# Jerrypiglet/monosdf

Measured on AMD Instinct MI355X. Metric: rays/sec fwd+bwd, 1024 rays x 98 samples, 8x256 SDF MLP, higher is better.
Workload: dtype f32; 1 GPU; configs[1]: 1024 rays x 98 samples per GPU, ImplicitNetwork 8x256 + RenderingNetwork 289-256-256-3, error-bounded sampler, random-init weights (density beta 0.1), training step = fwd + loss + bwd + Adam, a different one of 8 ray batches every step; rays_per_gpu=1024, samples_per_ray=98, ray_batches=8, matrix_core=fp32

## Files before the change

### include/monosdf_hip.h

```cpp
#ifndef MONOSDF_HIP_H
#define MONOSDF_HIP_H

#include <stdint.h>
#include "monosdf_plan.h"

#ifdef __cplusplus
extern "C" {
#endif

#define MSDF_OK 0
#define MSDF_ERR_ARG 1
#define MSDF_ERR_LAUNCH 2
#define MSDF_ERR_UNSUPPORTED 3

#define MSDF_ABI_VERSION 8
int msdf_abi_version(void);

int msdf_hash_encode_forward(const float* inputs, const float* embeddings, const int* offsets, float* outputs,
                             uint32_t B, uint32_t D, uint32_t C, uint32_t L, float S, uint32_t H,
                             int calc_grad_inputs, float* dy_dx, void* stream);
int msdf_hash_encode_backward(const float* grad, const float* inputs, const float* embeddings, const int* offsets,
                              float* grad_embeddings, uint32_t B, uint32_t D, uint32_t C, uint32_t L, float S,
                              uint32_t H, int calc_grad_inputs, const float* dy_dx, float* grad_inputs,
                              void* stream);
int msdf_hash_encode_second_backward(const float* grad, const float* inputs, const float* embeddings,
                                     const int* offsets, uint32_t B, uint32_t D, uint32_t C, uint32_t L, float S,
                                     uint32_t H, int calc_grad_inputs, const float* dy_dx,
                                     const float* grad_grad_inputs, float* grad_grad, float* grad2_embeddings,
                                     void* stream);

int64_t msdf_hash_scatter_workspace_bytes(uint32_t B, uint32_t C, uint32_t L, uint64_t n_entries);
int msdf_hash_encode_backward_ws(const float* grad, const float* inputs, const float* embeddings, const int* offsets,
                                 float* grad_embeddings, uint32_t B, uint32_t D, uint32_t C, uint32_t L, float S,
                                 uint32_t H, int calc_grad_inputs, const float* dy_dx, float* grad_inputs,
                                 uint64_t n_entries, void* workspace, uint64_t workspace_bytes, void* stream);
int msdf_hash_encode_second_backward_ws(const float* grad, const float* inputs, const float* embeddings,
                                        const int* offsets, uint32_t B, uint32_t D, uint32_t C, uint32_t L, float S,
                                        uint32_t H, int calc_grad_inputs, const float* dy_dx,
                                        const float* grad_grad_inputs, float* grad_grad, float* grad2_embeddings,
                                        uint64_t n_entries, void* workspace, uint64_t workspace_bytes, void* stream);
int msdf_hash_encode_backward_fused(const float* grad_first, const float* grad_second, const float* inputs,
                                    const int* offsets, float* grad_embeddings, uint32_t B, uint32_t D, uint32_t C,
                                    uint32_t L, float S, uint32_t H, const float* grad_grad_inputs,
                                    uint64_t n_entries, void* workspace, uint64_t workspace_bytes, void* stream);
int msdf_hash_encode_backward_fused_out(const float* grad_first, const float* grad_second, const float* inputs,
                                        const int* offsets, float* grad_embeddings, uint32_t B, uint32_t D, uint32_t C,
                                        uint32_t L, float S, uint32_t H, const float* grad_grad_inputs,
                                        uint64_t n_entries, void* workspace, uint64_t workspace_bytes, void* stream);

int msdf_hash_node_forward(const float* x, double divide_factor, float* x01_out, const float* embeddings,
                           const int* offsets, float* feat, uint32_t pitch, uint32_t B, uint32_t C, uint32_t L,
                           float S, uint32_t H, float* dy_dx, void* stream);
int msdf_hash_node_input_gradient(const float* g, uint32_t pitch, const float* dy_dx, uint32_t B, uint32_t C,
                                  uint32_t L, float scale, float* inout, void* stream);
int msdf_hash_node_second_grad(const float* g_a, const float* g_b, uint32_t n_split, float scale, float* gg_out,
                               const float* dy_dx, float* grad_grad, uint32_t pitch, uint32_t B, uint32_t C,
                               uint32_t L, void* stream);
int msdf_hash_transpose(const float* src, float* dst, const float* src2, float* dst2, uint32_t L, uint32_t B,
                        uint32_t C, uint32_t pitch, int to_point_major, void* stream);
int msdf_hash_node_scatter(const float* grad_first, const float* grad_second, uint32_t pitch, const float* inputs,
                           const int* offsets, float* grad_embeddings, uint32_t B, uint32_t C, uint32_t L, float S,
                           uint32_t H, const float* grad_grad_inputs, uint64_t n_entries, void* workspace,
                           uint64_t workspace_bytes, void* stream);

int msdf_pack_weights(const msdf_plan_t* plan, const msdf_packrule_t* rules_dev, const int* maps_dev,
                      const float* flat_w, const float* flat_b, void* wpack, float* bpack, void* stream);

typedef struct {
  const float* v;
  const float* g;
  const float* b;
  int32_t rows, cols;
  int32_t w_off;
  int32_t b_off;
  int32_t row_off;
  int32_t has_g;
} msdf_wn_layer_t;
int msdf_weightnorm_forward(const msdf_wn_layer_t* layers_dev, const int* row_layer_dev, int total_rows,
                            float* flat_w, float* flat_b, float* norms, void* stream);
int msdf_weightnorm_backward(const msdf_wn_layer_t* layers_dev, const int* row_layer_dev, int total_rows,
                             const float* g_flat_w, const float* norms, float* dv_flat, float* dg_rows, void* stream);

int msdf_sdf_forward(const msdf_plan_t* plan, const void* wpack, const float* bpack, const float* x,
                     const float* aux, int P, float clamp_radius, float sphere_scale, float* sdf, void* stream);
int msdf_sdf_forward_if(const msdf_plan_t* plan, const void* wpack, const float* bpack, const float* x,
                        const float* aux, int P, float clamp_radius, float sphere_scale, float* sdf,
                        const uint32_t* run_flag, void* stream);
int msdf_sdf_forward_lm(const msdf_plan_t* plan, const void* wpack, const float* bpack, const float* x,
                        const float* aux, int aux_C, int aux_LC, int P, float clamp_radius, float sphere_scale,
                        float* sdf, const uint32_t* run_flag, void* stream);

typedef struct {
  const void* wpack;
  const float* bpack;
  const float* x;
  const float* aux;
  int32_t P, P_pad;
  int32_t n_clamp;
  int32_t n_feat;
  float clamp_radius, sphere_scale;
  float* sdf;
  float* feat;
  float* nrm;
  float* r_aux;
  unsigned char* clamped;
  float* H;
  float* PM;
  float* IN0;
  int32_t save;
  int32_t aux_C;
  int32_t aux_LC;
  float aux_dx_scale;
  const float* dy_dx;
} msdf_fg_args_t;
int msdf_sdf_fwd_grad(const msdf_plan_t* plan, const msdf_fg_args_t* args, void* stream);

typedef struct {
  const void* wpack;
  const float* bpack;
  const float* x;
  int32_t P, P_pad;
  int32_t n_feat;
  int32_t n_split;
  const float* g_sdf;
  const float* g_feat;
  const float* g_nrm;
  const float* g_raux;
  const unsigned char* clamped;
  const float* H;
  const float* PM;
  float* QB;
  float* T;
  float* AB;
  float* GSDF;
  float* QLAST;
  float* g_aux;
  const float* g_sdf_b;
  const float* g_nrm_b;
  int32_t aux_C, aux_LC;
  const float* dy_dx;
  float* gg_out;
  float aux_dx_scale;
  int32_t pad_;
} msdf_bw_args_t;
int msdf_sdf_backward(const msdf_plan_t* plan, const msdf_bw_args_t* args, void* stream);

typedef struct {
  const void* wpack;
  const float* bpack;
  const float* x;
  const float* dirs;
  const float* nrm;
  const float* feat;
  const float* code;
  int32_t P, P_pad;
  int32_t spr;
  int32_t save;
  float* rgb;
  float* H;
  float* MISC;
} msdf_color_fwd_args_t;
int msdf_color_forward(const msdf_plan_t* plan, const msdf_color_fwd_args_t* args, void* stream);

typedef struct {
  const void* wpack;
  const float* bpack;
  const float* rgb;
  const float* g_rgb;
  int32_t P, P_pad;
  const float* H;
  float* AB;
  float* g_feat;
  float* g_misc;
  float* g_nrm;
} msdf_color_bwd_args_t;
int msdf_color_backward(const msdf_plan_t* plan, const msdf_color_bwd_args_t* args, void* stream);

int msdf_wgrad(const msdf_wgrad_item_t* items_dev, const int32_t* wg_map_dev, int n_wgs, float* partials,
               int P_pad, int precision , const float* base0, const float* base1 , void* stream);
int msdf_reduce(const msdf_reduce_rule_t* rules_dev, int n_rules, const int* maps_dev, const float* partials,
                float* dst, void* stream);

typedef struct {
  const float* z;
  const float* sdf;
  const float* rgb;
  const float* nrm;
  const float* beta;
  const float* depth_scale;
  int32_t N, S;
  int32_t white_bkgd;
  float bg0, bg1, bg2;
  float* weights;
  float* rgb_values;
  float* depth_values;
  float* normal_map;
  float* wsum;
  const float* pose;
  int32_t pose_stride;
  int32_t depth_scale_stride;
  float* depth_vals;
} msdf_composite_args_t;
int msdf_composite_forward(const msdf_composite_args_t* args, void* stream);

typedef struct {
  const float* z;
  const float* sdf;
  const float* rgb;
  const float* nrm;
  const float* beta;
  const float* depth_scale;
  const float* weights;
  const float* wsum;
  const float* depth_values;
  const float* g_rgb_values;
  const float* g_depth;
  const float* g_normal;
  const float* g_weights;
  int32_t N, S;
  int32_t white_bkgd;
  float bg0, bg1, bg2;
  float* g_sdf;
  float* g_rgb;
  float* g_nrm;
  float* g_beta_part;
  const float* pose;
  int32_t pose_stride;
  int32_t depth_scale_stride;
} msdf_composite_bwd_args_t;
int msdf_composite_backward(const msdf_composite_bwd_args_t* args, void* stream);

int msdf_beta_eff(const float* beta_raw, float beta_min, float* out, void* stream);
int msdf_beta_grad(const float* beta_raw, const float* g_part, int n, float* g_raw, void* stream);

typedef struct {
  const float* rgb;
  const float* nrm;
  const float* depth;
  const float* g1;
  const float* g2;
  int32_t N, M;
  float w_normal, w_depth, w_eik, w_smooth;
  float* g_rgb; float* g_nrm; float* g_depth; float* g_g1; float* g_g2;
  float* partial;
} msdf_probe_loss_args_t;
int msdf_probe_loss(const msdf_probe_loss_args_t* args, void* stream);

typedef struct {
  const float* rgb;
  const float* depth;
  const float* normal;
  const float* sdf;
  const float* grad_theta;
  const float* grad_nei;
  const float* rgb_gt;
  const float* depth_gt;
  const float* normal_gt;
  const float* mask_gt;
  int32_t N, S, E;
  int32_t gamma;
  int32_t scale_invariant;
  float w_eik, w_smooth, w_depth, w_nl1, w_ncos;
  float* mask;
  float* out;
  float* g_rgb; float* g_depth; float* g_normal; float* g_theta; float* g_nei;
} msdf_monosdf_loss_args_t;
int msdf_monosdf_loss(const msdf_monosdf_loss_args_t* args, void* stream);

typedef struct {
  const float* ray_o;
  const float* ray_d;
  int32_t N;
  int32_t M;
  int32_t m_max;
  int32_t n_eval, n_final, n_extra;
  int32_t round_idx, max_rounds;
  int32_t training;
  int32_t beta_iters;
  float near, far, bound;
  float eps, add_tiny;
  float lemma;
  const float* beta0;
  float* z;
  float* sdf;
  float* new_z;
  const float* new_sdf;
  int32_t* new_pos;
  float* pts;
  float* beta;
  uint32_t* flags;
  const float* jitter;
  const float* u_final;
  float* final_z;
  const int64_t* extra_idx;
  const int64_t* eik_idx;
  float* z_out;
  float* z_eik;
  float* pts_out;
  const float* eik_uniform;
  const float* nei_rand;
  float* far_out;
  int32_t* rounds_out;
  float* dbg_dstar;
  float* dbg_err0;
  float* dbg_cdf;
  const float* eik_u;
  int32_t eik_unit;
  int32_t pad_;
} msdf_sampler_args_t;
int msdf_sampler_init(const msdf_sampler_args_t* args, void* stream);
int msdf_sampler_beta(const msdf_sampler_args_t* args, void* stream);
int msdf_sampler_resample(const msdf_sampler_args_t* args, void* stream);
int msdf_sampler_finish(const msdf_sampler_args_t* args, void* stream);

int msdf_sampler_error_bound(const float* z, const float* sdf, const float* dstar, const float* beta,
                             int beta_stride, int N, int M, float* out, void* stream);

int msdf_laplace_density(const float* sdf, const float* beta, int beta_stride, int64_t n, int cols, float* out,
                         void* stream);
int msdf_laplace_density_backward(const float* sdf, const float* beta, int beta_stride, int64_t n, int cols,
                                  const float* g, float* g_sdf, float* g_beta_elem, void* stream);

int msdf_camera_rays(const float* uv, const float* pose, const float* intrinsics, int n, float* ray_dirs,
                     float* ray_dirs_cam, float* cam_loc, void* stream);

int msdf_pixel_rays(const int64_t* ray_idx, int n, const int32_t* frame_list, int n_frames, const float* pose_all,
                    const float* intrinsics_all, int width, int hw, float* ray_dirs, float* ray_dirs_cam,
                    float* cam_loc, float* ray_pose, int32_t* frame_pos, const float* const* gt_src,
                    float* const* gt_dst, const int32_t* gt_channels, int n_gt, void* stream);

int64_t msdf_mc_workspace_bytes(int nx, int ny, int nz);
int msdf_mc_count(const float* vol, int nx, int ny, int nz, float level, void* workspace, int64_t* totals,
                  void* stream);
int msdf_mc_emit(const float* vol, int nx, int ny, int nz, float level, float sx, float sy, float sz,
                 const void* workspace, float* verts, float* normals, int32_t* faces, void* stream);

int msdf_nn_split_count(int64_t n_ref, int64_t n_query, int n_splits);
int64_t msdf_nn_workspace_bytes(int64_t n_ref, int64_t n_query, int n_splits);
int msdf_nn_search(const float* ref, int64_t n_ref, const float* query, int64_t n_query, int n_splits,
                   void* workspace, float* dist, int32_t* idx, void* stream);
int msdf_voxel_keys(const float* points, int64_t n, const float* min_bound, float voxel_size, int64_t* keys,
                    void* stream);
int msdf_voxel_mean(const float* points, const int64_t* order, const int64_t* seg_start, int64_t n, int64_t m,
                    float* out, void* stream);

int msdf_raster_depth(const float* verts, int64_t n_verts, const int32_t* faces, int64_t n_faces, const float* w2c,
                      int n_views, float fx, float fy, float cx, float cy, int height, int width, float znear,
                      float zfar, float pixel_center, float* depth, void* stream);
int msdf_tsdf_integrate(const float* depth, const float* w2c, int n_views, float fx, float fy, float cx, float cy,
                        int height, int width, float ox, float oy, float oz, int i0, int j0, int k0, int nx, int ny,
                        int nz, float voxel_length, float sdf_trunc, float depth_trunc, int resume, float* tsdf,
                        float* weight, void* stream);
int msdf_tsdf_face_keep(const float* verts, int64_t n_verts, const int32_t* faces, int64_t n_faces,
                        const float* weight, int nx, int ny, int nz, uint8_t* keep, void* stream);
int msdf_cull_vertices(const float* verts, int64_t n_verts, const float* w2c, int n_views, float fx, float fy, float cx,
                       float cy, int height, int width, uint8_t* seen, void* stream);

#ifdef __cplusplus
}
#endif
#endif
```

### monosdf_amd/_lib.py

```python
import ctypes as C
import os

_HERE = os.path.dirname(os.path.abspath(__file__))
LIB_PATH = os.environ.get('MONOSDF_HIP_LIB') or os.path.join(_HERE, 'libmonosdf_hip.so')

MAX_LAYERS = 10
MAX_TILES = 17


class Layer(C.Structure):
    _fields_ = [(n, C.c_int32) for n in
                ('kt', 'ot', 'wf_off', 'wb_off', 'bias_off', 'skip_tile', 'hpre', 'qpre', 'abpre',
                 'ktp', 'otp', 'pad_')]


class Plan(C.Structure):
    _fields_ = [(n, C.c_int32) for n in
                ('n_layers', 'e_tiles', 'aux_tiles', 'n_freqs', 'sdf_slot', 'feat_tiles', 'hsum',
                 'qsum', 'absum', 'wsdf_off', 'mode', 'out_act', 'precision', 'out_rows')] + [('layer', Layer * MAX_LAYERS)]


class PackRule(C.Structure):
    _fields_ = [('w_off', C.c_int32), ('b_off', C.c_int32), ('rows', C.c_int32), ('cols', C.c_int32),
                ('rowmap_off', C.c_int32), ('colmap_off', C.c_int32), ('scale', C.c_float),
                ('pad_', C.c_int32)]


class WgradItem(C.Structure):
    _fields_ = [('x', C.c_int64), ('y', C.c_int64), ('v', C.c_int64),
                ('part_off', C.c_int64), ('colsum_off', C.c_int64), ('vrow_off', C.c_int64),
                ('x_ld', C.c_int32), ('y_ld', C.c_int32), ('wx', C.c_int32), ('wy', C.c_int32),
                ('n_splits', C.c_int32), ('bufs', C.c_int32)]


class ReduceRule(C.Structure):
    _fields_ = [('part_off', C.c_int64), ('dst_off', C.c_int64), ('n_blocks', C.c_int32),
                ('wx', C.c_int32), ('wy', C.c_int32), ('rowmap_off', C.c_int32),
                ('colmap_off', C.c_int32), ('dst_ld', C.c_int32), ('fixed_row', C.c_int32),
                ('scale', C.c_float)]


_P = C.c_void_p


class FgArgs(C.Structure):
    _fields_ = [('wpack', _P), ('bpack', _P), ('x', _P), ('aux', _P),
                ('P', C.c_int32), ('P_pad', C.c_int32), ('n_clamp', C.c_int32), ('n_feat', C.c_int32),
                ('clamp_radius', C.c_float), ('sphere_scale', C.c_float),
                ('sdf', _P), ('feat', _P), ('nrm', _P), ('r_aux', _P), ('clamped', _P),
                ('H', _P), ('PM', _P), ('IN0', _P), ('save', C.c_int32), ('aux_C', C.c_int32), ('aux_LC', C.c_int32),
                ('aux_dx_scale', C.c_float), ('dy_dx', _P)]


class BwArgs(C.Structure):
    _fields_ = [('wpack', _P), ('bpack', _P), ('x', _P),
                ('P', C.c_int32), ('P_pad', C.c_int32), ('n_feat', C.c_int32), ('n_split', C.c_int32),
                ('g_sdf', _P), ('g_feat', _P), ('g_nrm', _P), ('g_raux', _P), ('clamped', _P),
                ('H', _P), ('PM', _P), ('QB', _P), ('T', _P), ('AB', _P), ('GSDF', _P), ('QLAST', _P),
                ('g_aux', _P), ('g_sdf_b', _P), ('g_nrm_b', _P), ('aux_C', C.c_int32), ('aux_LC', C.c_int32),
                ('dy_dx', _P), ('gg_out', _P), ('aux_dx_scale', C.c_float), ('pad_', C.c_int32)]


class ColorFwdArgs(C.Structure):
    _fields_ = [('wpack', _P), ('bpack', _P), ('x', _P), ('dirs', _P), ('nrm', _P), ('feat', _P),
                ('code', _P), ('P', C.c_int32), ('P_pad', C.c_int32), ('spr', C.c_int32),
                ('save', C.c_int32), ('rgb', _P), ('H', _P), ('MISC', _P)]


class ColorBwdArgs(C.Structure):
    _fields_ = [('wpack', _P), ('bpack', _P), ('rgb', _P), ('g_rgb', _P),
                ('P', C.c_int32), ('P_pad', C.c_int32), ('H', _P), ('AB', _P), ('g_feat', _P),
                ('g_misc', _P), ('g_nrm', _P)]


class CompositeArgs(C.Structure):
    _fields_ = [('z', _P), ('sdf', _P), ('rgb', _P), ('nrm', _P), ('beta', _P), ('depth_scale', _P),
                ('N', C.c_int32), ('S', C.c_int32), ('white_bkgd', C.c_int32),
                ('bg0', C.c_float), ('bg1', C.c_float), ('bg2', C.c_float),
                ('weights', _P), ('rgb_values', _P), ('depth_values', _P), ('normal_map', _P),
                ('wsum', _P), ('pose', _P), ('pose_stride', C.c_int32), ('depth_scale_stride', C.c_int32),
                ('depth_vals', _P)]


class CompositeBwdArgs(C.Structure):
    _fields_ = [('z', _P), ('sdf', _P), ('rgb', _P), ('nrm', _P), ('beta', _P), ('depth_scale', _P),
                ('weights', _P), ('wsum', _P), ('depth_values', _P), ('g_rgb_values', _P),
                ('g_depth', _P), ('g_normal', _P), ('g_weights', _P),
                ('N', C.c_int32), ('S', C.c_int32), ('white_bkgd', C.c_int32),
                ('bg0', C.c_float), ('bg1', C.c_float), ('bg2', C.c_float),
                ('g_sdf', _P), ('g_rgb', _P), ('g_nrm', _P), ('g_beta_part', _P),
                ('pose', _P), ('pose_stride', C.c_int32), ('depth_scale_stride', C.c_int32)]


class WnLayer(C.Structure):
    _fields_ = [('v', _P), ('g', _P), ('b', _P), ('rows', C.c_int32), ('cols', C.c_int32),
                ('w_off', C.c_int32), ('b_off', C.c_int32), ('row_off', C.c_int32), ('has_g', C.c_int32)]


class ProbeLossArgs(C.Structure):
    _fields_ = [('rgb', _P), ('nrm', _P), ('depth', _P), ('g1', _P), ('g2', _P), ('N', C.c_int32), ('M', C.c_int32),
                ('w_normal', C.c_float), ('w_depth', C.c_float), ('w_eik', C.c_float), ('w_smooth', C.c_float),
                ('g_rgb', _P), ('g_nrm', _P), ('g_depth', _P), ('g_g1', _P), ('g_g2', _P), ('partial', _P)]


class MonoSdfLossArgs(C.Structure):
    _fields_ = [(n, _P) for n in ('rgb', 'depth', 'normal', 'sdf', 'grad_theta', 'grad_nei', 'rgb_gt', 'depth_gt',
                                  'normal_gt', 'mask_gt')] + \
               [(n, C.c_int32) for n in ('N', 'S', 'E', 'gamma', 'scale_invariant')] + \
               [(n, C.c_float) for n in ('w_eik', 'w_smooth', 'w_depth', 'w_nl1', 'w_ncos')] + \
               [(n, _P) for n in ('mask', 'out', 'g_rgb', 'g_depth', 'g_normal', 'g_theta', 'g_nei')]


class SamplerArgs(C.Structure):
    _fields_ = [('ray_o', _P), ('ray_d', _P), ('N', C.c_int32), ('M', C.c_int32), ('m_max', C.c_int32),
                ('n_eval', C.c_int32), ('n_final', C.c_int32), ('n_extra', C.c_int32),
                ('round_idx', C.c_int32), ('max_rounds', C.c_int32), ('training', C.c_int32),
                ('beta_iters', C.c_int32), ('near', C.c_float), ('far', C.c_float), ('bound', C.c_float),
                ('eps', C.c_float), ('add_tiny', C.c_float), ('lemma', C.c_float),
                ('beta0', _P), ('z', _P), ('sdf', _P), ('new_z', _P), ('new_sdf', _P), ('new_pos', _P),
                ('pts', _P), ('beta', _P), ('flags', _P), ('jitter', _P), ('u_final', _P), ('final_z', _P),
                ('extra_idx', _P), ('eik_idx', _P), ('z_out', _P), ('z_eik', _P), ('pts_out', _P),
                ('eik_uniform', _P), ('nei_rand', _P), ('far_out', _P), ('rounds_out', _P),
                ('dbg_dstar', _P), ('dbg_err0', _P), ('dbg_cdf', _P), ('eik_u', _P), ('eik_unit', C.c_int32),
                ('pad_', C.c_int32)]


_ERR = {1: 'invalid argument', 2: 'kernel launch failed', 3: 'unsupported configuration'}

_SIGNATURES = {
    'msdf_abi_version': [],
    'msdf_hash_encode_forward': [_P, _P, _P, _P, C.c_uint32, C.c_uint32, C.c_uint32, C.c_uint32,
                                 C.c_float, C.c_uint32, C.c_int, _P, _P],
    'msdf_hash_encode_backward': [_P, _P, _P, _P, _P, C.c_uint32, C.c_uint32, C.c_uint32, C.c_uint32,
                                  C.c_float, C.c_uint32, C.c_int, _P, _P, _P],
    'msdf_hash_encode_second_backward': [_P, _P, _P, _P, C.c_uint32, C.c_uint32, C.c_uint32,
                                         C.c_uint32, C.c_float, C.c_uint32, C.c_int, _P, _P, _P, _P, _P],
    'msdf_hash_scatter_workspace_bytes': [C.c_uint32, C.c_uint32, C.c_uint32, C.c_uint64],
    'msdf_hash_encode_backward_ws': [_P, _P, _P, _P, _P, C.c_uint32, C.c_uint32, C.c_uint32, C.c_uint32,
                                     C.c_float, C.c_uint32, C.c_int, _P, _P, C.c_uint64, _P, C.c_uint64, _P],
    'msdf_hash_encode_second_backward_ws': [_P, _P, _P, _P, C.c_uint32, C.c_uint32, C.c_uint32, C.c_uint32,
                                            C.c_float, C.c_uint32, C.c_int, _P, _P, _P, _P, C.c_uint64, _P,
                                            C.c_uint64, _P],
    'msdf_hash_encode_backward_fused': [_P, _P, _P, _P, _P, C.c_uint32, C.c_uint32, C.c_uint32, C.c_uint32,
                                        C.c_float, C.c_uint32, _P, C.c_uint64, _P, C.c_uint64, _P],
    'msdf_hash_encode_backward_fused_out': [_P, _P, _P, _P, _P, C.c_uint32, C.c_uint32, C.c_uint32, C.c_uint32,
                                            C.c_float, C.c_uint32, _P, C.c_uint64, _P, C.c_uint64, _P],
    'msdf_hash_node_forward': [_P, C.c_double, _P, _P, _P, _P, C.c_uint32, C.c_uint32, C.c_uint32, C.c_uint32,
                               C.c_float, C.c_uint32, _P, _P],
    'msdf_hash_node_input_gradient': [_P, C.c_uint32, _P, C.c_uint32, C.c_uint32, C.c_uint32, C.c_float, _P, _P],
    'msdf_hash_node_second_grad': [_P, _P, C.c_uint32, C.c_float, _P, _P, _P, C.c_uint32, C.c_uint32, C.c_uint32,
                                   C.c_uint32, _P],
    'msdf_hash_transpose': [_P, _P, _P, _P, C.c_uint32, C.c_uint32, C.c_uint32, C.c_uint32, C.c_int, _P],
    'msdf_hash_node_scatter': [_P, _P, C.c_uint32, _P, _P, _P, C.c_uint32, C.c_uint32, C.c_uint32, C.c_float,
                               C.c_uint32, _P, C.c_uint64, _P, C.c_uint64, _P],
    'msdf_weightnorm_forward': [_P, _P, C.c_int, _P, _P, _P, _P],
    'msdf_weightnorm_backward': [_P, _P, C.c_int, _P, _P, _P, _P, _P],
    'msdf_pack_weights': [C.POINTER(Plan), _P, _P, _P, _P, _P, _P, _P],
    'msdf_sdf_forward': [C.POINTER(Plan), _P, _P, _P, _P, C.c_int, C.c_float, C.c_float, _P, _P],
    'msdf_sdf_forward_if': [C.POINTER(Plan), _P, _P, _P, _P, C.c_int, C.c_float, C.c_float, _P, _P, _P],
    'msdf_sdf_forward_lm': [C.POINTER(Plan), _P, _P, _P, _P, C.c_int, C.c_int, C.c_int, C.c_float, C.c_float, _P, _P, _P],
    'msdf_sdf_fwd_grad': [C.POINTER(Plan), C.POINTER(FgArgs), _P],
    'msdf_sdf_backward': [C.POINTER(Plan), C.POINTER(BwArgs), _P],
    'msdf_color_forward': [C.POINTER(Plan), C.POINTER(ColorFwdArgs), _P],
    'msdf_color_backward': [C.POINTER(Plan), C.POINTER(ColorBwdArgs), _P],
    'msdf_wgrad': [_P, _P, C.c_int, _P, C.c_int, C.c_int, _P, _P, _P],
    'msdf_camera_rays': [_P, _P, _P, C.c_int, _P, _P, _P, _P],
    'msdf_pixel_rays': [_P, C.c_int, _P, C.c_int, _P, _P, C.c_int, C.c_int, _P, _P, _P, _P, _P, _P, _P, _P, C.c_int, _P],
    'msdf_monosdf_loss': [C.POINTER(MonoSdfLossArgs), _P],
    'msdf_reduce': [_P, C.c_int, _P, _P, _P, _P],
    'msdf_composite_forward': [C.POINTER(CompositeArgs), _P],
    'msdf_composite_backward': [C.POINTER(CompositeBwdArgs), _P],
    'msdf_beta_eff': [_P, C.c_float, _P, _P],
    'msdf_beta_grad': [_P, _P, C.c_int, _P, _P],
    'msdf_probe_loss': [C.POINTER(ProbeLossArgs), _P],
    'msdf_sampler_init': [C.POINTER(SamplerArgs), _P],
    'msdf_sampler_beta': [C.POINTER(SamplerArgs), _P],
    'msdf_sampler_resample': [C.POINTER(SamplerArgs), _P],
    'msdf_sampler_finish': [C.POINTER(SamplerArgs), _P],
    'msdf_sampler_error_bound': [_P, _P, _P, _P, C.c_int, C.c_int, C.c_int, _P, _P],
    'msdf_laplace_density': [_P, _P, C.c_int, C.c_int64, C.c_int, _P, _P],
    'msdf_laplace_density_backward': [_P, _P, C.c_int, C.c_int64, C.c_int, _P, _P, _P, _P],
    'msdf_mc_workspace_bytes': [C.c_int, C.c_int, C.c_int],
    'msdf_mc_count': [_P, C.c_int, C.c_int, C.c_int, C.c_float, _P, _P, _P],
    'msdf_mc_emit': [_P, C.c_int, C.c_int, C.c_int, C.c_float, C.c_float, C.c_float, C.c_float, _P, _P, _P, _P, _P],
    'msdf_nn_split_count': [C.c_int64, C.c_int64, C.c_int],
    'msdf_nn_workspace_bytes': [C.c_int64, C.c_int64, C.c_int],
    'msdf_nn_search': [_P, C.c_int64, _P, C.c_int64, C.c_int, _P, _P, _P, _P],
    'msdf_voxel_keys': [_P, C.c_int64, _P, C.c_float, _P, _P],
    'msdf_voxel_mean': [_P, _P, _P, C.c_int64, C.c_int64, _P, _P],
    'msdf_raster_depth': [_P, C.c_int64, _P, C.c_int64, _P, C.c_int, C.c_float, C.c_float, C.c_float, C.c_float,
                          C.c_int, C.c_int, C.c_float, C.c_float, C.c_float, _P, _P],
    'msdf_tsdf_integrate': [_P, _P, C.c_int, C.c_float, C.c_float, C.c_float, C.c_float, C.c_int, C.c_int,
                            C.c_float, C.c_float, C.c_float, C.c_int, C.c_int, C.c_int, C.c_int, C.c_int, C.c_int,
                            C.c_float, C.c_float, C.c_float, C.c_int, _P, _P, _P],
    'msdf_tsdf_face_keep': [_P, C.c_int64, _P, C.c_int64, _P, C.c_int, C.c_int, C.c_int, _P, _P],
    'msdf_cull_vertices': [_P, C.c_int64, _P, C.c_int, C.c_float, C.c_float, C.c_float, C.c_float, C.c_int, C.c_int,
                           _P, _P],
}

ABI_VERSION = 8

_lib = None


def load():
    global _lib
    if _lib is not None:
        return _lib
    if not os.path.exists(LIB_PATH):
        raise RuntimeError(
            'monosdf_amd: %s not found -- build it with `python __graft_entry__.py` or '
            '`make -C monosdf_amd/csrc` (there is no non-HIP fallback)' % LIB_PATH)
    lib = C.CDLL(LIB_PATH)
    for name, argtypes in _SIGNATURES.items():
        fn = getattr(lib, name)
        fn.argtypes = argtypes
        fn.restype = C.c_int64 if name.endswith('_bytes') else C.c_int
    if lib.msdf_abi_version() != ABI_VERSION:
        raise RuntimeError('monosdf_amd: ABI version mismatch, rebuild the library')
    _lib = lib
    return lib


def exported_symbols():
    return sorted(_SIGNATURES)


PROFILE = None


PROFILE_NAMES = None


def call(name, *args):
    prof = PROFILE
    if prof is not None and PROFILE_NAMES is not None and name not in PROFILE_NAMES:
        prof = None
    if prof is not None:
        import torch
        e0, e1 = torch.cuda.Event(enable_timing=True), torch.cuda.Event(enable_timing=True)
        e0.record()
    status = getattr(load(), name)(*args)
    if prof is not None:
        e1.record()
        prof.setdefault(name, []).append((e0, e1))
    if status != 0:
        raise RuntimeError('%s failed: %s' % (name, _ERR.get(status, 'status %d' % status)))


def ptr(t):
    return None if t is None else C.c_void_p(t.data_ptr())


def stream_ptr():
    import torch
    return C.c_void_p(torch.cuda.current_stream().cuda_stream)
```

### monosdf_amd/csrc/mlp_core.h

```cpp
#pragma once
#include <type_traits>
#include "common.h"
#include "../../include/monosdf_plan.h"

#define MT MSDF_MAX_TILES
#ifndef MLP_WAVES
#define MLP_WAVES 4
#endif
#define MLP_PTS_PER_WAVE 16
#define CHUNK_OT 2
#define LDS_BUF_F4 (CHUNK_OT * MT * 64)

#define V4ZERO ((v4f){0.f, 0.f, 0.f, 0.f})

__device__ __forceinline__ v4f mfma4(const v4f a, const v4f b, v4f c) {
  c = __builtin_amdgcn_mfma_f32_16x16x4f32(a.x, b.x, c, 0, 0, 0);
  c = __builtin_amdgcn_mfma_f32_16x16x4f32(a.y, b.y, c, 0, 0, 0);
  c = __builtin_amdgcn_mfma_f32_16x16x4f32(a.z, b.z, c, 0, 0, 0);
  c = __builtin_amdgcn_mfma_f32_16x16x4f32(a.w, b.w, c, 0, 0, 0);
  return c;
}

__device__ __forceinline__ void mfma4_pair(const v4f a0, const v4f a1, const v4f b, v4f& c0, v4f& c1) {
  c0 = __builtin_amdgcn_mfma_f32_16x16x4f32(a0.x, b.x, c0, 0, 0, 0);
// ... 117 lines not shown
        if (!DYN) {
          v4f a0 = w0[0];
          v4f c0 = acc[o0];
#pragma unroll
          for (int kt = 0; kt < KMAX; ++kt) {
            v4f n0 = a0;
            if (kt + 1 < KMAX) n0 = w0[(kt + 1) * 64];
            __builtin_amdgcn_sched_barrier(0);
            c0 = mfma4(a0, in[kt], c0);
            a0 = n0;
          }
          acc[o0] = c0;
        } else {
#pragma unroll
          for (int kt = 0; kt < KMAX; ++kt) {
            if (kt < K) acc[o0] = mfma4(w0[kt * 64], in[kt], acc[o0]);
          }
        }
      }
      hk.post(o0, 2 * c + 1, 2 * c + 1 < MT && 2 * c + 1 < OT, acc[o0], acc[o1]);
        }
      }
      __syncthreads();
    }
  }
}

template <class Hooks>
__device__ __forceinline__ void gemm_dispatch(const int kp, v4f (&acc)[MT], const v4f (&in)[MT], const int OT,
                                              const v4f* __restrict__ wsrc, v4f* lds, Hooks& hk) {
  switch (kp) {
    case 3: gemm_tiles<3, 4>(acc, in, OT, 3, wsrc, lds, hk); break;
    case 5: gemm_tiles<5, 3>(acc, in, OT, 5, wsrc, lds, hk); break;
    case 16: gemm_tiles<16, 1>(acc, in, OT, 16, wsrc, lds, hk); break;
    case 17: gemm_tiles<17, 1>(acc, in, OT, 17, wsrc, lds, hk); break;
    default: gemm_tiles<0, 1>(acc, in, OT, kp, wsrc, lds, hk); break;
  }
  hk.drain();
}

__device__ __forceinline__ void zero_tiles(v4f (&a)[MT]) {
#pragma unroll
  for (int t = 0; t < MT; ++t) a[t] = V4ZERO;
}

__device__ __forceinline__ void place_tiles(v4f (&dst)[MT], const int base, const v4f (&src)[5], const int n) {
#pragma unroll
  for (int t = 0; t < MT; ++t) {
    if (t >= base) {
      v4f v = V4ZERO;
#pragma unroll
      for (int j = 0; j < 5; ++j)
        if (j < n && t == base + j) v = src[j];
      dst[t] = v;
    }
  }
}

__device__ __forceinline__ void gather_tiles(v4f (&dst)[5], const v4f (&src)[MT], const int base, const int n) {
#pragma unroll
  for (int t = 0; t < MT; ++t) {
#pragma unroll
    for (int j = 0; j < 5; ++j)
      if (j < n && t == base + j) dst[j] += src[t];
  }
}

__device__ __forceinline__ void pe_slot(const int j, const int n_valid, const float x0, const float x1,
                                        const float x2, float& val, float& dval, int& c) {
  val = 0.f; dval = 0.f; c = 3;
  if (j < 3) {
    c = j;
    val = (c == 0) ? x0 : (c == 1) ? x1 : x2;
    dval = 1.f;
  } else if (j < n_valid) {
    const int m = j - 3;
    const int k = m / 6;
    const int w = m - 6 * k;
    c = (w >= 3) ? w - 3 : w;
    const float xc = (c == 0) ? x0 : (c == 1) ? x1 : x2;
    const float f = (float)(1 << k);
    float sn, cs;
    sincosf(xc * f, &sn, &cs);
    if (w < 3) { val = sn; dval = f * cs; } else { val = cs; dval = -f * sn; }
  }
}

__device__ __forceinline__ void pe_values(v4f (&e)[5], const float x0, const float x1, const float x2,
                                          const int n_freqs) {
  const int q = lane_id() >> 4;
  const int n_valid = 3 + 6 * n_freqs;
#pragma unroll
  for (int t = 0; t < 3; ++t) {
#pragma unroll
    for (int r = 0; r < 4; ++r) {
      float v, dv; int c;
      pe_slot(16 * t + 4 * q + r, n_valid, x0, x1, x2, v, dv, c);
      e[t][r] = v;
    }
  }
}

__device__ __forceinline__ void pe_jacobian_transpose(const v4f (&r)[5], const float x0, const float x1,
                                                      const float x2, const int n_freqs, float& n0, float& n1,
                                                      float& n2) {
  const int q = lane_id() >> 4;
  const int n_valid = 3 + 6 * n_freqs;
  float a0 = 0.f, a1 = 0.f, a2 = 0.f;
#pragma unroll
  for (int t = 0; t < 3; ++t) {
#pragma unroll
    for (int k = 0; k < 4; ++k) {
      float v, dv; int c;
      pe_slot(16 * t + 4 * q + k, n_valid, x0, x1, x2, v, dv, c);
      const float w = r[t][k] * dv;
      a0 += (c == 0) ? w : 0.f;
      a1 += (c == 1) ? w : 0.f;
      a2 += (c == 2) ? w : 0.f;
    }
  }
  n0 = sum_over_quarters(a0);
  n1 = sum_over_quarters(a1);
  n2 = sum_over_quarters(a2);
}

__device__ __forceinline__ void pe_jacobian(v4f (&rbar)[5], const float x0, const float x1, const float x2,
                                            const int n_freqs, const float g0, const float g1, const float g2) {
  const int q = lane_id() >> 4;
  const int n_valid = 3 + 6 * n_freqs;
#pragma unroll
  for (int t = 0; t < 3; ++t) {
#pragma unroll
    for (int k = 0; k < 4; ++k) {
      float v, dv; int c;
      pe_slot(16 * t + 4 * q + k, n_valid, x0, x1, x2, v, dv, c);
      const float g = (c == 0) ? g0 : (c == 1) ? g1 : (c == 2) ? g2 : 0.f;
      rbar[t][k] = dv * g;
    }
  }
}


struct CoreF32 {
  typedef v4f wvec;
  static constexpr int THREADS = 64 * MLP_WAVES;
  static constexpr int PTS_PER_WG = MLP_PTS_PER_WAVE * MLP_WAVES;
  static constexpr int WGS_PER_CU = 8 / MLP_WAVES;
  static constexpr int LDS_BYTES = 2 * LDS_BUF_F4 * 16;
  static constexpr bool BIAS_IN_HOOKS = true;
#ifndef MLP_F32_AUX_LEVEL_MAJOR
#define MLP_F32_AUX_LEVEL_MAJOR true
#endif
  static constexpr bool AUX_LEVEL_MAJOR = MLP_F32_AUX_LEVEL_MAJOR;
  static __device__ __forceinline__ float softplus(const float a) {
    float h, s;
    softplus100(a, h, s);
    return h;
  }
  template <class Hooks>
  static __device__ __forceinline__ void gemm(const int kp, v4f (&acc)[MT], const v4f (&in)[MT], const int OT,
                                              const wvec* __restrict__ wsrc, void* lds, Hooks&& hk) {
    gemm_dispatch(kp, acc, in, OT, wsrc, (v4f*)lds, hk);
  }
  template <class Hooks>
  static __device__ __forceinline__ void gemm_bias(const int kp, v4f (&acc)[MT], const v4f (&in)[MT], const int OT,
                                                   const wvec* __restrict__ wsrc, void* lds, Hooks&& hk,
                                                   const float* __restrict__ bias) {
    zero_tiles(acc);
    BiasHooks<typename std::remove_reference<Hooks>::type> bh(hk, bias, OT);
    gemm_dispatch(kp, acc, in, OT, wsrc, (v4f*)lds, bh);
  }
};

__device__ __forceinline__ void pack_bias_rows(const msdf_plan_t& plan, const int l, const msdf_packrule_t& R,
                                               const int* __restrict__ rowmap, const int* __restrict__ colmap,
                                               const float* __restrict__ W, const float* __restrict__ flat_b,
                                               float* __restrict__ bpack, const int t0, const int stride) {
  const msdf_layer_t L = plan.layer[l];
  for (int i = t0; i < 16 * L.ot; i += stride) {
    const int row = rowmap[i];
    bpack[L.bias_off + i] = (row >= 0) ? flat_b[R.b_off + row] : 0.f;
  }
  if (l == plan.n_layers - 1 && plan.wsdf_off >= 0) {
    for (int rr = 0; rr < plan.out_rows; ++rr) {
      const int row = rowmap[plan.sdf_slot + rr];
      for (int i = t0; i < 16 * L.kt; i += stride) {
        const int col = colmap[i];
        bpack[plan.wsdf_off + rr * 16 * L.kt + i] = (col >= 0 && row >= 0) ? R.scale * W[(size_t)row * R.cols + col] : 0.f;
      }
    }
  }
}
```

### monosdf_amd/csrc/mlp_core_b16.h

```cpp
#pragma once
#include "mlp_core.h"


typedef __bf16 v8bf __attribute__((ext_vector_type(8)));
typedef __attribute__((address_space(3))) v8bf lds_v8bf;

__device__ __forceinline__ float softplus100_lean(const float a) {
  const float e = __builtin_amdgcn_exp2f(-fabsf(a * 144.26950408889634f));
  const float relu = __int_as_float(max(__float_as_int(a), 0));
  return fmaf(0.006931471805599453f, __builtin_amdgcn_logf(1.0f + e), relu);
}

#define KB_MAX ((MT + 1) / 2)
#define B16_WAVES 4

template <int NS>
struct B16Cfg {
  static_assert(NS == 2 || NS == 3, "two planes (bf16x3) or three (bf16x6)");
  static constexpr int CH = (NS == 2) ? 2 : 1;
  static constexpr int BUF_V8 = CH * KB_MAX * NS * 64;
  static constexpr int RING = (NS == 2) ? 3 : 2;
};

template <int NS>
// ... 37 lines not shown
__device__ __forceinline__ void b16_chunk_issue(const v8bf* __restrict__ src, v8bf* dst, const int n_v8) {
  const int wave = __builtin_amdgcn_readfirstlane(threadIdx.x >> 6);
  const int lane = threadIdx.x & 63;
  const int pieces = n_v8 >> 6;
#pragma unroll
  for (int i = 0; i < (PIECES_MAX + B16_WAVES - 1) / B16_WAVES; ++i) {
    const int piece = wave + B16_WAVES * i;
    if (piece < pieces) {
      __builtin_amdgcn_global_load_lds((const __attribute__((address_space(1))) void*)(src + piece * 64 + lane),
                                       (__attribute__((address_space(3))) void*)(dst + piece * 64), 16, 0, 0);
    }
  }
}

template <int NS>
__device__ __forceinline__ v4f b16_step(v4f c, const v8bf (&f)[NS], const B16Act<NS>& act, const int kb) {
  c = __builtin_amdgcn_mfma_f32_16x16x32_bf16(f[0], act.p[0][kb], c, 0, 0, 0);
  c = __builtin_amdgcn_mfma_f32_16x16x32_bf16(f[0], act.p[1][kb], c, 0, 0, 0);
  c = __builtin_amdgcn_mfma_f32_16x16x32_bf16(f[1], act.p[0][kb], c, 0, 0, 0);
  if constexpr (NS == 3) {
    c = __builtin_amdgcn_mfma_f32_16x16x32_bf16(f[0], act.p[2][kb], c, 0, 0, 0);
    c = __builtin_amdgcn_mfma_f32_16x16x32_bf16(f[1], act.p[1][kb], c, 0, 0, 0);
    c = __builtin_amdgcn_mfma_f32_16x16x32_bf16(f[2], act.p[0][kb], c, 0, 0, 0);
  }
  return c;
}

template <int NS>
__device__ __forceinline__ v4f b16_tile_dyn(v4f c, const v8bf* __restrict__ w, const B16Act<NS>& act, const int KB) {
  v8bf a[NS];
#pragma unroll
  for (int n = 0; n < NS; ++n) a[n] = w[n * 64];
#pragma unroll
  for (int kb = 0; kb < KB_MAX; ++kb) {
    if (kb < KB) {
      v8bf nx[NS];
#pragma unroll
      for (int n = 0; n < NS; ++n) nx[n] = a[n];
      if (kb + 1 < KB_MAX && kb + 1 < KB) {
#pragma unroll
        for (int n = 0; n < NS; ++n) nx[n] = w[((kb + 1) * NS + n) * 64];
      }
      __builtin_amdgcn_sched_barrier(0);
      c = b16_step<NS>(c, a, act, kb);
#pragma unroll
      for (int n = 0; n < NS; ++n) a[n] = nx[n];
    }
  }
  return c;
}

template <int NS, int KB_T, class Hooks>
__device__ __forceinline__ void gemm_b16(v4f (&acc)[MT], const B16Act<NS>& act, const int OT, const int kb_rt,
                                         const v8bf* __restrict__ wsrc, v8bf* lds, Hooks& hk) {
  typedef B16Cfg<NS> Cfg;
  constexpr int CH = Cfg::CH;
  constexpr int RING = Cfg::RING;
  constexpr bool DYN = (KB_T == 0);
  constexpr int KMAX = DYN ? KB_MAX : KB_T;
  const int KB = DYN ? kb_rt : KB_T;
  const int ch_v8 = CH * KB * NS * 64;
  const int lane = threadIdx.x & 63;
  const int nchunks = (OT + CH - 1) / CH;
  constexpr int BUF = Cfg::BUF_V8;
  b16_chunk_issue<CH * KMAX * NS>(wsrc, lds, ch_v8);
  __syncthreads();
#pragma unroll
  for (int c = 0; c < (MT + CH - 1) / CH; ++c) {
    if (c < nchunks) {
      const int buf = c & 1;
      if (c + 1 < nchunks)
        b16_chunk_issue<CH * KMAX * NS>(wsrc + (size_t)(c + 1) * ch_v8, lds + (buf ^ 1) * BUF, ch_v8);
      const int t0 = CH * c;
      if ((t0 & 1) == 0) hk.pre(t0, t0 + 1);
      const v8bf* w = lds + buf * BUF + lane;
      const lds_v8bf* wl0 = (const lds_v8bf*)w;
      asm volatile("" : "+v"(wl0));
      static_assert(BUF * 16 <= 65536, "fragment offsets must fit the ds_read immediate");
#define B16_FRAG(i, plane) (wl0[((i) * NS + (plane)) * 64])
      if constexpr (DYN) {
#pragma unroll
        for (int o = 0; o < CH; ++o) {
          const int ot = CH * c + o;
          if (ot < MT && ot < OT) {
            const int oi = (ot < MT) ? ot : 0;
            acc[oi] = b16_tile_dyn<NS>(acc[oi], w + o * KB * NS * 64, act, KB);
          }
        }
      } else {
        const int n_o = OT - CH * c;
        v8bf fr[RING][NS];
#pragma unroll
        for (int i = 0; i < RING - 1; ++i) {
          if (i < CH * KB_T) {
#pragma unroll
            for (int n = 0; n < NS; ++n) fr[i][n] = B16_FRAG(i, n);
          }
        }
#pragma unroll
        for (int o = 0; o < CH; ++o) {
          const int ot = CH * c + o;
          if (ot < MT && o < n_o) {
            const int oi = (ot < MT) ? ot : 0;
            v4f cc = acc[oi];
#pragma unroll
            for (int kb = 0; kb < KB_T; ++kb) {
              const int i = o * KB_T + kb;
              if (i + RING - 1 < CH * KB_T) {
#pragma unroll
                for (int n = 0; n < NS; ++n) fr[(i + RING - 1) % RING][n] = B16_FRAG(i + RING - 1, n);
              }
              __builtin_amdgcn_sched_barrier(0);
              cc = b16_step<NS>(cc, fr[i % RING], act, kb);
            }
            acc[oi] = cc;
          }
        }
      }
#undef B16_FRAG
      const int t_last = CH * c + CH - 1;
      if ((t_last & 1) == 1 || t_last + 1 >= OT) {
        const int e = t_last & ~1;
        if (e < MT)
          hk.post(e, e + 1, e + 1 < MT && e + 1 < OT, acc[e < MT ? e : 0], acc[(e + 1 < MT) ? e + 1 : 0]);
      }
      __syncthreads();
    }
  }
}

template <int NS, class Hooks>
__device__ __forceinline__ void gemm_b16_dispatch(const int kbp, v4f (&acc)[MT], const B16Act<NS>& act, const int OT,
                                                  const v8bf* __restrict__ wsrc, v8bf* lds, Hooks& hk) {
  switch (kbp) {
    case 2: gemm_b16<NS, 2>(acc, act, OT, 2, wsrc, lds, hk); break;
    case 3: gemm_b16<NS, 3>(acc, act, OT, 3, wsrc, lds, hk); break;
    case 8: gemm_b16<NS, 8>(acc, act, OT, 8, wsrc, lds, hk); break;
    case 9: gemm_b16<NS, 9>(acc, act, OT, 9, wsrc, lds, hk); break;
    default: gemm_b16<NS, 0>(acc, act, OT, kbp, wsrc, lds, hk); break;
  }
  hk.drain();
}

template <int NS>
struct CoreB16N {
  typedef v8bf wvec;
  static constexpr int PLANES = NS;
  static constexpr int THREADS = 64 * B16_WAVES;
  static constexpr int PTS_PER_WG = MLP_PTS_PER_WAVE * B16_WAVES;
  static constexpr int WGS_PER_CU = 2;
  static constexpr int LDS_BYTES = 2 * B16Cfg<NS>::BUF_V8 * 16;
  static constexpr bool BIAS_IN_HOOKS = (NS == 3);
  static constexpr bool AUX_LEVEL_MAJOR = false;
  static __device__ __forceinline__ float softplus(const float a) {
    if constexpr (NS == 2) return softplus100_lean(a);
    float h, s;
    softplus100(a, h, s);
    return h;
  }
  template <class Hooks>
  static __device__ __forceinline__ void gemm(const int kbp, v4f (&acc)[MT], const v4f (&in)[MT], const int OT,
                                              const wvec* __restrict__ wsrc, void* lds, Hooks&& hk) {
    B16Act<NS> act;
    b16_from_tiles<NS>(act, in);
    gemm_b16_dispatch<NS>(kbp, acc, act, OT, wsrc, (v8bf*)lds, hk);
  }
  template <class Hooks>
  static __device__ __forceinline__ void gemm_bias(const int kbp, v4f (&acc)[MT], const v4f (&in)[MT], const int OT,
                                                   const wvec* __restrict__ wsrc, void* lds, Hooks&& hk,
                                                   const float* __restrict__ bias) {
    B16Act<NS> act;
    b16_from_tiles<NS>(act, in);
    zero_tiles(acc);
    BiasHooks<typename std::remove_reference<Hooks>::type> bh(hk, bias, OT);
    gemm_b16_dispatch<NS>(kbp, acc, act, OT, wsrc, (v8bf*)lds, bh);
  }
};
typedef CoreB16N<2> CoreB16;
typedef CoreB16N<3> CoreB16X6;
```

### monosdf_amd/csrc/sampler.hip

```cpp
#include "common.h"

#define SMP_WAVES 4

__device__ __forceinline__ float smp_scan_incl(float v) {
  const int lane = lane_id();
#pragma unroll
  for (int d = 1; d < 64; d <<= 1) {
    const float o = __shfl_up(v, d, 64);
    if (lane >= d) v += o;
  }
  return v;
}
__device__ __forceinline__ float smp_sum(float v) {
#pragma unroll
  for (int d = 32; d >= 1; d >>= 1) v += __shfl_xor(v, d, 64);
  return v;
}
__device__ __forceinline__ float smp_max(float v) {
#pragma unroll
  for (int d = 32; d >= 1; d >>= 1) v = fmaxf(v, __shfl_xor(v, d, 64));
  return v;
}
__device__ __forceinline__ float smp_density(const float s, const float beta) {
  const float e = expm1f(-fabsf(s) / beta);
  const float sg = (s > 0.f) ? 1.f : (s < 0.f) ? -1.f : 0.f;
  return (1.0f / beta) * (0.5f + 0.5f * sg * e);
}
__device__ __forceinline__ float smp_linspace01(const int j, const int n) {
  const float step = 1.0f / (float)(n - 1);
  return (j < n / 2) ? step * (float)j : 1.0f - step * (float)(n - 1 - j);
}

typedef msdf_sampler_args_t SmpArgs;

__global__ void __launch_bounds__(64 * SMP_WAVES) smp_init_k(const SmpArgs a) {
  const int ray = blockIdx.x * SMP_WAVES + (threadIdx.x >> 6);
  if (ray >= a.N) return;
  const int lane = lane_id();
  if (ray == 0 && a.flags != nullptr)
    for (int i = lane; i < 2 * a.max_rounds; i += 64) a.flags[i] = 0u;
  const int n = a.n_eval;
  const float o0 = a.ray_o[ray * 3 + 0], o1 = a.ray_o[ray * 3 + 1], o2 = a.ray_o[ray * 3 + 2];
  const float d0 = a.ray_d[ray * 3 + 0], d1 = a.ray_d[ray * 3 + 1], d2 = a.ray_d[ray * 3 + 2];
  const float ta0 = (-a.bound - o0) / (d0 + 1e-15f), tb0 = (a.bound - o0) / (d0 + 1e-15f);
  const float ta1 = (-a.bound - o1) / (d1 + 1e-15f), tb1 = (a.bound - o1) / (d1 + 1e-15f);
  const float ta2 = (-a.bound - o2) / (d2 + 1e-15f), tb2 = (a.bound - o2) / (d2 + 1e-15f);
  float near_c = fmaxf(fmaxf(fminf(ta0, tb0), fminf(ta1, tb1)), fminf(ta2, tb2));
  float far_c = fminf(fminf(fmaxf(ta0, tb0), fmaxf(ta1, tb1)), fmaxf(ta2, tb2));
  if (far_c < near_c) far_c = 1e9f;
  const float far = (a.bound > 0.f) ? fminf(far_c, a.far) : a.far;
  const float near = a.near;
  float sumsq = 0.f;
  float* zrow = a.z + (size_t)ray * a.m_max;
  auto zu = [&](int k) { const float t = smp_linspace01(k, n); return near * (1.f - t) + far * t; };
  auto zfin = [&](int k) {
    float z = zu(k);
    if (a.jitter != nullptr) {
      const float zl = (k > 0) ? 0.5f * (zu(k) + zu(k - 1)) : zu(0);
      const float zh = (k + 1 < n) ? 0.5f * (zu(k + 1) + zu(k)) : zu(n - 1);
      z = zl + (zh - zl) * a.jitter[(size_t)ray * n + k];
    }
    return z;
  };
  for (int j = lane; j < n; j += 64) {
    const float z = zfin(j);
    zrow[j] = z;
    a.new_z[(size_t)ray * n + j] = z;
    a.new_pos[(size_t)ray * n + j] = j;
    float* p = a.pts + ((size_t)ray * n + j) * 3;
    p[0] = o0 + z * d0; p[1] = o1 + z * d1; p[2] = o2 + z * d2;
    if (j + 1 < n) {
      const float dz = zfin(j + 1) - z;
      sumsq += dz * dz;
    }
  }
  sumsq = smp_sum(sumsq);
  if (lane == 0) {
    a.beta[ray] = sqrtf(a.lemma * sumsq);
    if (a.far_out != nullptr) a.far_out[ray] = far;
  }
}

struct SmpLds {
  float* z; float* sdf; float* dist; float* dstar; float* tmp; float* snew;
};
__device__ __forceinline__ SmpLds smp_lds(float* base, const int m_max, const int n_eval) {
  const int w = threadIdx.x >> 6;
  const int per = 5 * (m_max + 1) + n_eval;
  float* p = base + (size_t)w * per;
  SmpLds l;
  l.z = p; l.sdf = p + (m_max + 1); l.dist = p + 2 * (m_max + 1); l.dstar = p + 3 * (m_max + 1);
  l.tmp = p + 4 * (m_max + 1); l.snew = p + 5 * (m_max + 1);
  return l;
}
__device__ __forceinline__ void smp_sync() {
  __builtin_amdgcn_fence(__ATOMIC_RELEASE, "workgroup");
  __builtin_amdgcn_wave_barrier();
  __builtin_amdgcn_fence(__ATOMIC_ACQUIRE, "workgroup");
}

__device__ __forceinline__ bool smp_round_active(const SmpArgs& a) {
  return a.round_idx == 0 || a.flags[2 * (a.round_idx - 1) + 1] != 0u;
}

__device__ __forceinline__ void smp_load_ray(const SmpArgs& a, const SmpLds& l, const int ray, const bool scatter) {
  const int lane = lane_id();
  const int M = a.M;
  const float* zrow = a.z + (size_t)ray * a.m_max;
  float* srow = a.sdf + (size_t)ray * a.m_max;
  for (int i = lane; i < M; i += 64) { l.z[i] = zrow[i]; l.sdf[i] = srow[i]; }
  smp_sync();
  if (scatter) {
    for (int j = lane; j < a.n_eval; j += 64)
      l.sdf[a.new_pos[(size_t)ray * a.n_eval + j]] = a.new_sdf[(size_t)ray * a.n_eval + j];
    smp_sync();
    for (int i = lane; i < M; i += 64) srow[i] = l.sdf[i];
  }
  for (int i = lane; i + 1 < M; i += 64) {
    const float aa = l.z[i + 1] - l.z[i];
    const float b = fabsf(l.sdf[i]), c = fabsf(l.sdf[i + 1]);
    const bool first = aa * aa + b * b <= c * c;
    const bool second = aa * aa + c * c <= b * b;
    float ds = 0.f;
    if (first) ds = b;
    if (second) ds = c;
    if (!first && !second && (b + c - aa > 0.f)) {
      const float s = (aa + b + c) / 2.0f;
      const float area = s * (s - aa) * (s - b) * (s - c);
      ds = (2.0f * sqrtf(area)) / aa;
    }
    const float s0 = l.sdf[i], s1 = l.sdf[i + 1];
    const float sg0 = (s0 > 0.f) ? 1.f : (s0 < 0.f) ? -1.f : 0.f;
    const float sg1 = (s1 > 0.f) ? 1.f : (s1 < 0.f) ? -1.f : 0.f;
    l.dist[i] = aa;
    const float dsv = (sg0 * sg1 == 1.f) ? ds : 0.f;
    l.dstar[i] = dsv;
    if (scatter && a.dbg_dstar != nullptr) a.dbg_dstar[(size_t)ray * a.m_max + i] = dsv;
  }
  smp_sync();
}

__device__ __forceinline__ float smp_error_bound(const SmpLds& l, const int M, const float beta) {
  const int lane = lane_id();
  float carry_fe = 0.f, carry_err = 0.f, best = -1e30f;
  const float inv4b2 = 1.0f / (4.0f * beta * beta);
  for (int base = 0; base < M - 1; base += 64) {
    const int i = base + lane;
    const bool ok = i < M - 1;
    float fe = 0.f, er = 0.f;
    if (ok) {
      const float d = l.dist[i];
      fe = d * smp_density(l.sdf[i], beta);
      er = expf(-l.dstar[i] / beta) * (d * d) * inv4b2;
    }
    const float fe_incl = smp_scan_incl(fe);
    const float er_incl = smp_scan_incl(er);
    if (ok) {
      const float integral = carry_fe + fe_incl - fe;
      const float errint = carry_err + er_incl;
      const float bound = (fminf(expf(errint), 1.0e6f) - 1.0f) * expf(-integral);
      best = fmaxf(best, bound);
    }
    carry_fe += __shfl(fe_incl, 63, 64);
    carry_err += __shfl(er_incl, 63, 64);
  }
  return smp_max(best);
}

__global__ void __launch_bounds__(64 * SMP_WAVES) smp_beta_k(const SmpArgs a) {
  extern __shared__ float smp_lds_mem[];
  const int ray = blockIdx.x * SMP_WAVES + (threadIdx.x >> 6);
  if (ray >= a.N || !smp_round_active(a)) return;
  const SmpLds l = smp_lds(smp_lds_mem, a.m_max, a.n_eval);
  smp_load_ray(a, l, ray, true);
  const float beta0 = a.beta0[0];
  float beta = a.beta[ray];
  const float e0 = smp_error_bound(l, a.M, beta0);
  if (a.dbg_err0 != nullptr && lane_id() == 0) a.dbg_err0[ray] = e0;
  if (e0 <= a.eps) beta = beta0;
  float lo = beta0, hi = beta;
  const int iters = (e0 <= a.eps) ? 0 : a.beta_iters;
  for (int it = 0; it < iters; ++it) {
    const float mid = (lo + hi) / 2.0f;
    const float e = smp_error_bound(l, a.M, mid);
    if (e <= a.eps) hi = mid;
    if (e > a.eps) lo = mid;
  }
  if (lane_id() == 0) {
    a.beta[ray] = hi;
    atomicMax(a.flags + 2 * a.round_idx, __float_as_uint(hi));
  }
}

__global__ void __launch_bounds__(64 * SMP_WAVES) smp_resample_k(const SmpArgs a) {
  extern __shared__ float smp_lds_mem[];
  const int ray = blockIdx.x * SMP_WAVES + (threadIdx.x >> 6);
  if (ray >= a.N || !smp_round_active(a)) return;
  const int lane = lane_id();
  const int M = a.M;
  const SmpLds l = smp_lds(smp_lds_mem, a.m_max, a.n_eval);
  const float beta0 = a.beta0[0];
  const float maxbeta = __uint_as_float(a.flags[2 * a.round_idx]);
  const bool unconverged = maxbeta > beta0;
  const bool more = unconverged && (a.round_idx + 1 < a.max_rounds);
  if (ray == 0 && lane == 0) a.flags[2 * a.round_idx + 1] = more ? 1u : 0u;
  smp_load_ray(a, l, ray, false);
  const float beta = a.beta[ray];
  const float inv4b2 = 1.0f / (4.0f * beta * beta);

  float carry_fe = 0.f, carry_err = 0.f, psum = 0.f;
  for (int base = 0; base < M; base += 64) {
    const int i = base + lane;
    const bool ok = i < M;
    float fe = 0.f, er = 0.f;
    if (ok) {
      const float d = (i + 1 < M) ? l.dist[i] : 1e10f;
      fe = d * smp_density(l.sdf[i], beta);
      if (more && i + 1 < M) er = expf(-l.dstar[i] / beta) * (l.dist[i] * l.dist[i]) * inv4b2;
    }
    float fprev = __shfl_up(fe, 1, 64);
    if (lane == 0) fprev = 0.f;
    const float fe_excl = smp_scan_incl(fprev);
    const float fe_incl = fe_excl + fe;
    const float er_incl = smp_scan_incl(er);
    if (ok && i + 1 < M) {
      const float trans = expf(-(carry_fe + fe_excl));
      float p;
      if (more) p = (fminf(expf(carry_err + er_incl), 1.0e6f) - 1.0f) * trans + a.add_tiny;
      else p = (1.0f - expf(-fe)) * trans + 1e-5f;
      l.tmp[i] = p;
      psum += p;
    }
    carry_fe += __shfl(fe_incl, 63, 64);
    carry_err += __shfl(er_incl, 63, 64);
  }
  psum = smp_sum(psum);
  smp_sync();
  float carry = 0.f;
  for (int base = 0; base < M - 1; base += 64) {
    const int i = base + lane;
    const float p = (i < M - 1) ? l.tmp[i] / psum : 0.f;
    const float incl = smp_scan_incl(p);
    if (i < M - 1) l.dstar[i + 1] = carry + incl;
    carry += __shfl(incl, 63, 64);
  }
  if (lane == 0) l.dstar[0] = 0.f;
  smp_sync();
  const float* cdf = l.dstar;
  if (a.dbg_cdf != nullptr)
    for (int i = lane; i < M; i += 64) a.dbg_cdf[(size_t)ray * a.m_max + i] = cdf[i];

  const int n_new = more ? a.n_eval : a.n_final;
  for (int j = lane; j < n_new; j += 64) {
    float u;
    if (more || !a.training || a.u_final == nullptr) u = smp_linspace01(j, n_new);
    else u = a.u_final[(size_t)ray * a.n_final + j];
    int lo = 0, hi = M;
    while (lo < hi) {
      const int mid = (lo + hi) >> 1;
      if (cdf[mid] <= u) lo = mid + 1; else hi = mid;
    }
    const int below = max(lo - 1, 0), above = min(lo, M - 1);
    float denom = cdf[above] - cdf[below];
    if (denom < 1e-5f) denom = 1.0f;
    const float t = (u - cdf[below]) / denom;
    const float s = l.z[below] + t * (l.z[above] - l.z[below]);
    l.snew[j] = s;
  }
  smp_sync();

  if (!more) {
    for (int j = lane; j < n_new; j += 64) a.final_z[(size_t)ray * a.n_final + j] = l.snew[j];
    return;
  }
  const float o0 = a.ray_o[ray * 3 + 0], o1 = a.ray_o[ray * 3 + 1], o2 = a.ray_o[ray * 3 + 2];
  const float d0 = a.ray_d[ray * 3 + 0], d1 = a.ray_d[ray * 3 + 1], d2 = a.ray_d[ray * 3 + 2];
  float* zrow = a.z + (size_t)ray * a.m_max;
  float* srow = a.sdf + (size_t)ray * a.m_max;
  for (int i = lane; i < M; i += 64) {
    const float zi = l.z[i];
    int cnt = 0;
    for (int k = 0; k < n_new; ++k) cnt += (l.snew[k] < zi) ? 1 : 0;
    zrow[i + cnt] = zi;
    srow[i + cnt] = l.sdf[i];
  }
  for (int j = lane; j < n_new; j += 64) {
    const float sj = l.snew[j];
    int cnt = 0;
    for (int i = 0; i < M; ++i) cnt += (l.z[i] <= sj) ? 1 : 0;
    for (int k = 0; k < n_new; ++k) cnt += (l.snew[k] < sj || (l.snew[k] == sj && k < j)) ? 1 : 0;
    zrow[cnt] = sj;
    a.new_z[(size_t)ray * a.n_eval + j] = sj;
    a.new_pos[(size_t)ray * a.n_eval + j] = cnt;
    float* p = a.pts + ((size_t)ray * a.n_eval + j) * 3;
    p[0] = o0 + sj * d0; p[1] = o1 + sj * d1; p[2] = o2 + sj * d2;
  }
}

__global__ void __launch_bounds__(64 * SMP_WAVES) smp_finish_k(const SmpArgs a) {
  extern __shared__ float smp_lds_mem[];
  const int ray = blockIdx.x * SMP_WAVES + (threadIdx.x >> 6);
  if (ray >= a.N) return;
  const int lane = lane_id();
  const int S = a.n_final + a.n_extra + 2;
  float* v = smp_lds_mem + (size_t)(threadIdx.x >> 6) * 2 * S;
  float* sorted = v + S;
  const float* zrow = a.z + (size_t)ray * a.m_max;
  int rounds = 1;
  while (rounds < a.max_rounds && a.flags[2 * (rounds - 1) + 1] != 0u) ++rounds;
  const int64_t* extra = a.extra_idx + (size_t)(rounds - 1) * a.n_extra;
  if (a.rounds_out != nullptr && ray == 0 && lane == 0) a.rounds_out[0] = rounds;
  for (int j = lane; j < S; j += 64) {
    float x;
    if (j < a.n_final) x = a.final_z[(size_t)ray * a.n_final + j];
    else if (j == a.n_final) x = a.near;
    else if (j == a.n_final + 1) x = a.far;
    else x = zrow[min((int)extra[j - a.n_final - 2], rounds * a.n_eval - 1)];
    v[j] = x;
  }
  smp_sync();
  const float o0 = a.ray_o[ray * 3 + 0], o1 = a.ray_o[ray * 3 + 1], o2 = a.ray_o[ray * 3 + 2];
  const float d0 = a.ray_d[ray * 3 + 0], d1 = a.ray_d[ray * 3 + 1], d2 = a.ray_d[ray * 3 + 2];
  for (int j = lane; j < S; j += 64) {
    const float x = v[j];
    int r = 0;
    for (int k = 0; k < S; ++k) r += (v[k] < x || (v[k] == x && k < j)) ? 1 : 0;
    sorted[r] = x;
    a.z_out[(size_t)ray * S + r] = x;
    if (a.pts_out != nullptr) {
      float* p = a.pts_out + ((size_t)ray * S + r) * 3;
      p[0] = o0 + x * d0; p[1] = o1 + x * d1; p[2] = o2 + x * d2;
    }
  }
  smp_sync();
  if (lane == 0) {
    const int idx = (a.eik_idx != nullptr) ? (int)a.eik_idx[ray]
                    : (a.eik_u != nullptr) ? min(S - 1, (int)(a.eik_u[ray] * (float)S)) : 0;
    const float ze = sorted[idx];
    if (a.z_eik != nullptr) a.z_eik[ray] = ze;
    if (a.pts_out != nullptr && a.eik_uniform != nullptr) {
      float* e = a.pts_out + (size_t)a.N * S * 3;
      const float od[3] = {o0 + ze * d0, o1 + ze * d1, o2 + ze * d2};
#pragma unroll
      for (int c = 0; c < 3; ++c) {
        float u = a.eik_uniform[(size_t)ray * 3 + c];
        if (a.eik_unit) u = (2.0f * u - 1.0f) * a.bound;
        e[((size_t)ray) * 3 + c] = u;
        e[((size_t)a.N + ray) * 3 + c] = od[c];
        e[((size_t)2 * a.N + ray) * 3 + c] = u + (a.nei_rand[(size_t)ray * 3 + c] - 0.5f) * 0.01f;
        e[((size_t)3 * a.N + ray) * 3 + c] = od[c] + (a.nei_rand[((size_t)a.N + ray) * 3 + c] - 0.5f) * 0.01f;
      }
    }
  }
}

__global__ void __launch_bounds__(64 * SMP_WAVES) smp_error_bound_k(const float* __restrict__ z,
                                                                     const float* __restrict__ sdf,
                                                                     const float* __restrict__ dstar,
                                                                     const float* __restrict__ beta, const int beta_stride,
                                                                     const int N, const int M, float* __restrict__ out) {
  extern __shared__ float smp_lds_mem[];
  const int ray = blockIdx.x * SMP_WAVES + (threadIdx.x >> 6);
  if (ray >= N) return;
  const int lane = lane_id();
  const SmpLds l = smp_lds(smp_lds_mem, M, 0);
  for (int i = lane; i < M; i += 64) { l.z[i] = z[(size_t)ray * M + i]; l.sdf[i] = sdf[(size_t)ray * M + i]; }
  smp_sync();
  for (int i = lane; i + 1 < M; i += 64) {
    l.dist[i] = l.z[i + 1] - l.z[i];
    l.dstar[i] = dstar[(size_t)ray * (M - 1) + i];
  }
  smp_sync();
  const float e = smp_error_bound(l, M, beta[(size_t)ray * beta_stride]);
  if (lane == 0) out[ray] = e;
}

__global__ void __launch_bounds__(256) laplace_density_k(const float* __restrict__ sdf, const float* __restrict__ beta,
                                                         const int beta_stride, const int64_t n, const int cols,
                                                         float* __restrict__ out) {
  for (int64_t i = (int64_t)blockIdx.x * 256 + threadIdx.x; i < n; i += (int64_t)gridDim.x * 256)
    out[i] = smp_density(sdf[i], beta[(i / cols) * beta_stride]);
}
__global__ void __launch_bounds__(256) laplace_density_bwd_k(const float* __restrict__ sdf, const float* __restrict__ beta,
                                                             const int beta_stride, const int64_t n, const int cols,
                                                             const float* __restrict__ g, float* __restrict__ g_sdf,
                                                             float* __restrict__ g_beta_elem) {
  for (int64_t i = (int64_t)blockIdx.x * 256 + threadIdx.x; i < n; i += (int64_t)gridDim.x * 256) {
    const float s = sdf[i], b = beta[(i / cols) * beta_stride], gi = g[i];
    const float a = fabsf(s);
    const float ex = expf(-a / b);
    const float sg = (s > 0.f) ? 1.f : (s < 0.f) ? -1.f : 0.f;
    g_sdf[i] = gi * (1.0f / b) * 0.5f * sg * ex * (-sg / b);
    const float em1 = expm1f(-a / b);
    g_beta_elem[i] = gi * (-(1.0f / (b * b)) * (0.5f + 0.5f * sg * em1) + (1.0f / b) * 0.5f * sg * ex * (a / (b * b)));
  }
}

static int smp_check(const msdf_sampler_args_t* a) {
  if (a == nullptr || a->N < 0 || a->n_eval < 2 || a->m_max < a->n_eval) return MSDF_ERR_ARG;
  return MSDF_OK;
}
static size_t smp_lds_bytes(const msdf_sampler_args_t* a) {
  return (size_t)SMP_WAVES * (5 * (a->m_max + 1) + a->n_eval) * sizeof(float);
}
template <typename K>
static int smp_launch(K kernel, const msdf_sampler_args_t* a, size_t lds, void* stream) {
  if (a->N == 0) return MSDF_OK;
  if (lds > 160 * 1024) return MSDF_ERR_UNSUPPORTED;
  if (lds > 48 * 1024 &&
      hipFuncSetAttribute((const void*)kernel, hipFuncAttributeMaxDynamicSharedMemorySize, (int)lds) != hipSuccess)
    return MSDF_ERR_LAUNCH;
  kernel<<<(a->N + SMP_WAVES - 1) / SMP_WAVES, 64 * SMP_WAVES, lds, (hipStream_t)stream>>>(*a);
  return msdf_check_launch();
}

extern "C" int msdf_sampler_init(const msdf_sampler_args_t* a, void* stream) {
  if (smp_check(a)) return MSDF_ERR_ARG;
  return smp_launch(smp_init_k, a, 0, stream);
}
static int smp_round_check(const msdf_sampler_args_t* a) {
  return a->flags == nullptr || a->round_idx < 0 || a->round_idx >= a->max_rounds || a->M > a->m_max || a->M < 2;
}
extern "C" int msdf_sampler_beta(const msdf_sampler_args_t* a, void* stream) {
  if (smp_check(a) || smp_round_check(a)) return MSDF_ERR_ARG;
  return smp_launch(smp_beta_k, a, smp_lds_bytes(a), stream);
}
extern "C" int msdf_sampler_resample(const msdf_sampler_args_t* a, void* stream) {
  if (smp_check(a) || smp_round_check(a) || a->n_final > a->n_eval) return MSDF_ERR_ARG;
  return smp_launch(smp_resample_k, a, smp_lds_bytes(a), stream);
}
extern "C" int msdf_sampler_finish(const msdf_sampler_args_t* a, void* stream) {
  if (smp_check(a) || a->flags == nullptr || (a->extra_idx == nullptr && a->n_extra > 0) ||
      a->m_max < a->n_eval * a->max_rounds)
    return MSDF_ERR_ARG;
  const size_t lds = (size_t)SMP_WAVES * 2 * (a->n_final + a->n_extra + 2) * sizeof(float);
  return smp_launch(smp_finish_k, a, lds, stream);
}

extern "C" int msdf_sampler_error_bound(const float* z, const float* sdf, const float* dstar, const float* beta,
                                        int beta_stride, int N, int M, float* out, void* stream) {
  if (N < 0 || M < 2 || (beta_stride != 0 && beta_stride != 1)) return MSDF_ERR_ARG;
  if (N == 0) return MSDF_OK;
  const size_t lds = (size_t)SMP_WAVES * 5 * (M + 1) * sizeof(float);
  if (lds > 160 * 1024) return MSDF_ERR_UNSUPPORTED;
  if (lds > 48 * 1024 && hipFuncSetAttribute((const void*)smp_error_bound_k,
                                             hipFuncAttributeMaxDynamicSharedMemorySize, (int)lds) != hipSuccess)
    return MSDF_ERR_LAUNCH;
  smp_error_bound_k<<<(N + SMP_WAVES - 1) / SMP_WAVES, 64 * SMP_WAVES, lds, (hipStream_t)stream>>>(
      z, sdf, dstar, beta, beta_stride, N, M, out);
  return msdf_check_launch();
}

static int dens_grid(int64_t n) { return (int)((n + 255) / 256 < 2048 ? (n + 255) / 256 : 2048); }
extern "C" int msdf_laplace_density(const float* sdf, const float* beta, int beta_stride, int64_t n, int cols,
                                    float* out, void* stream) {
  if (n < 0 || cols < 1 || (beta_stride != 0 && beta_stride != 1)) return MSDF_ERR_ARG;
  if (n == 0) return MSDF_OK;
  laplace_density_k<<<dens_grid(n), 256, 0, (hipStream_t)stream>>>(sdf, beta, beta_stride, n, cols, out);
  return msdf_check_launch();
}
extern "C" int msdf_laplace_density_backward(const float* sdf, const float* beta, int beta_stride, int64_t n, int cols,
                                             const float* g, float* g_sdf, float* g_beta_elem, void* stream) {
  if (n < 0 || cols < 1 || (beta_stride != 0 && beta_stride != 1)) return MSDF_ERR_ARG;
  if (n == 0) return MSDF_OK;
  laplace_density_bwd_k<<<dens_grid(n), 256, 0, (hipStream_t)stream>>>(sdf, beta, beta_stride, n, cols, g, g_sdf,
                                                                     g_beta_elem);
  return msdf_check_launch();
}
```

### monosdf_amd/csrc/sdf_kernels.h

```cpp
#pragma once
#include "mlp_core.h"

struct PointCtx {
  int pt;
  int ptc;
  bool valid;
  int q;
  float x0, x1, x2;
};

template <class Core>
__device__ __forceinline__ PointCtx load_point(const float* __restrict__ x, const int P) {
  PointCtx c;
  const int lane = lane_id();
  const int wave = threadIdx.x >> 6;
  c.pt = blockIdx.x * Core::PTS_PER_WG + wave * MLP_PTS_PER_WAVE + (lane & 15);
  c.valid = c.pt < P;
  c.ptc = c.valid ? c.pt : (P - 1);
  c.q = lane >> 4;
  c.x0 = x[(size_t)c.ptc * 3 + 0];
  c.x1 = x[(size_t)c.ptc * 3 + 1];
  c.x2 = x[(size_t)c.ptc * 3 + 2];
  return c;
}

struct AuxView {
  int C, LC, P;
};
typedef float v2f_aux __attribute__((ext_vector_type(2)));

template <bool LM>
__device__ __forceinline__ v4f aux_load_tile(const float* __restrict__ base, const AuxView av, const int aux_tiles,
                                             const int t, const int pt, const int q) {
  const int s0 = 16 * t + 4 * q;
  if (!LM || av.C == 0) return *(const v4f*)(base + (size_t)pt * (16 * aux_tiles) + s0);
  const int l = (s0 < av.LC) ? (s0 >> 1) : 0;
  const v2f_aux a = *(const v2f_aux*)(base + ((size_t)l * av.P + pt) * 2);
  const v2f_aux b = *(const v2f_aux*)(base + ((size_t)(l + (s0 + 2 < av.LC ? 1 : 0)) * av.P + pt) * 2);
  v4f v = (v4f){a.x, a.y, b.x, b.y};
  if (s0 >= av.LC) v = V4ZERO;
  else if (s0 + 2 >= av.LC) { v.z = 0.f; v.w = 0.f; }
  return v;
}

template <bool LM>
__device__ __forceinline__ void aux_store_tile(float* __restrict__ base, const AuxView av, const int aux_tiles,
                                               const int t, const int pt, const int q, const v4f v) {
  const int s0 = 16 * t + 4 * q;
  if (!LM || av.C == 0) { *(v4f*)(base + (size_t)pt * (16 * aux_tiles) + s0) = v; return; }
  if (s0 >= av.LC) return;
  const int l = s0 >> 1;
  *(v2f_aux*)(base + ((size_t)l * av.P + pt) * 2) = (v2f_aux){v.x, v.y};
  if (s0 + 2 < av.LC) *(v2f_aux*)(base + ((size_t)(l + 1) * av.P + pt) * 2) = (v2f_aux){v.z, v.w};
}

__device__ __forceinline__ void aux_jacobian_transpose(const float* __restrict__ dy_dx, const AuxView av,
                                                       const int aux_tiles, const v4f (&r)[2], const int pt, const int q,
                                                       float& m0, float& m1, float& m2) {
  m0 = m1 = m2 = 0.f;
#pragma unroll
  for (int t = 0; t < 2; ++t) {
#pragma unroll
    for (int h = 0; h < 2; ++h) {
      const int s0 = 16 * t + 4 * q + 2 * h;
      if (t < aux_tiles && s0 < av.LC) {
        const float* d = dy_dx + ((size_t)(s0 >> 1) * av.P + pt) * 6;
        const v2f_aux j0 = *(const v2f_aux*)d, j1 = *(const v2f_aux*)(d + 2), j2 = *(const v2f_aux*)(d + 4);
        const float g0 = r[t][2 * h], g1 = r[t][2 * h + 1];
        m0 += g0 * j0.x + g1 * j0.y;
        m1 += g0 * j1.x + g1 * j1.y;
        m2 += g0 * j2.x + g1 * j2.y;
      }
    }
  }
}

__device__ __forceinline__ v4f aux_jacobian_tile(const float* __restrict__ dy_dx, const AuxView av, const int t,
                                                 const int pt, const int q, const float g0, const float g1, const float g2) {
  v4f v = V4ZERO;
#pragma unroll
  for (int h = 0; h < 2; ++h) {
    const int s0 = 16 * t + 4 * q + 2 * h;
    if (s0 < av.LC) {
      const float* d = dy_dx + ((size_t)(s0 >> 1) * av.P + pt) * 6;
      const v2f_aux j0 = *(const v2f_aux*)d, j1 = *(const v2f_aux*)(d + 2), j2 = *(const v2f_aux*)(d + 4);
      v[2 * h] = __fadd_rn(__fadd_rn(__fmul_rn(g0, j0.x), __fmul_rn(g1, j1.x)), __fmul_rn(g2, j2.x));
      v[2 * h + 1] = __fadd_rn(__fadd_rn(__fmul_rn(g0, j0.y), __fmul_rn(g1, j1.y)), __fmul_rn(g2, j2.y));
    }
  }
  return v;
}

template <bool LM>
__device__ __forceinline__ void load_input_tiles(v4f (&in0)[5], const msdf_plan_t& plan,
                                                 const float* __restrict__ aux, const AuxView av, const PointCtx& c) {
  pe_values(in0, c.x0, c.x1, c.x2, plan.n_freqs);
  in0[3] = in0[4] = V4ZERO;
  if (plan.aux_tiles > 0) {
#pragma unroll
    for (int t = 0; t < 2; ++t)
      if (t < plan.aux_tiles) in0[3 + t] = aux_load_tile<LM>(aux, av, plan.aux_tiles, t, c.ptc, c.q);
  }
}

__device__ __forceinline__ float sdf_row_dot(const v4f (&in)[MT], const msdf_plan_t& plan,
                                             const float* __restrict__ bpack, const int q) {
  const msdf_layer_t LL = plan.layer[plan.n_layers - 1];
  float part = 0.f;
#pragma unroll
  for (int t = 0; t < MT; ++t) {
    if (t < LL.kt) {
      const v4f w = *(const v4f*)(bpack + plan.wsdf_off + 16 * t + 4 * q);
      part += w.x * in[t].x + w.y * in[t].y + w.z * in[t].z + w.w * in[t].w;
    }
  }
  return sum_over_quarters(part) + bpack[LL.bias_off + plan.sdf_slot];
}

struct PendingStores {
  float* dst;
  v4f s0, s1;
  int t0, n;
  __device__ __forceinline__ void issue() {
    if (n > 0) *(v4f*)(dst + 16 * t0) = s0;
    if (n > 1) *(v4f*)(dst + 16 * t0 + 16) = s1;
    n = 0;
  }
};

template <class Core>
struct SoftplusHooks {
  __device__ __forceinline__ void pre(const int, const int) {}
  __device__ __forceinline__ void post(const int, const int, const bool pair, v4f& a0, v4f& a1) {
#pragma unroll
    for (int r = 0; r < 4; ++r) a0[r] = Core::softplus(a0[r]);
    if (pair) {
#pragma unroll
      for (int r = 0; r < 4; ++r) a1[r] = Core::softplus(a1[r]);
    }
  }
  __device__ __forceinline__ void drain() {}
};

template <class Core>
struct SoftplusSaveHooks {
  PendingStores st;
  __device__ __forceinline__ SoftplusSaveHooks(float* H) { st.dst = H; st.n = 0; st.t0 = 0; }
  __device__ __forceinline__ void pre(const int, const int) { st.issue(); }
  __device__ __forceinline__ void post(const int o0, const int, const bool pair, v4f& a0, v4f& a1) {
#pragma unroll
    for (int r = 0; r < 4; ++r) a0[r] = Core::softplus(a0[r]);
    st.s0 = a0; st.t0 = o0; st.n = 1;
    if (pair) {
#pragma unroll
      for (int r = 0; r < 4; ++r) a1[r] = Core::softplus(a1[r]);
      st.s1 = a1; st.n = 2;
    }
  }
  __device__ __forceinline__ void drain() { st.issue(); }
};

struct GradSweepHooks {
  const float* H;
  int ot;
  bool save;
  v4f h0, h1;
  PendingStores st;
  __device__ __forceinline__ GradSweepHooks(const float* H_, float* PM, const int ot_, const bool save_)
      : H(H_), ot(ot_), save(save_) { st.dst = PM; st.n = 0; st.t0 = 0; }
  __device__ __forceinline__ void pre(const int o0, const int o1) {
    st.issue();
    if (ot > 0) {
      h0 = *(const v4f*)(H + 16 * (o0 < ot ? o0 : ot - 1));
      h1 = *(const v4f*)(H + 16 * (o1 < ot ? o1 : ot - 1));
    }
  }
  __device__ __forceinline__ void post(const int o0, const int o1, const bool pair, v4f& a0, v4f& a1) {
    if (o0 < ot) {
#pragma unroll
      for (int r = 0; r < 4; ++r) a0[r] = (1.0f - one_minus_sigmoid_from_h(h0[r])) * a0[r];
      st.s0 = a0; st.t0 = o0; st.n = save ? 1 : 0;
      if (pair && o1 < ot) {
#pragma unroll
        for (int r = 0; r < 4; ++r) a1[r] = (1.0f - one_minus_sigmoid_from_h(h1[r])) * a1[r];
        st.s1 = a1; st.n = save ? 2 : 0;
      }
    }
  }
  __device__ __forceinline__ void drain() { st.issue(); }
};

struct SweepUpHooks {
  const float* H;
  int ot;
  v4f h0, h1;
  __device__ __forceinline__ SweepUpHooks(const float* H_, const int ot_) : H(H_), ot(ot_) {}
  __device__ __forceinline__ void pre(const int o0, const int o1) {
    const int c0 = o0 < ot ? o0 : ot - 1, c1 = o1 < ot ? o1 : ot - 1;
    h0 = *(const v4f*)(H + 16 * c0);
    h1 = *(const v4f*)(H + 16 * c1);
  }
  __device__ __forceinline__ void post(const int, const int, const bool pair, v4f& a0, v4f& a1) {
#pragma unroll
    for (int r = 0; r < 4; ++r) a0[r] = (1.0f - one_minus_sigmoid_from_h(h0[r])) * a0[r];
    if (pair) {
#pragma unroll
      for (int r = 0; r < 4; ++r) a1[r] = (1.0f - one_minus_sigmoid_from_h(h1[r])) * a1[r];
    }
  }
  __device__ __forceinline__ void drain() {}
};

struct SweepDownHooks {
  const float* H;
  const float* PM;
  const float* Q;
  int ot;
  v4f h0, h1, p0, p1, q0, q1;
  PendingStores st;
  __device__ __forceinline__ SweepDownHooks(const float* H_, const float* PM_, const float* Q_, float* AB, const int ot_)
      : H(H_), PM(PM_), Q(Q_), ot(ot_) { st.dst = AB; st.n = 0; st.t0 = 0; }
  __device__ __forceinline__ void pre(const int o0, const int o1) {
    st.issue();
    if (ot > 0) {
      const int c0 = o0 < ot ? o0 : ot - 1, c1 = o1 < ot ? o1 : ot - 1;
      h0 = *(const v4f*)(H + 16 * c0);
      h1 = *(const v4f*)(H + 16 * c1);
      p0 = *(const v4f*)(PM + 16 * c0);
      p1 = *(const v4f*)(PM + 16 * c1);
      q0 = *(const v4f*)(Q + 16 * c0);
      q1 = *(const v4f*)(Q + 16 * c1);
    }
  }
  static __device__ __forceinline__ void tile(const v4f h, const v4f p, const v4f q, v4f& a) {
#pragma unroll
    for (int r = 0; r < 4; ++r) {
      const float u = one_minus_sigmoid_from_h(h[r]);
      const float sg = 1.0f - u;
      const float pb = (sg > 0.f) ? q[r] * __builtin_amdgcn_rcpf(sg) : 0.f;
      a[r] = a[r] * sg + 100.0f * u * p[r] * pb;
    }
  }
  __device__ __forceinline__ void post(const int o0, const int o1, const bool pair, v4f& a0, v4f& a1) {
    if (o0 < ot) {
      tile(h0, p0, q0, a0);
      st.s0 = a0; st.t0 = o0; st.n = 1;
      if (pair && o1 < ot) {
        tile(h1, p1, q1, a1);
        st.s1 = a1; st.n = 2;
      }
    }
  }
  __device__ __forceinline__ void drain() { st.issue(); }
};

template <class Core>
__device__ __forceinline__ void sdf_forward_body(const msdf_plan_t& plan, const typename Core::wvec* __restrict__ wpack,
                                                 const float* __restrict__ bpack, const float* __restrict__ x,
                                                 const float* __restrict__ aux, const AuxView av, const int P,
                                                 const float clamp_radius, const float sphere_scale,
                                                 float* __restrict__ sdf_out, void* lds) {
  const PointCtx c = load_point<Core>(x, P);
  v4f in[MT], acc[MT];
  const int in0_tiles = plan.e_tiles + plan.aux_tiles;
  {
    v4f in0[5];
    load_input_tiles<Core::AUX_LEVEL_MAJOR>(in0, plan, aux, av, c);
    place_tiles(in, 0, in0, in0_tiles);
  }
  const int nl = plan.n_layers;
  for (int l = 0; l < nl - 1; ++l) {
    const msdf_layer_t L = plan.layer[l];
    if (L.skip_tile >= 0) {
      v4f in0[5];
      load_input_tiles<Core::AUX_LEVEL_MAJOR>(in0, plan, aux, av, c);
      place_tiles(in, L.skip_tile, in0, in0_tiles);
    }
    if constexpr (Core::BIAS_IN_HOOKS) {
      Core::gemm_bias(L.ktp, acc, in, L.ot, wpack + L.wf_off, lds, SoftplusHooks<Core>(), bpack + L.bias_off + 4 * c.q);
    } else {
      load_bias(acc, bpack + L.bias_off, L.ot, c.q);
      Core::gemm(L.ktp, acc, in, L.ot, wpack + L.wf_off, lds, SoftplusHooks<Core>());
    }
#pragma unroll
    for (int t = 0; t < MT; ++t) in[t] = (t < L.ot) ? acc[t] : V4ZERO;
  }
  float sdf = sdf_row_dot(in, plan, bpack, c.q);
  if (clamp_radius > 0.f) {
    const float nx = sqrtf(c.x0 * c.x0 + c.x1 * c.x1 + c.x2 * c.x2);
    sdf = fminf(sdf, sphere_scale * (clamp_radius - nx));
  }
  if (c.valid && c.q == 0) sdf_out[c.pt] = sdf;
}

typedef msdf_fg_args_t FgArgs;

template <class Core>
__device__ __forceinline__ void sdf_fwd_grad_body(const msdf_plan_t& plan, const FgArgs& a, void* lds) {
  typedef typename Core::wvec wvec;
  const PointCtx c = load_point<Core>(a.x, a.P);
  const AuxView av = {a.aux_C, a.aux_LC, a.P};
  v4f in[MT], acc[MT];
  const int nl = plan.n_layers;
  const int in0_tiles = plan.e_tiles + plan.aux_tiles;
  const size_t Pp = (size_t)a.P_pad;
  {
    v4f in0[5];
    load_input_tiles<Core::AUX_LEVEL_MAJOR>(in0, plan, a.aux, av, c);
    place_tiles(in, 0, in0, in0_tiles);
    if (a.save) {
#pragma unroll
      for (int t = 0; t < 5; ++t)
        if (t < in0_tiles) *(v4f*)(a.IN0 + (size_t)c.pt * (16 * in0_tiles) + 16 * t + 4 * c.q) = in0[t];
    }
  }
  const bool want_feat = (int)(blockIdx.x * Core::PTS_PER_WG) < a.n_feat;

  for (int l = 0; l < nl - 1; ++l) {
    const msdf_layer_t L = plan.layer[l];
    if (L.skip_tile >= 0) {
      v4f in0[5];
      load_input_tiles<Core::AUX_LEVEL_MAJOR>(in0, plan, a.aux, av, c);
      place_tiles(in, L.skip_tile, in0, in0_tiles);
    }
    float* Hl = a.H + (size_t)L.hpre * Pp + (size_t)c.pt * (16 * L.ot) + 4 * c.q;
    if constexpr (Core::BIAS_IN_HOOKS) {
      Core::gemm_bias(L.ktp, acc, in, L.ot, (const wvec*)a.wpack + L.wf_off, lds, SoftplusSaveHooks<Core>(Hl),
                      a.bpack + L.bias_off + 4 * c.q);
    } else {
      load_bias(acc, a.bpack + L.bias_off, L.ot, c.q);
      Core::gemm(L.ktp, acc, in, L.ot, (const wvec*)a.wpack + L.wf_off, lds, SoftplusSaveHooks<Core>(Hl));
    }
#pragma unroll
    for (int t = 0; t < MT; ++t) in[t] = (t < L.ot) ? acc[t] : V4ZERO;
  }
  const msdf_layer_t LL = plan.layer[nl - 1];
  float sdf;
  if (want_feat) {
    if constexpr (Core::BIAS_IN_HOOKS) {
      Core::gemm_bias(LL.ktp, acc, in, LL.ot, (const wvec*)a.wpack + LL.wf_off, lds, NoHooks(),
                      a.bpack + LL.bias_off + 4 * c.q);
    } else {
      load_bias(acc, a.bpack + LL.bias_off, LL.ot, c.q);
      Core::gemm(LL.ktp, acc, in, LL.ot, (const wvec*)a.wpack + LL.wf_off, lds, NoHooks());
    }
    if (c.valid && c.pt < a.n_feat) {
      float* f = a.feat + (size_t)c.pt * (16 * plan.feat_tiles) + 4 * c.q;
#pragma unroll
      for (int t = 0; t < MT; ++t)
        if (t < plan.feat_tiles) *(v4f*)(f + 16 * t) = acc[t];
    }
    float sv = 0.f;
#pragma unroll
    for (int t = 0; t < MT; ++t)
      if (t == plan.feat_tiles) sv = acc[t].x;
    sdf = __shfl(sv, lane_id() & 15, 64);
  } else {
    sdf = sdf_row_dot(in, plan, a.bpack, c.q);
  }

#pragma unroll
  for (int t = 0; t < MT; ++t)
    acc[t] = (t < LL.kt) ? *(const v4f*)(a.bpack + plan.wsdf_off + 16 * t + 4 * c.q) : V4ZERO;
  float n0 = 0.f, n1 = 0.f, n2 = 0.f;
  v4f r_aux[2] = {V4ZERO, V4ZERO};
  auto take_input_grad = [&](const int base) {
    v4f r[5];
#pragma unroll
    for (int t = 0; t < 5; ++t) r[t] = V4ZERO;
    gather_tiles(r, acc, base, in0_tiles);
    float m0, m1, m2;
    pe_jacobian_transpose(r, c.x0, c.x1, c.x2, plan.n_freqs, m0, m1, m2);
    n0 += m0; n1 += m1; n2 += m2;
    r_aux[0] += r[3];
    r_aux[1] += r[4];
  };
  auto row = [&](const msdf_layer_t& L) { return (size_t)L.hpre * Pp + (size_t)c.pt * (16 * L.ot) + 4 * c.q; };
  if (nl >= 2) {
    const msdf_layer_t L = plan.layer[nl - 2];
    const float* Hl = a.H + row(L);
    float* Pl = a.PM + row(L);
    const int otl = L.ot - 1;
    v4f hh[MT];
#pragma unroll
    for (int t = 0; t < MT; ++t) hh[t] = *(const v4f*)(Hl + 16 * (t < otl ? t : otl));
#pragma unroll
    for (int t = 0; t < MT; ++t) {
      if (t == 0 || t < L.ot) {
#pragma unroll
        for (int r = 0; r < 4; ++r) acc[t][r] = (1.0f - one_minus_sigmoid_from_h(hh[t][r])) * acc[t][r];
        if (a.save) *(v4f*)(Pl + 16 * t) = acc[t];
      }
    }
  }
  for (int l = nl - 2; l >= 0; --l) {
    const msdf_layer_t L = plan.layer[l];
#pragma unroll
    for (int t = 0; t < MT; ++t) in[t] = (t < L.ot) ? acc[t] : V4ZERO;
    zero_tiles(acc);
    const msdf_layer_t Lp = plan.layer[l > 0 ? l - 1 : 0];
    Core::gemm(L.otp, acc, in, L.kt, (const wvec*)a.wpack + L.wb_off, lds,
               GradSweepHooks(a.H + row(Lp), a.PM + row(Lp), l > 0 ? Lp.ot : 0, a.save != 0));
    if (l == 0) take_input_grad(0);
    else if (L.skip_tile >= 0) take_input_grad(L.skip_tile);
  }
  if (Core::AUX_LEVEL_MAJOR && a.dy_dx != nullptr && plan.aux_tiles > 0) {
    float m0, m1, m2;
    aux_jacobian_transpose(a.dy_dx, av, plan.aux_tiles, r_aux, c.ptc, c.q, m0, m1, m2);
    n0 = __fadd_rn(n0, __fmul_rn(sum_over_quarters(m0), a.aux_dx_scale));
    n1 = __fadd_rn(n1, __fmul_rn(sum_over_quarters(m1), a.aux_dx_scale));
    n2 = __fadd_rn(n2, __fmul_rn(sum_over_quarters(m2), a.aux_dx_scale));
  }
  bool is_clamped = false;
  if (a.clamp_radius > 0.f && c.pt < a.n_clamp) {
    const float nx = sqrtf(c.x0 * c.x0 + c.x1 * c.x1 + c.x2 * c.x2);
    const float sph = a.sphere_scale * (a.clamp_radius - nx);
    if (sph < sdf) {
      is_clamped = true;
      sdf = sph;
      const float inv = -a.sphere_scale / nx;
      n0 = c.x0 * inv; n1 = c.x1 * inv; n2 = c.x2 * inv;
    }
  }
  if (c.valid) {
    if (c.q == 0) {
      a.sdf[c.pt] = sdf;
      a.nrm[(size_t)c.pt * 3 + 0] = n0;
      a.nrm[(size_t)c.pt * 3 + 1] = n1;
      a.nrm[(size_t)c.pt * 3 + 2] = n2;
      a.clamped[c.pt] = is_clamped ? 1 : 0;
    }
    if (a.r_aux != nullptr) {
#pragma unroll
      for (int t = 0; t < 2; ++t)
        if (t < plan.aux_tiles) {
          v4f v = r_aux[t];
          if (is_clamped) v = V4ZERO;
          aux_store_tile<Core::AUX_LEVEL_MAJOR>(a.r_aux, av, plan.aux_tiles, t, c.pt, c.q, v);
        }
    }
  }
}

typedef msdf_bw_args_t BwArgs;

template <bool LM>
__device__ __forceinline__ void load_rbar(v4f (&rbar)[5], const msdf_plan_t& plan, const BwArgs& a,
                                          const PointCtx& c, const bool live, const float gn0, const float gn1,
                                          const float gn2) {
  pe_jacobian(rbar, c.x0, c.x1, c.x2, plan.n_freqs, gn0, gn1, gn2);
  rbar[3] = rbar[4] = V4ZERO;
  if (LM && a.dy_dx != nullptr && live) {
    const AuxView av = {a.aux_C, a.aux_LC, a.P};
    const float g0 = __fmul_rn(gn0, a.aux_dx_scale), g1 = __fmul_rn(gn1, a.aux_dx_scale), g2 = __fmul_rn(gn2, a.aux_dx_scale);
#pragma unroll
    for (int t = 0; t < 2; ++t)
      if (t < plan.aux_tiles) rbar[3 + t] = aux_jacobian_tile(a.dy_dx, av, t, c.pt, c.q, g0, g1, g2);
  } else if (a.g_raux != nullptr && live) {
    const AuxView av = {a.aux_C, a.aux_LC, a.P};
#pragma unroll
    for (int t = 0; t < 2; ++t)
      if (t < plan.aux_tiles) rbar[3 + t] = aux_load_tile<LM>(a.g_raux, av, plan.aux_tiles, t, c.pt, c.q);
  }
}

template <class Core>
__device__ __forceinline__ void sdf_backward_body(const msdf_plan_t& plan, const BwArgs& a, void* lds) {
  typedef typename Core::wvec wvec;
  const PointCtx c = load_point<Core>(a.x, a.P);
  const int nl = plan.n_layers;
  const size_t Pp = (size_t)a.P_pad;
  const bool live = c.valid && !(a.clamped != nullptr && a.clamped[c.ptc]);
  float gs = 0.f, gn0 = 0.f, gn1 = 0.f, gn2 = 0.f;
  if (live) {
    const bool first = c.pt < a.n_split;
    const float* gsp = first ? a.g_sdf : a.g_sdf_b;
    const float* gnp = first ? a.g_nrm : a.g_nrm_b;
    const size_t j = first ? (size_t)c.pt : (size_t)(c.pt - a.n_split);
    if (gsp) gs = gsp[j];
    if (gnp) {
      gn0 = gnp[j * 3 + 0];
      gn1 = gnp[j * 3 + 1];
      gn2 = gnp[j * 3 + 2];
    }
  }
  if (c.q == 0) a.GSDF[c.pt] = gs;
  if (Core::AUX_LEVEL_MAJOR && a.gg_out != nullptr && c.valid && c.q == 0) {
    float r0 = 0.f, r1 = 0.f, r2 = 0.f;
    const bool first = c.pt < a.n_split;
    const float* gnp = first ? a.g_nrm : a.g_nrm_b;
    if (gnp != nullptr) {
      const size_t j = first ? (size_t)c.pt : (size_t)(c.pt - a.n_split);
      r0 = gnp[j * 3 + 0]; r1 = gnp[j * 3 + 1]; r2 = gnp[j * 3 + 2];
    }
    a.gg_out[(size_t)c.pt * 3 + 0] = __fmul_rn(r0, a.aux_dx_scale);
    a.gg_out[(size_t)c.pt * 3 + 1] = __fmul_rn(r1, a.aux_dx_scale);
    a.gg_out[(size_t)c.pt * 3 + 2] = __fmul_rn(r2, a.aux_dx_scale);
  }
  const int in0_tiles = plan.e_tiles + plan.aux_tiles;

  v4f in[MT], acc[MT];
  {
    v4f rbar[5];
    load_rbar<Core::AUX_LEVEL_MAJOR>(rbar, plan, a, c, live, gn0, gn1, gn2);
    place_tiles(in, 0, rbar, in0_tiles);
  }

  for (int l = 0; l < nl - 1; ++l) {
    const msdf_layer_t L = plan.layer[l];
    if (L.skip_tile >= 0) {
      v4f rbar[5];
      load_rbar<Core::AUX_LEVEL_MAJOR>(rbar, plan, a, c, live, gn0, gn1, gn2);
      place_tiles(in, L.skip_tile, rbar, in0_tiles);
    }
    float* Ql = a.QB + (size_t)L.qpre * Pp + (size_t)c.pt * (16 * L.kt) + 4 * c.q;
#pragma unroll
    for (int t = 0; t < MT; ++t)
      if (t < L.kt) *(v4f*)(Ql + 16 * t) = in[t];
    zero_tiles(acc);
    const size_t off = (size_t)L.hpre * Pp + (size_t)c.pt * (16 * L.ot) + 4 * c.q;
    Core::gemm(L.ktp, acc, in, L.ot, (const wvec*)a.wpack + L.wf_off, lds, SweepUpHooks(a.H + off, L.ot));
#pragma unroll
    for (int t = 0; t < MT; ++t) in[t] = (t < L.ot) ? acc[t] : V4ZERO;
  }
  const msdf_layer_t LL = plan.layer[nl - 1];
  {
    float* Ql = a.QLAST + (size_t)c.pt * (16 * LL.kt) + 4 * c.q;
#pragma unroll
    for (int t = 0; t < MT; ++t)
      if (t < LL.kt) *(v4f*)(Ql + 16 * t) = in[t];
  }

  const bool has_feat = (a.g_feat != nullptr) && c.valid && c.pt < a.n_feat;
  {
    float* ABl = a.AB + (size_t)LL.abpre * Pp + (size_t)c.pt * (16 * LL.ot) + 4 * c.q;
    const float* gf = a.g_feat + (size_t)(has_feat ? c.pt : 0) * (16 * plan.feat_tiles) + 4 * c.q;
    const int ftl = plan.feat_tiles - 1;
#pragma unroll
    for (int t = 0; t < MT; ++t) {
      v4f v = V4ZERO;
      if (a.g_feat != nullptr && ftl >= 0) v = *(const v4f*)(gf + 16 * (t < ftl ? t : ftl));
      if (!has_feat || t >= plan.feat_tiles) v = V4ZERO;
      if (t == plan.feat_tiles && c.q == 0) v.x = gs;
      in[t] = v;
    }
#pragma unroll
    for (int t = 0; t < MT; ++t)
      if (t < LL.ot) *(v4f*)(ABl + 16 * t) = in[t];
  }
  zero_tiles(acc);
  auto down_hooks = [&](const int l) {
    const msdf_layer_t Ln = plan.layer[l >= 0 ? l : 0];
    const size_t off = (size_t)Ln.hpre * Pp + (size_t)c.pt * (16 * Ln.ot) + 4 * c.q;
    const int ln = (l >= 0 ? l : 0) + 1;
    const msdf_layer_t Lq = plan.layer[ln];
    const float* Q = (ln == nl - 1) ? a.QLAST + (size_t)c.pt * (16 * Lq.kt) + 4 * c.q
                                    : a.QB + (size_t)Lq.qpre * Pp + (size_t)c.pt * (16 * Lq.kt) + 4 * c.q;
    return SweepDownHooks(a.H + off, a.PM + off, Q,
                          a.AB + (size_t)Ln.abpre * Pp + (size_t)c.pt * (16 * Ln.ot) + 4 * c.q, l >= 0 ? Ln.ot : 0);
  };
  Core::gemm(LL.otp, acc, in, LL.kt, (const wvec*)a.wpack + LL.wb_off, lds, down_hooks(nl - 2));
  v4f g_in_aux[5];
#pragma unroll
  for (int t = 0; t < 5; ++t) g_in_aux[t] = V4ZERO;
  for (int l = nl - 2; l >= 0; --l) {
    const msdf_layer_t L = plan.layer[l];
#pragma unroll
    for (int t = 0; t < MT; ++t) in[t] = (t < L.ot) ? acc[t] : V4ZERO;
    if (l == 0 && a.g_aux == nullptr) break;
    zero_tiles(acc);
    Core::gemm(L.otp, acc, in, L.kt, (const wvec*)a.wpack + L.wb_off, lds, down_hooks(l - 1));
    if (a.g_aux != nullptr) {
      if (l == 0) gather_tiles(g_in_aux, acc, plan.e_tiles, plan.aux_tiles);
      else if (L.skip_tile >= 0) gather_tiles(g_in_aux, acc, L.skip_tile + plan.e_tiles, plan.aux_tiles);
    }
  }
  if (a.g_aux != nullptr && c.valid) {
    const AuxView av = {a.aux_C, a.aux_LC, a.P};
#pragma unroll
    for (int t = 0; t < 2; ++t)
      if (t < plan.aux_tiles) aux_store_tile<Core::AUX_LEVEL_MAJOR>(a.g_aux, av, plan.aux_tiles, t, c.pt, c.q, g_in_aux[t]);
  }
}
```

### monosdf_amd/csrc/sdf_mlp.hip

```cpp
#include "mlp_launch.h"

__global__ void __launch_bounds__(256) msdf_pack_kernel(const msdf_plan_t plan,
                                                        const msdf_packrule_t* __restrict__ rules,
                                                        const int* __restrict__ maps,
                                                        const float* __restrict__ flat_w,
                                                        const float* __restrict__ flat_b,
                                                        v4f* __restrict__ wpack, float* __restrict__ bpack) {
  const int l = blockIdx.y;
  const int which = blockIdx.z;
  const msdf_layer_t L = plan.layer[l];
  const msdf_packrule_t R = rules[l];
  const int* rowmap = maps + R.rowmap_off;
  const int* colmap = maps + R.colmap_off;
  const float* W = flat_w + R.w_off;
  const int stride = gridDim.x * blockDim.x;
  const int t0 = blockIdx.x * blockDim.x + threadIdx.x;
  if (which < 2) {
    const int n_rt = which == 0 ? L.ot : L.kt;
    const int n_kt = which == 0 ? L.kt : L.ot;
    const int ktp = which == 0 ? L.ktp : L.otp;
    const int off = which == 0 ? L.wf_off : L.wb_off;
    const int total = ((n_rt + 1) & ~1) * ktp * 64;
    for (int i = t0; i < total; i += stride) {
      const int lane = i & 63;
      const int blk = i >> 6;
      const int kt = blk % ktp, rt = blk / ktp;
      const int rslot = 16 * rt + (lane & 15);
      v4f v;
#pragma unroll
      for (int r = 0; r < 4; ++r) {
        const int kslot = 16 * kt + 4 * (lane >> 4) + r;
        float w = 0.f;
        if (rt < n_rt && kt < n_kt) {
          const int row = which == 0 ? rowmap[rslot] : rowmap[kslot];
          const int col = which == 0 ? colmap[kslot] : colmap[rslot];
          if (row >= 0 && col >= 0) w = R.scale * W[(size_t)row * R.cols + col];
        }
        v[r] = w;
      }
      wpack[off + i] = v;
    }
  } else {
    pack_bias_rows(plan, l, R, rowmap, colmap, W, flat_b, bpack, t0, stride);
  }
}

__global__ void __launch_bounds__(CoreF32::THREADS, CoreF32::WGS_PER_CU)
msdf_sdf_forward_k(const msdf_plan_t plan, const v4f* __restrict__ wpack, const float* __restrict__ bpack,
                   const float* __restrict__ x, const float* __restrict__ aux, const AuxView av, const int P,
                   const float clamp_radius, const float sphere_scale, float* __restrict__ sdf_out,
                   const uint32_t* __restrict__ run_flag) {
  extern __shared__ v4f lds[];
  if (run_flag != nullptr && *run_flag == 0u) return;
  sdf_forward_body<CoreF32>(plan, wpack, bpack, x, aux, av, P, clamp_radius, sphere_scale, sdf_out, lds);
}

__global__ void __launch_bounds__(CoreF32::THREADS, CoreF32::WGS_PER_CU)
msdf_sdf_fwd_grad_k(const msdf_plan_t plan, const FgArgs a) {
  extern __shared__ v4f lds[];
  sdf_fwd_grad_body<CoreF32>(plan, a, lds);
}

__global__ void __launch_bounds__(CoreF32::THREADS, CoreF32::WGS_PER_CU)
msdf_sdf_backward_k(const msdf_plan_t plan, const BwArgs a) {
  extern __shared__ v4f lds[];
  sdf_backward_body<CoreF32>(plan, a, lds);
}

static auto pack_kernel(CoreF32) { return msdf_pack_kernel; }
static auto forward_kernel(CoreF32) { return msdf_sdf_forward_k; }
static auto fwd_grad_kernel(CoreF32) { return msdf_sdf_fwd_grad_k; }
static auto backward_kernel(CoreF32) { return msdf_sdf_backward_k; }
template <int NS> static auto pack_kernel(CoreB16N<NS>) { return msdf_pack_b16_kernel<NS>; }
template <int NS> static auto forward_kernel(CoreB16N<NS>) { return msdf_sdf_forward_b16_k<NS>; }
template <int NS> static auto fwd_grad_kernel(CoreB16N<NS>) { return msdf_sdf_fwd_grad_b16_k<NS>; }
template <int NS> static auto backward_kernel(CoreB16N<NS>) { return msdf_sdf_backward_b16_k<NS>; }

extern "C" int msdf_abi_version(void) { return MSDF_ABI_VERSION; }

extern "C" int msdf_pack_weights(const msdf_plan_t* plan, const msdf_packrule_t* rules_dev, const int* maps_dev,
                                 const float* flat_w, const float* flat_b, void* wpack, float* bpack,
                                 void* stream) {
  if (plan == nullptr || plan->n_layers < 1 || plan->n_layers > MSDF_MAX_LAYERS) return MSDF_ERR_ARG;
  return mlp_with_core(plan, [&](auto core) {
    typedef typename decltype(core)::wvec wvec;
    const dim3 grid(32, plan->n_layers, 3);
    pack_kernel(core)<<<grid, 256, 0, (hipStream_t)stream>>>(*plan, rules_dev, maps_dev, flat_w, flat_b, (wvec*)wpack,
                                                             bpack);
    return msdf_check_launch();
  });
}

static bool aux_layout_ok(const msdf_plan_t* plan, const int aux_C, const int aux_LC) {
  if (aux_C == 0) return true;
  return aux_C == 2 && aux_LC > 0 && (aux_LC % aux_C) == 0 &&
         aux_LC <= 16 * plan->aux_tiles;
}

static bool padded_ok(const int P, const int P_pad) { return P_pad >= P && (P_pad % CoreF32::PTS_PER_WG) == 0; }

extern "C" int msdf_sdf_forward_lm(const msdf_plan_t* plan, const void* wpack, const float* bpack, const float* x,
                                   const float* aux, int aux_C, int aux_LC, int P, float clamp_radius,
                                   float sphere_scale, float* sdf, const uint32_t* run_flag, void* stream) {
  if (plan == nullptr || P < 0) return MSDF_ERR_ARG;
  if (P == 0) return MSDF_OK;
  if (plan->aux_tiles > 0 && aux == nullptr) return MSDF_ERR_ARG;
  if (!aux_layout_ok(plan, aux_C, aux_LC)) return MSDF_ERR_ARG;
  return mlp_with_core(plan, [&](auto core) {
    typedef decltype(core) Core;
    if (!Core::AUX_LEVEL_MAJOR && aux_C != 0) return MSDF_ERR_UNSUPPORTED;
    const AuxView av = {aux_C, aux_LC, P};
    return mlp_launch<Core>(forward_kernel(core), (P + Core::PTS_PER_WG - 1) / Core::PTS_PER_WG, stream, *plan,
                            (const typename Core::wvec*)wpack, bpack, x, aux, av, P, clamp_radius, sphere_scale, sdf,
                            run_flag);
  });
}

extern "C" int msdf_sdf_forward_if(const msdf_plan_t* plan, const void* wpack, const float* bpack, const float* x,
                                   const float* aux, int P, float clamp_radius, float sphere_scale, float* sdf,
                                   const uint32_t* run_flag, void* stream) {
  return msdf_sdf_forward_lm(plan, wpack, bpack, x, aux, 0, 0, P, clamp_radius, sphere_scale, sdf, run_flag, stream);
}

extern "C" int msdf_sdf_forward(const msdf_plan_t* plan, const void* wpack, const float* bpack, const float* x,
                                const float* aux, int P, float clamp_radius, float sphere_scale, float* sdf,
                                void* stream) {
  return msdf_sdf_forward_if(plan, wpack, bpack, x, aux, P, clamp_radius, sphere_scale, sdf, nullptr, stream);
}

extern "C" int msdf_sdf_fwd_grad(const msdf_plan_t* plan, const msdf_fg_args_t* a, void* stream) {
  if (plan == nullptr || a == nullptr || a->P < 0) return MSDF_ERR_ARG;
  if (a->P == 0) return MSDF_OK;
  if (!padded_ok(a->P, a->P_pad)) return MSDF_ERR_ARG;
  if (plan->aux_tiles > 0 && a->aux == nullptr) return MSDF_ERR_ARG;
  if (!aux_layout_ok(plan, a->aux_C, a->aux_LC)) return MSDF_ERR_ARG;
  if (a->dy_dx != nullptr && (a->aux_C != 2 || a->r_aux == nullptr)) return MSDF_ERR_ARG;
  return mlp_with_core(plan, [&](auto core) {
    typedef decltype(core) Core;
    if (!Core::AUX_LEVEL_MAJOR && (a->aux_C != 0 || a->dy_dx != nullptr)) return MSDF_ERR_UNSUPPORTED;
    return mlp_launch<Core>(fwd_grad_kernel(core), a->P_pad / Core::PTS_PER_WG, stream, *plan, *a);
  });
}

extern "C" int msdf_sdf_backward(const msdf_plan_t* plan, const msdf_bw_args_t* a, void* stream) {
  if (plan == nullptr || a == nullptr || a->P < 0) return MSDF_ERR_ARG;
  if (a->P == 0) return MSDF_OK;
  if (!padded_ok(a->P, a->P_pad)) return MSDF_ERR_ARG;
  if (!aux_layout_ok(plan, a->aux_C, a->aux_LC)) return MSDF_ERR_ARG;
  if (a->dy_dx != nullptr && a->aux_C != 2) return MSDF_ERR_ARG;
  return mlp_with_core(plan, [&](auto core) {
    typedef decltype(core) Core;
    if (!Core::AUX_LEVEL_MAJOR && (a->aux_C != 0 || a->dy_dx != nullptr)) return MSDF_ERR_UNSUPPORTED;
    return mlp_launch<Core>(backward_kernel(core), a->P_pad / Core::PTS_PER_WG, stream, *plan, *a);
  });
}
```

### monosdf_amd/model/network.py

```python
import math

import os

import numpy as np
import torch
import torch.nn as nn

from .. import ops, plan as planlib
from ..hashencoder.hashgrid import HashEncoder
from .density import LaplaceDensity
from .ray_sampler import ErrorBoundSampler


class WNLinear(nn.Module):

    def __init__(self, in_dim, out_dim, init_fn=None, weight_norm=True):
        super().__init__()
        lin = nn.Linear(in_dim, out_dim)
        if init_fn is not None:
            init_fn(lin)
        self.in_features, self.out_features = in_dim, out_dim
        self.has_weight_norm = weight_norm
        self.bias = nn.Parameter(lin.bias.data.clone())
        if weight_norm:
            w = lin.weight.data
            self.weight_g = nn.Parameter(torch.norm_except_dim(w, 2, 0).clone())
            self.weight_v = nn.Parameter(w.clone())
        else:
            self.weight = nn.Parameter(lin.weight.data.clone())

    def effective_weight(self):
        if self.has_weight_norm:
            return torch._weight_norm(self.weight_v, self.weight_g, 0)
        return self.weight


class _FusedNet(nn.Module):

    def _layers(self):
        return [getattr(self, 'lin%d' % l) for l in range(self.num_layers - 1)]

    precision = None
    supports_bf16x3 = False

    def set_precision(self, precision):
        if precision not in ops.PRECISIONS:
            raise ValueError('precision must be one of %s' % (ops.PRECISIONS,))
        if precision != 'fp32' and not self.supports_bf16x3:
            precision = 'fp32'
        object.__setattr__(self, 'precision', precision)
        object.__setattr__(self, '_fused_state', None)

    def _fused(self, device):
        f = getattr(self, '_fused_state', None)
        if f is None or f.device != device:
            prec = self.precision or os.environ.get('MONOSDF_PRECISION', 'fp32')
            if not self.supports_bf16x3:
                prec = 'fp32'
            f = ops.FusedMlp(self._build_plan(), device, prec)
            object.__setattr__(self, '_fused_state', f)
        return f

    def packed(self, device):
        shared = getattr(self, '_shared', None)
        if shared is not None:
            return shared
        fused = self._fused(device)
        wn = getattr(self, '_wn_state', None)
        if wn is None:
            wn = ops.WeightNormState()
            object.__setattr__(self, '_wn_state', wn)
        flat_w, flat_b = ops.fused_weight_norm(wn, self._layers())
        wpack, bpack = fused.pack(flat_w, flat_b)
        return fused, flat_w, flat_b, wpack, bpack

    def share(self, device):
        object.__setattr__(self, '_shared', None)
        object.__setattr__(self, '_shared', self.packed(device))

    def unshare(self):
        object.__setattr__(self, '_shared', None)


def _geometric_init(l, num_layers, dims, skip_in, multires, bias, inside_outside, out_dim):
    def fn(lin):
        if l == num_layers - 2:
            if not inside_outside:
                torch.nn.init.normal_(lin.weight, mean=np.sqrt(np.pi) / np.sqrt(dims[l]), std=0.0001)
                torch.nn.init.constant_(lin.bias, -bias)
            else:
                torch.nn.init.normal_(lin.weight, mean=-np.sqrt(np.pi) / np.sqrt(dims[l]), std=0.0001)
                torch.nn.init.constant_(lin.bias, bias)
        elif multires > 0 and l == 0:
            torch.nn.init.constant_(lin.bias, 0.0)
            torch.nn.init.constant_(lin.weight[:, 3:], 0.0)
            torch.nn.init.normal_(lin.weight[:, :3], 0.0, np.sqrt(2) / np.sqrt(out_dim))
        elif multires > 0 and l in skip_in:
            torch.nn.init.constant_(lin.bias, 0.0)
            torch.nn.init.normal_(lin.weight, 0.0, np.sqrt(2) / np.sqrt(out_dim))
            torch.nn.init.constant_(lin.weight[:, -(dims[0] - 3):], 0.0)
        else:
            torch.nn.init.constant_(lin.bias, 0.0)
            torch.nn.init.normal_(lin.weight, 0.0, np.sqrt(2) / np.sqrt(out_dim))
    return fn


class _SdfBase(_FusedNet):

    supports_bf16x3 = True

    def _make_layers(self, dims, geometric_init, bias, skip_in, weight_norm, multires, inside_outside):
        self.num_layers = len(dims)
        self.skip_in = tuple(skip_in)
        self.dims = list(dims)
        for l in range(self.num_layers - 1):
            out_dim = dims[l + 1] - dims[0] if (l + 1) in self.skip_in else dims[l + 1]
            init = _geometric_init(l, self.num_layers, dims, self.skip_in, multires, bias, inside_outside,
                                   out_dim) if geometric_init else None
            setattr(self, 'lin%d' % l, WNLinear(dims[l], out_dim, init, weight_norm))

    def _build_plan(self):
        shapes = [(l.out_features, l.in_features) for l in self._layers()]
        return planlib.build_sdf_plan(shapes, self.skip_in, self.multires, self.aux_cols, self.aux_active,
                                      self.feature_vector_size)

    def evaluate(self, x, n_clamp, n_feat, save=None, split=None):
        if save is None:
            save = torch.is_grad_enabled()
        x = x.detach()
        fused, flat_w, flat_b, wpack, bpack = self.packed(x.device)
        ns = x.shape[0] if split is None else int(split)
        if self.aux_active and ops.HASH_SCATTER == 'binned' and self.encoding.level_dim > 1:
            enc = self.encoding
            sdf, _, feat, nrm, nrm_b = ops.GridSdfFunction.apply(
                x, enc.embeddings, enc.offsets, flat_w, flat_b, wpack, bpack, fused, enc.kernel_dims, int(n_clamp),
                int(n_feat), self.sphere_scale, bool(save), ns, float(self.divide_factor))
            feat = self._trim_features(feat)
            return (sdf, feat, nrm) if split is None else (sdf, feat, nrm, nrm_b)
        aux, handle = None, None
        if self.aux_active:
            aux, handle = self.encoding.encode_with_jacobian((x / self.divide_factor + 1.0) / 2.0)
            aux = self._pad_aux(aux)
        radius = self.sdf_bounding_sphere if self.clamps else 0.0
        sdf, _, feat, nrm, nrm_b, r_aux = ops.SdfMlpFunction.apply(
            x, aux, flat_w, flat_b, wpack, bpack, fused, int(n_clamp), int(n_feat), radius, self.sphere_scale,
            bool(save), ns)
        if self.aux_active:
            r_aux = r_aux[:, :self.aux_cols]
            through_grid = self.encoding.input_gradient(handle, r_aux) * (0.5 / self.divide_factor)
            nrm = nrm + through_grid[:ns]
            nrm_b = nrm_b + through_grid[ns:]
        feat = self._trim_features(feat)
        if split is None:
            return sdf, feat, nrm
        return sdf, feat, nrm, nrm_b

    def _trim_features(self, feat):
        F = self.feature_vector_size
        return feat if feat.shape[1] == F else feat[:, :F]

    def _pad_aux(self, aux):
        pad = (-aux.shape[1]) % 16
        if pad:
            aux = torch.nn.functional.pad(aux, (0, pad))
        return aux.contiguous()

    def gradient_sdf(self, x):
        return self.evaluate(x, 0, 0)[2]

    def get_outputs(self, x):
        P = x.shape[0]
        return self.evaluate(x, P, P)

    def raw_sdf(self, x):
        with torch.no_grad():
            return self._sdf_only(x, clamp=False)[:, 0]

    def _sdf_only(self, x, run_flag=None, clamp=True):
        fused, _, _, wpack, bpack = self.packed(x.device)
        aux, aux_lm = None, None
        if self.aux_active:
            enc = self.encoding
            if x.shape[-1] == 3 and x.dim() == 2:
                aux, aux_lm = ops.hash_node_features(
                    x, self.divide_factor, enc.embeddings, enc.offsets, enc.kernel_dims, 16 * fused.plan.aux_tiles,
                    level_major=(fused.precision == 'fp32'))
            else:
                with torch.no_grad():
                    aux = self._pad_aux(enc((x / self.divide_factor).detach(), calc_grad_inputs=False))
        radius = self.sdf_bounding_sphere if (self.clamps and clamp) else 0.0
        return ops.sdf_forward_nograd(fused, wpack, bpack, x.detach(), aux, radius, self.sphere_scale, run_flag, aux_lm)


class ImplicitNetwork(_SdfBase):
    def __init__(self, feature_vector_size, sdf_bounding_sphere, d_in, d_out, dims, geometric_init=True,
                 bias=1.0, skip_in=(), weight_norm=True, multires=0, sphere_scale=1.0, inside_outside=False):
        super().__init__()
        self.sdf_bounding_sphere = sdf_bounding_sphere
        self.sphere_scale = sphere_scale
        self.feature_vector_size = feature_vector_size
        self.multires = multires
        self.aux_cols, self.aux_active, self.clamps = 0, False, True
        dims = [d_in] + list(dims) + [d_out + feature_vector_size]
        if multires > 0:
            dims[0] = d_in + 2 * d_in * multires
        self._make_layers(dims, geometric_init, bias, skip_in, weight_norm, multires, inside_outside)

    def forward(self, x):
        P = x.shape[0]
        sdf, feat, _ = self.evaluate(x, 0, P)
        return torch.cat([sdf, feat], 1)

    def get_sdf_vals(self, x):
        if torch.is_grad_enabled() and any(p.requires_grad for p in self.parameters()):
            P = x.shape[0]
            return self.evaluate(x, P, 0)[0]
        return self._sdf_only(x)


class ImplicitNetworkGrid(_SdfBase):
    def __init__(self, feature_vector_size, sdf_bounding_sphere, d_in, d_out, dims, geometric_init=True,
                 bias=1.0, skip_in=(), weight_norm=True, multires=0, sphere_scale=1.0, inside_outside=False,
                 base_size=16, end_size=2048, logmap=19, num_levels=16, level_dim=2, divide_factor=1.5,
                 use_grid_feature=True, debug=False):
        super().__init__()
        self.sdf_bounding_sphere = sdf_bounding_sphere
        self.sphere_scale = sphere_scale
        self.feature_vector_size = feature_vector_size
        self.multires = multires
        self.divide_factor = divide_factor
        self.grid_feature_dim = num_levels * level_dim
        self.use_grid_feature = use_grid_feature
        self.aux_cols, self.aux_active, self.clamps = self.grid_feature_dim, bool(use_grid_feature), False
        dims = [d_in] + list(dims) + [d_out + feature_vector_size]
        dims[0] += self.grid_feature_dim
        self.encoding = HashEncoder(input_dim=3, num_levels=num_levels, level_dim=level_dim, per_level_scale=2,
                                    base_resolution=base_size, log2_hashmap_size=logmap,
                                    desired_resolution=end_size)
        if multires > 0:
            dims[0] += 2 * d_in * multires
        self._make_layers(dims, geometric_init, bias, skip_in, weight_norm, multires, inside_outside)

    def forward(self, x):
        P = x.shape[0]
        sdf, feat, _ = self.evaluate(x, 0, P)
        return {'sdf': sdf, 'feature': feat}

    def get_sdf_vals(self, x):
        if torch.is_grad_enabled() and any(p.requires_grad for p in self.parameters()):
            return self.evaluate(x, 0, 0)[0]
        return self._sdf_only(x)

    def mlp_parameters(self):
        params = []
        for l in self._layers():
            params += list(l.parameters())
        return params

    def grid_parameters(self):
        return self.encoding.parameters()


class RenderingNetwork(_FusedNet):
    supports_bf16x3 = True

    def __init__(self, feature_vector_size, mode, d_in, d_out, dims, weight_norm=True, multires_view=0,
                 per_image_code=False, if_hdr=False, spec=False, debug=False):
        super().__init__()
        if spec:
            raise NotImplementedError('monosdf_amd: the diffuse/specular split (spec=True) is outside the hot path')
        if mode not in ('idr', 'nerf'):
            raise NotImplementedError(mode)
        self.mode = mode
        self.spec = False
        self.feature_vector_size = feature_vector_size
        self.multires_view = multires_view
        dims = [d_in + feature_vector_size] + list(dims) + [d_out]
        if multires_view > 0:
            dims[0] += 6 * multires_view
        self.per_image_code = per_image_code
        if per_image_code:
            self.embeddings = nn.Parameter(torch.empty(1024, 32))
            self.embeddings.data.uniform_(-1e-4, 1e-4)
            dims[0] += 32
        self.num_layers = len(dims)
        self.if_hdr = if_hdr
        for l in range(self.num_layers - 1):
            setattr(self, 'lin%d' % l, WNLinear(dims[l], dims[l + 1], None, weight_norm))

    def _build_plan(self):
        shapes = [(l.out_features, l.in_features) for l in self._layers()]
        return planlib.build_color_plan(shapes, self.mode, self.multires_view, self.feature_vector_size,
                                        32 if self.per_image_code else 0, self.if_hdr)

    def forward(self, points, normals, view_dirs, feature_vectors, indices, if_pixel_input=False,
                samples_per_ray=None):
        P = points.shape[0]
        if samples_per_ray is None:
            samples_per_ray, dirs = 1, view_dirs
        else:
            dirs = view_dirs
        code = None
        if self.per_image_code:
            n_rays = P // samples_per_ray
            if not if_pixel_input:
                code = self.embeddings[indices].expand(n_rays, -1)
            else:
                code = self.embeddings[indices]
                if code.shape[0] != n_rays:
                    code = code.unsqueeze(1).expand(-1, n_rays // code.shape[0], -1).flatten(0, 1)
            code = code.contiguous()
        fused, flat_w, flat_b, wpack, bpack = self.packed(points.device)
        rgb = ops.ColorMlpFunction.apply(points, dirs, normals, feature_vectors, code, flat_w, flat_b, wpack, bpack,
                                         fused, int(samples_per_ray), torch.is_grad_enabled())
        return {'rgb': rgb}


class MonoSDFNetwork(nn.Module):
    def __init__(self, conf, if_hdr=False):
        super().__init__()
        self.feature_vector_size = conf.get_int('feature_vector_size')
        self.scene_bounding_sphere = conf.get_float('scene_bounding_sphere', default=1.0)
        self.white_bkgd = conf.get_bool('white_bkgd', default=False)
        self.register_buffer('bg_color', torch.tensor(conf.get_list('bg_color', default=[1.0, 1.0, 1.0])).float(),
                             persistent=False)
        self.if_hdr = if_hdr
        Grid_MLP = conf.get_bool('Grid_MLP', default=False)
        self.Grid_MLP = Grid_MLP
        sphere = 0.0 if self.white_bkgd else self.scene_bounding_sphere
        cls = ImplicitNetworkGrid if Grid_MLP else ImplicitNetwork
        self.implicit_network = cls(self.feature_vector_size, sphere, **conf.get_config('implicit_network'))
        self.rendering_network = RenderingNetwork(self.feature_vector_size, **conf.get_config('rendering_network'),
                                                  if_hdr=self.if_hdr)
        self.spec = False
        self.density = LaplaceDensity(**conf.get_config('density'))
        self.ray_sampler = ErrorBoundSampler(self.scene_bounding_sphere, **conf.get_config('ray_sampler'))
        self._noise = None
        env = os.environ.get('MSDF_SPECULATE_ROUNDS', '1')
        self.speculate_rounds = False if env == '0' else ('all' if env == 'all' else True)

    def set_precision(self, precision):
        self.implicit_network.set_precision(precision)
        self.rendering_network.set_precision(precision)
        return self

    def _bg_list(self):
        bg = getattr(self, '_bg_cache', None)
        if bg is None:
            bg = [float(v) for v in self.bg_color.tolist()]
            object.__setattr__(self, '_bg_cache', bg)
        return bg

    def _rays(self, input_dict, if_pixel_input):
        if not if_pixel_input:
            uv, pose, intrinsics = input_dict['uv'], input_dict['pose'], input_dict['intrinsics']
            if uv.shape[0] != 1:
                raise NotImplementedError('image mode renders one image (one pose) per call, as the runner does')
            ray_dirs, ray_dirs_tmp, cam_loc = ops.camera_rays(uv[0], pose[0], intrinsics[0])
            ray_dirs, ray_dirs_tmp = ray_dirs.unsqueeze(0), ray_dirs_tmp.unsqueeze(0)
        else:
            ray_dirs = input_dict['ray_dirs'].unsqueeze(0)
            cam_loc = input_dict['ray_cam_loc']
            ray_dirs_tmp = input_dict['ray_dirs_tmp'].unsqueeze(0)
        return ray_dirs, cam_loc, ray_dirs_tmp

    def forward(self, input_dict, indices, if_pixel_input=False):
        ray_dirs, cam_loc, ray_dirs_tmp = self._rays(input_dict, if_pixel_input)
        depth_scale = ray_dirs_tmp[0, :, 2:]
        batch_size, num_pixels, _ = ray_dirs.shape
        ray_dirs = ray_dirs.reshape(-1, 3).contiguous()
        cam_loc = cam_loc.contiguous()
        device = ray_dirs.device
        noise = self._noise or {}
        net = self.implicit_network
        beta = ops.effective_beta(self.density.beta, self.density.beta_min_f)
        net.share(device)
        self.rendering_network.share(device)
        try:
            pose = input_dict['ray_pose'] if if_pixel_input else input_dict['pose'][:1]
            K = self.ray_sampler.max_total_iters
            mode = self.speculate_rounds
            guess = 0 if not mode else (K if mode == 'all' else min(K, self.ray_sampler.guess_rounds()))
            for attempt in (guess, K if guess else 0):
                z_vals, z_samples_eik, x_all = self.ray_sampler.sample(ray_dirs, cam_loc, self, speculate=attempt,
                                                                      beta0=beta)
                N, S = z_vals.shape
                P = N * S
                points_flat = x_all[:P]
                sdf, feature_vectors, gradients_sdf, grad_eik = net.evaluate(x_all, P, P, save=torch.is_grad_enabled(),
                                                                                split=P)
                rgb_flat = self.rendering_network(points_flat, gradients_sdf, ray_dirs, feature_vectors, indices,
                                                  if_pixel_input=if_pixel_input, samples_per_ray=S)['rgb']
                rgb = rgb_flat.reshape(-1, S, 3)
                weights, rgb_values, depth_values, normal_map, depth_vals = ops.CompositeFunction.apply(
                    z_vals, sdf, rgb_flat, gradients_sdf, beta, depth_scale, self.white_bkgd,
                    self._bg_list(), pose, self.density.beta, True)
                if attempt == 0 or attempt == K or self.ray_sampler.confirm():
                    break
        finally:
            net.unshare()
            self.rendering_network.unshare()

        output = {
            'rgb': rgb,
            'rgb_values': rgb_values,
            'depth_values': depth_values,
            'z_vals': z_vals,
            'depth_vals': depth_vals,
            'sdf': sdf.reshape(z_vals.shape),
            'weights': weights,
        }
        if self.training:
            output['grad_theta'], output['grad_theta_nei'] = ops.SplitRowsFunction.apply(grad_eik,
                                                                                          grad_eik.shape[0] // 2)
        output['normal_map'] = normal_map
        return output

    def volume_rendering(self, z_vals, sdf):
        N, S = z_vals.shape
        zeros = torch.zeros(N * S, 3, device=z_vals.device)
        ones = torch.ones(N, device=z_vals.device)
        return ops.CompositeFunction.apply(z_vals, sdf, zeros, zeros, self.density.get_beta(), ones, False,
                                           [0.0, 0.0, 0.0])[0]
```

### monosdf_amd/model/ray_sampler.py

```python
import ctypes as C

import torch

from .. import _lib


class RaySampler:
    def __init__(self, near, far):
        self.near, self.far = near, far


def _need_gpu(t):
    if not t.is_cuda:
        raise RuntimeError('monosdf_amd: the samplers run on the GPU only (no CPU fallback)')
    return t.detach().float().contiguous()


class UniformSampler(RaySampler):

    def __init__(self, scene_bounding_sphere, near, N_samples, take_sphere_intersection=False, far=-1):
        super().__init__(near, 2.0 * scene_bounding_sphere * 1.75 if far == -1 else far)
        self.N_samples = N_samples
        self.scene_bounding_sphere = scene_bounding_sphere
        self.take_sphere_intersection = take_sphere_intersection

    def get_z_vals(self, ray_dirs, cam_loc, model, jitter=None):
        ray_dirs, cam_loc = _need_gpu(ray_dirs), _need_gpu(cam_loc)
        dev = ray_dirs.device
        N, n = ray_dirs.shape[0], self.N_samples
        f32 = dict(device=dev, dtype=torch.float32)
        if model.training and jitter is None:
            jitter = torch.rand(N, n, **f32)
        z = torch.empty(N, n, **f32)
        far = torch.empty(N, 1, **f32)
        scratch = torch.empty(N * n * 5 + N, **f32)
        a = _lib.SamplerArgs()
        a.ray_o, a.ray_d, a.N = cam_loc.data_ptr(), ray_dirs.data_ptr(), N
        a.M, a.m_max, a.n_eval, a.n_final, a.n_extra = n, n, n, 0, 0
        a.max_rounds = 1
        a.near, a.far = float(self.near), float(self.far)
        a.bound = float(self.scene_bounding_sphere) if self.take_sphere_intersection else 0.0
        a.lemma = 1.0
        a.z, a.new_z = z.data_ptr(), scratch.data_ptr()
        a.new_pos = scratch.data_ptr() + 4 * N * n
        a.pts, a.beta = scratch.data_ptr() + 8 * N * n, scratch.data_ptr() + 20 * N * n
        a.jitter = _need_gpu(jitter).data_ptr() if jitter is not None else None
        a.far_out = far.data_ptr()
        _lib.call('msdf_sampler_init', C.byref(a), _lib.stream_ptr())
        self._keep = (jitter, scratch)
        return z, torch.full((N, 1), float(self.near), **f32), far


class ErrorBoundSampler(RaySampler):
    def __init__(self, scene_bounding_sphere, near, N_samples, N_samples_eval, N_samples_extra, eps, beta_iters,
                 max_total_iters, inverse_sphere_bg=False, N_samples_inverse_sphere=0, add_tiny=1.0e-6):
        super().__init__(near, 2.0 * scene_bounding_sphere * 1.75)
        if inverse_sphere_bg:
            raise NotImplementedError('monosdf_amd: inverse_sphere_bg is not used by any conf of the reference fork')
        self.N_samples = N_samples
        self.N_samples_eval = N_samples_eval
        self.uniform_sampler = UniformSampler(scene_bounding_sphere, near, N_samples_eval,
                                              take_sphere_intersection=True)
        self.N_samples_extra = N_samples_extra
        self.eps = eps
        self.beta_iters = beta_iters
        self.max_total_iters = max_total_iters
        self.scene_bounding_sphere = scene_bounding_sphere
        self.add_tiny = add_tiny
        self._last_rounds = 0
        self._hist = [[], []]
        self._miss = [0, 0]
        self._pending = None
        self._eval_columns = {}
        self.stats = {'calls': 0, 'repeats': 0, 'idle_rounds': 0}
        self.global_rounds = None
        self._lemma = float(1.0 / (4.0 * torch.log(torch.tensor(self.eps + 1.0))))

    def get_z_vals(self, ray_dirs, cam_loc, model):
        z, z_eik, _ = self.sample(ray_dirs, cam_loc, model, want_points=False)
        return z, z_eik

    def get_error_bound(self, beta, model, sdf, z_vals, dists, d_star):
        z = _need_gpu(z_vals)
        N, M = z.shape
        sdf = _need_gpu(sdf).reshape(N, M)
        d_star = _need_gpu(d_star).reshape(N, M - 1)
        beta = _need_gpu(beta if torch.is_tensor(beta) else torch.tensor(beta, device=z.device)).reshape(-1)
        if beta.numel() not in (1, N):
            raise RuntimeError('monosdf_amd: beta must hold one value or one per ray')
        out = torch.empty(N, device=z.device, dtype=torch.float32)
        _lib.call('msdf_sampler_error_bound', _lib.ptr(z), _lib.ptr(sdf), _lib.ptr(d_star), _lib.ptr(beta),
                  int(beta.numel() == N and N > 1), N, M, _lib.ptr(out), _lib.stream_ptr())
        return out

    def _extra_columns(self, training, noise, dev):
        n_extra, n_eval, K = self.N_samples_extra, self.N_samples_eval, self.max_total_iters
        if n_extra <= 0:
            return torch.zeros(K, 1, device=dev, dtype=torch.int64)
        if training:
            given = noise.get('extra_idx')
            if given is not None:
                given = given.to(device=dev, dtype=torch.int64)
                if given.dim() == 2:
                    return given.contiguous()
                return given.reshape(1, n_extra).expand(K, n_extra).contiguous()
            host = torch.empty(K, n_extra, dtype=torch.int64, pin_memory=True)
            for k in range(K):
                host[k] = torch.randperm(n_eval * (k + 1))[:n_extra]
            return host.to(dev, non_blocking=True)
        key = (str(dev), n_eval, K, n_extra)
        if key not in self._eval_columns:
            rows = [torch.linspace(0, n_eval * (k + 1) - 1, n_extra).long() for k in range(K)]
            self._eval_columns[key] = torch.stack(rows).to(dev)
        return self._eval_columns[key]

    @property
    def last_rounds(self):
        self._resolve()
        return self._last_rounds

    @last_rounds.setter
    def last_rounds(self, value):
        self._resolve()
        self._last_rounds = int(value)

    def _resolve(self):
        if self._pending is None:
            return True
        ev, host, k, which = self._pending
        self._pending = None
        ev.synchronize()
        ran = 1
        while ran <= k and int(host[2 * (ran - 1) + 1]):
            ran += 1
        if ran > k:
            self.stats['repeats'] += 1
            self._note_rounds(k + 1, which)
            self._miss[which] = self.HISTORY
            return False
        self.stats['idle_rounds'] += k - ran
        self._note_rounds(ran, which)
        return True

    def confirm(self):
        if self._pending is None or self._pending[2] >= self.max_total_iters:
            return True
        return self._resolve()

    HISTORY = 32

    def _note_rounds(self, rounds, which=0):
        self._last_rounds = rounds
        self._hist[which] = (self._hist[which] + [rounds])[-self.HISTORY:]

    def guess_rounds(self):
        which = 1 if self.global_rounds is not None else 0
        if self._miss[which] > 0:
            self._miss[which] -= 1
            return self.max_total_iters
        return max(self._hist[which]) if self._hist[which] else 1

    def sample(self, ray_dirs, cam_loc, model, want_points=True, speculate=0, beta0=None):
        dev = ray_dirs.device
        ray_dirs, cam_loc = _need_gpu(ray_dirs), _need_gpu(cam_loc)
        self._resolve()
        N = ray_dirs.shape[0]
        n_eval, n_final, n_extra = self.N_samples_eval, self.N_samples, self.N_samples_extra
        K = self.max_total_iters
        m_max = n_eval * K
        S = n_final + n_extra + 2
        noise = getattr(model, '_noise', None) or {}
        training = bool(model.training)
        net = model.implicit_network
        beta0 = (model.density.get_beta() if beta0 is None else beta0).detach().float().reshape(1).contiguous()
        f32 = dict(device=dev, dtype=torch.float32)
        z = torch.empty(N, m_max, **f32)
        sdf = torch.empty(N, m_max, **f32)
        new_z = torch.empty(N, n_eval, **f32)
        new_pos = torch.empty(N, n_eval, device=dev, dtype=torch.int32)
        pts = torch.empty(N * n_eval, 3, **f32)
        beta = torch.empty(N, **f32)
        flags = torch.empty(2 * K, device=dev, dtype=torch.int32)
        final_z = torch.empty(N, n_final, **f32)
        jitter = u_final = nei_drawn = eik_u_drawn = eik_unit_drawn = None
        if training:
            need = [k for k in ('jitter', 'final_u', 'nei_rand', 'eik_idx', 'eik_uniform') if noise.get(k) is None]
            sizes = {'jitter': N * n_eval, 'final_u': N * n_final, 'nei_rand': 6 * N if want_points else 0,
                     'eik_idx': N, 'eik_uniform': 3 * N if want_points else 0}
            pool = torch.rand(sum(sizes[k] for k in need), **f32) if need else None
            drawn, off = {}, 0
            for k in need:
                drawn[k] = pool[off:off + sizes[k]]
                off += sizes[k]
            jitter = noise.get('jitter')
            jitter = drawn['jitter'].view(N, n_eval) if jitter is None else jitter.to(**f32).contiguous()
            u_final = noise.get('final_u')
            u_final = drawn['final_u'].view(N, n_final) if u_final is None else u_final.to(**f32).contiguous()
            nei_drawn = drawn.get('nei_rand')
            eik_u_drawn, eik_unit_drawn = drawn.get('eik_idx'), drawn.get('eik_uniform')
        a = _lib.SamplerArgs()
        a.ray_o, a.ray_d, a.N = cam_loc.data_ptr(), ray_dirs.data_ptr(), N
        a.m_max, a.n_eval, a.n_final, a.n_extra = m_max, n_eval, n_final, n_extra
        a.max_rounds, a.training, a.beta_iters = K, int(training), self.beta_iters
        a.near, a.far, a.bound = float(self.near), float(self.far), float(self.scene_bounding_sphere)
        a.eps, a.add_tiny, a.lemma = float(self.eps), float(self.add_tiny), self._lemma
        a.beta0, a.z, a.sdf = beta0.data_ptr(), z.data_ptr(), sdf.data_ptr()
        a.new_z, a.new_pos, a.pts, a.beta = new_z.data_ptr(), new_pos.data_ptr(), pts.data_ptr(), beta.data_ptr()
        a.flags = flags.data_ptr()
        a.jitter = jitter.data_ptr() if jitter is not None else None
        a.u_final = u_final.data_ptr() if u_final is not None else None
        a.final_z = final_z.data_ptr()
        st = _lib.stream_ptr()
        a.M = n_eval
        _lib.call('msdf_sampler_init', C.byref(a), st)
        z_out = z_eik = x_all = extra_idx = eik_idx = None

        def prepare_finish():
            nonlocal z_out, z_eik, x_all, extra_idx, eik_idx
            eik_idx = noise.get('eik_idx')
            a.eik_u, a.eik_unit = None, 0
            if eik_idx is None and eik_u_drawn is not None:
                a.eik_idx, a.eik_u = None, eik_u_drawn.data_ptr()
            else:
                if eik_idx is None:
                    eik_idx = torch.randint(S, (N,), device=dev)
                eik_idx = eik_idx.to(device=dev, dtype=torch.int64).contiguous()
                a.eik_idx = eik_idx.data_ptr()
            z_out = torch.empty(N, S, **f32)
            z_eik = torch.empty(N, 1, **f32)
            a.z_out, a.z_eik, a.pts_out = z_out.data_ptr(), z_eik.data_ptr(), None
            if want_points:
                n_eik = 4 * N if training else 0
                x_all = torch.empty(N * S + n_eik, 3, **f32)
                a.pts_out = x_all.data_ptr()
                if training:
                    R = self.scene_bounding_sphere
                    eik_uniform = noise.get('eik_uniform')
                    if eik_uniform is None and eik_unit_drawn is not None and eik_unit_drawn.numel() == 3 * N:
                        eik_uniform, a.eik_unit = eik_unit_drawn.view(N, 3), 1
                    else:
                        eik_uniform = (torch.empty(N, 3, **f32).uniform_(-R, R) if eik_uniform is None
                                       else eik_uniform.to(**f32).contiguous())
                    nei = noise.get('nei_rand')
                    nei = nei_drawn.view(2 * N, 3) if nei is None else nei.to(**f32).contiguous()
                    a.eik_uniform, a.nei_rand = eik_uniform.data_ptr(), nei.data_ptr()
                    self._keep = (eik_uniform, nei)
            extra_idx = self._extra_columns(training, noise, dev)
            a.extra_idx = extra_idx.data_ptr()

        group = self.global_rounds
        which = 1 if group is not None else 0
        rounds = 0
        with torch.no_grad():
            while True:
                run_flag = flags.data_ptr() + 4 * (2 * rounds - 1) if (speculate > 0 and rounds > 0) else None
                new_sdf = net._sdf_only(pts, run_flag=run_flag)
                a.new_sdf = new_sdf.data_ptr()
                a.M, a.round_idx = n_eval * (rounds + 1), rounds
                _lib.call('msdf_sampler_beta', C.byref(a), st)
                if group is not None:
                    import torch.distributed as dist
                    dist.all_reduce(flags[2 * rounds:2 * rounds + 1], op=dist.ReduceOp.MAX,
                                    group=None if group is True else group)
                _lib.call('msdf_sampler_resample', C.byref(a), st)
                if rounds == 0:
                    prepare_finish()
                rounds += 1
                if speculate > 0:
                    more = rounds < min(speculate, K)
                else:
                    more = bool(flags[2 * rounds - 1].item())
                if not more:
                    break
        self._pending = None
        self.stats['calls'] += 1
        if speculate > 0:
            host = torch.empty(flags.shape, dtype=flags.dtype, pin_memory=True)
            host.copy_(flags, non_blocking=True)
            ev = torch.cuda.Event()
            ev.record()
            self._pending = (ev, host, rounds, which)
        else:
            self._note_rounds(rounds, which)
        _lib.call('msdf_sampler_finish', C.byref(a), st)
        return z_out, z_eik, x_all
```

### monosdf_amd/ops.py

```python
import collections
import ctypes as C

import numpy as np
import torch

from . import _lib, parallel, plan as planlib


def _need_cuda(t, name):
    if not t.is_cuda:
        raise RuntimeError('monosdf_amd: %s must be a GPU tensor (the HIP path has no CPU fallback)' % name)
    if t.dtype != torch.float32:
        raise RuntimeError('monosdf_amd: %s must be float32' % name)
    return t.contiguous()


def _pad64(n):
    return (n + 63) // 64 * 64


def _cont(t):
    return None if t is None else t.contiguous()


# ... 53 lines not shown

    def __init__(self, mlp_plan, device, precision='fp32'):
        if precision not in PRECISIONS:
            raise ValueError('monosdf_amd: precision must be one of %s, got %r' % (PRECISIONS, precision))
        self.mp = mlp_plan
        self.device = device
        self.precision = precision
        self.plan = mlp_plan.plan if precision == 'fp32' else mlp_plan.build_b16(_PLANES[precision])
        self.rules_dev = torch.from_numpy(mlp_plan.rules_np).to(device)
        self.maps_dev = torch.from_numpy(mlp_plan.maps_np).to(device)
        self._wgrad_cache = {}

    def pack(self, flat_w, flat_b):
        mp = self.mp
        flat_w = _need_cuda(flat_w.detach(), 'weights')
        flat_b = _need_cuda(flat_b.detach(), 'biases')
        assert flat_w.numel() == mp.n_w and flat_b.numel() == mp.n_b
        units16 = mp.wpack_f4 if self.precision == 'fp32' else mp.wpack16_units(_PLANES[self.precision])
        wpack = torch.empty(units16 * 4 + 4 * 17 * 64 * 4, device=self.device, dtype=torch.float32)
        bpack = torch.empty(mp.bpack_f + 64, device=self.device, dtype=torch.float32)
        _lib.call('msdf_pack_weights', C.byref(self.plan), _lib.ptr(self.rules_dev), _lib.ptr(self.maps_dev),
                  _lib.ptr(flat_w), _lib.ptr(flat_b), _lib.ptr(wpack), _lib.ptr(bpack), _lib.stream_ptr())
        return wpack, bpack

    def wgrad_program(self, P_pad):
        key = P_pad
        if key not in self._wgrad_cache:
            build = planlib.build_sdf_wgrad if self.mp.kind == 'sdf' else planlib.build_color_wgrad
            program = planlib.uniform_program if self.precision == 'bf16x3' else planlib.balanced_program
            prog = program(build, self.mp, P_pad)
            rules_dev = torch.from_numpy(prog.rules_bytes()).to(self.device)
            wg_map = torch.from_numpy(prog.wg_map()).to(self.device)
            items_dev = torch.from_numpy(prog.items_bytes()).to(self.device)
            full = prog.writes_every_element(self.mp.n_w + self.mp.n_b, self.mp.maps_np)
            self._wgrad_cache[key] = dict(prog=prog, rules=rules_dev, wg_map=wg_map, items=items_dev, full=full)
        return self._wgrad_cache[key]

    def run_wgrad(self, P_pad, base_addr, defer=False):
        ent = self.wgrad_program(P_pad)
        prog = ent['prog']
        items_dev = ent['items']
        bases = [base_addr.get(name) for name in prog.BUFFERS]
        part = torch.empty(prog.part_f + 64, device=self.device, dtype=torch.float32)
        alloc = torch.empty if ent['full'] else torch.zeros
        grad = alloc(self.mp.n_w + self.mp.n_b, device=self.device, dtype=torch.float32)
        wg_map = ent['wg_map']
        held = list(base_addr.values())

        rules_dev = ent['rules']

        def launch(stream=None):
            if stream is not None:
                for t in held + [part, grad, items_dev, wg_map, rules_dev, self.maps_dev]:
                    t.record_stream(stream)
            st = _lib.stream_ptr()
            _lib.call('msdf_wgrad', _lib.ptr(items_dev), _lib.ptr(wg_map), wg_map.numel() // 2,
                      _lib.ptr(part), P_pad, PRECISIONS.index(self.precision), _lib.ptr(bases[0]), _lib.ptr(bases[1]), st)
            _lib.call('msdf_reduce', _lib.ptr(rules_dev), len(prog.rules), _lib.ptr(self.maps_dev),
                      _lib.ptr(part), _lib.ptr(grad), st)

        if defer:
            _DEFERRED.append(launch)
        else:
            launch()
        return grad


class WeightNormTables:

    def __init__(self, shapes, tensors):
        dev = tensors[0].device
        recs, row_layer, w_off, b_off, it = [], [], 0, 0, iter(tensors)
        for i, (rows, cols, has_g) in enumerate(shapes):
            r = _lib.WnLayer()
            v = next(it)
            g = next(it) if has_g else None
            b = next(it)
            r.v, r.g, r.b = v.data_ptr(), _addr(g), b.data_ptr()
            r.rows, r.cols = rows, cols
            r.w_off, r.b_off, r.row_off, r.has_g = w_off, b_off, b_off, int(has_g)
            recs.append(bytes(r))
            row_layer += [i] * rows
            w_off += rows * cols
            b_off += rows
        self.layers_dev = torch.from_numpy(np.frombuffer(b''.join(recs), dtype=np.uint8).copy()).to(dev)
        self.row_layer_dev = torch.tensor(row_layer, dtype=torch.int32, device=dev)
        self.n_w, self.total_rows = w_off, b_off


class WeightNormState:

    def __init__(self):
        self.key, self.cur = None, None

    def tables(self, shapes, tensors):
        key = tuple(t.data_ptr() for t in tensors)
        if key != self.key:
            self.cur = WeightNormTables(shapes, tensors)
            self.key = key
        return self.cur


class FusedWeightNormFunction(torch.autograd.Function):

    @staticmethod
    def forward(ctx, state, shapes, *params):
        st = state.tables(shapes, params)
        dev = params[0].device
        flat_w = torch.empty(st.n_w, device=dev, dtype=torch.float32)
        flat_b = torch.empty(st.total_rows, device=dev, dtype=torch.float32)
        norms = torch.empty(st.total_rows, device=dev, dtype=torch.float32)
        _lib.call('msdf_weightnorm_forward', _lib.ptr(st.layers_dev), _lib.ptr(st.row_layer_dev), st.total_rows,
                  _lib.ptr(flat_w), _lib.ptr(flat_b), _lib.ptr(norms), _lib.stream_ptr())
        ctx.state, ctx.shapes = state, shapes
        ctx.save_for_backward(norms, *params)
        return flat_w, flat_b

    @staticmethod
    @torch.autograd.function.once_differentiable
    def backward(ctx, g_w, g_b):
        norms, *params = ctx.saved_tensors
        shapes = ctx.shapes
        st = ctx.state.tables(shapes, params)
        dev = norms.device
        join_side_work()
        g_w = g_w.contiguous()
        dv = torch.empty(st.n_w, device=dev, dtype=torch.float32)
        dg = torch.empty(st.total_rows, device=dev, dtype=torch.float32)
        _lib.call('msdf_weightnorm_backward', _lib.ptr(st.layers_dev), _lib.ptr(st.row_layer_dev), st.total_rows,
                  _lib.ptr(g_w), _lib.ptr(norms), _lib.ptr(dv), _lib.ptr(dg), _lib.stream_ptr())
        grads, w_off, b_off = [], 0, 0
        for rows, cols, has_g in shapes:
            n = rows * cols
            grads.append(dv[w_off:w_off + n].view(rows, cols))
            if has_g:
                grads.append(dg[b_off:b_off + rows].view(rows, 1))
            grads.append(g_b[b_off:b_off + rows])
            w_off += n
            b_off += rows
        return (None, None) + tuple(grads)


def fused_weight_norm(state, layers):
    params, shapes = [], []
    for l in layers:
        params.append(l.weight_v if l.has_weight_norm else l.weight)
        if l.has_weight_norm:
            params.append(l.weight_g)
        params.append(l.bias)
        shapes.append((l.out_features, l.in_features, bool(l.has_weight_norm)))
    return FusedWeightNormFunction.apply(state, tuple(shapes), *params)


def sdf_forward_nograd(mlp, wpack, bpack, x, aux, clamp_radius, sphere_scale, run_flag=None, aux_lm=None):
    x = _need_cuda(x, 'points')
    P = x.shape[0]
    out = torch.empty(P, 1, device=x.device, dtype=torch.float32)
    aC, aLC = aux_lm if aux_lm is not None else (0, 0)
    _lib.call('msdf_sdf_forward_lm', C.byref(mlp.plan), _lib.ptr(wpack), _lib.ptr(bpack),
              _lib.ptr(x), _lib.ptr(aux), int(aC), int(aLC), P, float(clamp_radius), float(sphere_scale), _lib.ptr(out),
              C.c_void_p(run_flag) if run_flag else None, _lib.stream_ptr())
    return out


_SdfState = collections.namedtuple(
    '_SdfState', 'mlp P P_pad n_feat n_split saved has_aux aux_lm aux_shape jac_scale')


def _sdf_fwd_grad(x, aux, wpack, bpack, mlp, n_clamp, n_feat, clamp_radius, sphere_scale, save, n_split=None,
                  aux_lm=None, aux_jac=None):
    mp = mlp.mp
    plan = mlp.plan
    x = _need_cuda(x.detach(), 'points')
    P = x.shape[0]
    P_pad = _pad64(max(P, 1))
    dev = x.device
    has_aux = plan.aux_tiles > 0
    aux = _need_cuda(aux.detach(), 'aux features') if has_aux else None
    woff, total = planlib.sdf_workspace(mp, P_pad)
    if not save:
        total = woff['PM']
    ws = torch.empty(max(total, 64), device=dev, dtype=torch.float32)
    F = 16 * plan.feat_tiles
    sdf = torch.empty(P, 1, device=dev, dtype=torch.float32)
    feat_full = torch.empty(_pad64(max(n_feat, 1)), F, device=dev, dtype=torch.float32)
    feat_full[n_feat:].zero_()
    feat = feat_full[:n_feat]
    nrm = torch.empty(P, 3, device=dev, dtype=torch.float32)
    aC, aLC = aux_lm if (aux_lm is not None and has_aux) else (0, 0)
    aux_shape = (aLC // aC, P, aC) if aC else (P, 16 * plan.aux_tiles)
    r_aux = torch.empty(*aux_shape, device=dev, dtype=torch.float32) if has_aux else None
    clamped = torch.empty(max(P, 1), device=dev, dtype=torch.uint8)
    a = _lib.FgArgs()
    a.wpack, a.bpack, a.x, a.aux = wpack.data_ptr(), bpack.data_ptr(), x.data_ptr(), _addr(aux)
    a.P, a.P_pad, a.n_clamp, a.n_feat = P, P_pad, n_clamp, n_feat
    a.clamp_radius, a.sphere_scale = float(clamp_radius), float(sphere_scale)
    a.sdf, a.feat, a.nrm, a.r_aux, a.clamped = sdf.data_ptr(), feat.data_ptr(), nrm.data_ptr(), _addr(r_aux), \
        clamped.data_ptr()
    base = ws.data_ptr()
    a.H = base + 4 * woff['H']
    a.PM = base + 4 * woff['PM'] if save else None
    a.IN0 = base + 4 * woff['IN0'] if save else None
    a.save = 1 if save else 0
    a.aux_C, a.aux_LC = int(aC), int(aLC)
    jac_scale = None
    if aux_jac is not None and aC == 2:
        jac_scale = float(aux_jac[1])
        a.dy_dx, a.aux_dx_scale = aux_jac[0].data_ptr(), jac_scale
    if P > 0:
        _lib.call('msdf_sdf_fwd_grad', C.byref(plan), C.byref(a), _lib.stream_ptr())
    ns = P if n_split is None else int(n_split)
    state = _SdfState(mlp, P, P_pad, n_feat, ns, save, has_aux, (int(aC), int(aLC)), aux_shape, jac_scale)
    return (sdf[:ns], sdf[ns:], feat, nrm[:ns], nrm[ns:], r_aux), (x, ws, clamped, wpack, bpack), state


def _sdf_backward(state, saved, grads, dy_dx=None, gg_out=None, after_sweeps=None):
    if not state.saved:
        raise RuntimeError('monosdf_amd: backward through an inference-mode SDF evaluation')
    x, ws, clamped, wpack, bpack = saved
    mlp, P, P_pad = state.mlp, state.P, state.P_pad
    mp = mlp.mp
    dev = x.device
    woff, _ = planlib.sdf_workspace(mp, P_pad)
    g_sdf, g_sdf_b, g_feat, g_nrm, g_nrm_b, g_raux = [_cont(g) for g in grads]
    g_aux = torch.empty(*state.aux_shape, device=dev, dtype=torch.float32) if state.has_aux else None
    b = _lib.BwArgs()
    b.aux_C, b.aux_LC = state.aux_lm
    if state.jac_scale is not None:
        b.dy_dx, b.aux_dx_scale, b.gg_out = dy_dx.data_ptr(), state.jac_scale, _addr(gg_out)
    b.wpack, b.bpack, b.x = wpack.data_ptr(), bpack.data_ptr(), x.data_ptr()
    b.P, b.P_pad, b.n_feat, b.n_split = P, P_pad, state.n_feat, state.n_split
    b.g_sdf, b.g_sdf_b, b.g_nrm, b.g_nrm_b = _addr(g_sdf), _addr(g_sdf_b), _addr(g_nrm), _addr(g_nrm_b)
    b.g_feat = _addr(g_feat) if state.n_feat > 0 else None
    b.g_raux = _addr(g_raux) if state.has_aux else None
    b.clamped = clamped.data_ptr()
    base = ws.data_ptr()
    for k in ('H', 'PM', 'QB', 'AB', 'GSDF', 'QLAST'):
        setattr(b, k, base + 4 * woff[k])
    b.g_aux = _addr(g_aux)
    if P > 0:
        _lib.call('msdf_sdf_backward', C.byref(mlp.plan), C.byref(b), _lib.stream_ptr())
        start_side_work(dev)
    if after_sweeps is not None:
        after_sweeps(g_aux)
    grad = mlp.run_wgrad(P_pad, {'ws': ws}) if P > 0 else torch.zeros(mp.n_w + mp.n_b, device=dev)
    return g_aux, grad


class SdfMlpFunction(torch.autograd.Function):

    @staticmethod
    def forward(ctx, x, aux, flat_w, flat_b, wpack, bpack, mlp, n_clamp, n_feat, clamp_radius,
                sphere_scale, save, n_split=None):
        ctx.set_materialize_grads(False)
        outs, saved, ctx.state = _sdf_fwd_grad(x, aux, wpack, bpack, mlp, n_clamp, n_feat, clamp_radius,
                                               sphere_scale, save, n_split)
        ctx.save_for_backward(*saved)
        return outs

    @staticmethod
    @torch.autograd.function.once_differentiable
    def backward(ctx, *grads):
        g_aux, grad = _sdf_backward(ctx.state, ctx.saved_tensors, grads)
        n_w = ctx.state.mlp.mp.n_w
        return (None, g_aux, grad[:n_w], grad[n_w:]) + (None,) * 9


def _encode_points(x, divide_factor, embeddings, offsets, enc, pitch, level_major, jacobian):
    x = _need_cuda(x.detach(), 'points')
    emb = _need_cuda(embeddings.detach(), 'embeddings')
    L, Cdim, S, H = enc
    B, D = x.shape
    dev = x.device
    x01 = torch.empty(B, D, device=dev, dtype=torch.float32) if jacobian else None
    outputs = torch.empty(L, B, Cdim, device=dev, dtype=torch.float32)
    dy_dx = torch.empty(B, L * D * Cdim, device=dev, dtype=torch.float32) if jacobian else None
    st = _lib.stream_ptr()
    _lib.call('msdf_hash_node_forward', _lib.ptr(x), float(divide_factor), _lib.ptr(x01), _lib.ptr(emb),
              _lib.ptr(offsets), _lib.ptr(outputs), 0, B, Cdim, L, S, H, _lib.ptr(dy_dx), st)
    if Cdim == 2 and level_major:
        return x, outputs, (Cdim, L * Cdim), x01, dy_dx
    aux = torch.empty(B, pitch, device=dev, dtype=torch.float32)
    _lib.call('msdf_hash_transpose', _lib.ptr(outputs), _lib.ptr(aux), None, None, L, B, Cdim, pitch, 1, st)
    return x, aux, None, x01, dy_dx


class GridSdfFunction(torch.autograd.Function):

    @staticmethod
    def forward(ctx, x, embeddings, offsets, flat_w, flat_b, wpack, bpack, mlp, enc, n_clamp, n_feat, sphere_scale,
                save, n_split, divide_factor):
        ctx.set_materialize_grads(False)
        L, Cdim, S, H = enc
        A = 16 * mlp.plan.aux_tiles
        x, aux, lm, x01, dy_dx = _encode_points(x, divide_factor, embeddings, offsets, enc, A,
                                                mlp.precision == 'fp32', True)
        B = x.shape[0]
        k = 0.5 / divide_factor
        jac = (dy_dx, k) if (lm is not None and FUSE_JACOBIAN) else None
        (sdf_a, sdf_b, feat, nrm_a, nrm_b, r_aux), saved, ctx.state = _sdf_fwd_grad(
            x, aux, wpack, bpack, mlp, n_clamp, n_feat, 0.0, sphere_scale, save, n_split, lm, jac)
        if jac is None:
            assert nrm_a.data_ptr() + 12 * nrm_a.shape[0] == nrm_b.data_ptr() or nrm_b.shape[0] == 0
            _lib.call('msdf_hash_node_input_gradient', _lib.ptr(r_aux), 0 if lm is not None else A, _lib.ptr(dy_dx), B,
                      Cdim, L, float(k), _lib.ptr(nrm_a), _lib.stream_ptr())
        ctx.enc, ctx.k, ctx.n_entries, ctx.lm, ctx.offsets = enc, k, embeddings.shape[0], lm, offsets
        ctx.save_for_backward(x01, dy_dx, r_aux, *saved)
        return sdf_a, sdf_b, feat, nrm_a, nrm_b

    @staticmethod
    @torch.autograd.function.once_differentiable
    def backward(ctx, g_sdf, g_sdf_b, g_feat, g_nrm, g_nrm_b):
        x01, dy_dx, r_aux, *saved = ctx.saved_tensors
        state, (L, Cdim, S, H), k, lm = ctx.state, ctx.enc, ctx.k, ctx.lm
        B, D = x01.shape
        dev = x01.device
        st = _lib.stream_ptr()
        A = 16 * state.mlp.plan.aux_tiles
        gg = torch.empty(B, D, device=dev, dtype=torch.float32)
        if state.jac_scale is not None:
            g_raux = None
        else:
            g_raux = torch.empty(*((L, B, Cdim) if lm is not None else (B, A)), device=dev, dtype=torch.float32)
            _lib.call('msdf_hash_node_second_grad', _lib.ptr(_cont(g_nrm)), _lib.ptr(_cont(g_nrm_b)), state.n_split,
                      float(k), _lib.ptr(gg), _lib.ptr(dy_dx), _lib.ptr(g_raux), 0 if lm is not None else A, B, Cdim,
                      L, st)
        done = []

        def scatter(g_aux):
            g_emb = torch.empty(ctx.n_entries, Cdim, device=dev, dtype=torch.float32)
            ws, nbytes = _hash_workspace(B, Cdim, L, g_emb)
            if lm is not None:
                g_lm = (g_aux, r_aux)
            else:
                g_lm = torch.empty(2, L, B, Cdim, device=dev, dtype=torch.float32)
                _lib.call('msdf_hash_transpose', _lib.ptr(g_aux), _lib.ptr(g_lm[0]), _lib.ptr(r_aux), _lib.ptr(g_lm[1]),
                          L, B, Cdim, A, 0, st)
            _lib.call('msdf_hash_node_scatter', _lib.ptr(g_lm[0]), _lib.ptr(g_lm[1]), 0, _lib.ptr(x01),
                      _lib.ptr(ctx.offsets), _lib.ptr(g_emb), B, Cdim, L, S, H, _lib.ptr(gg), ctx.n_entries,
                      _lib.ptr(ws), nbytes, st)
            parallel.mark_grad_ready(g_emb)
            done.append(g_emb)

        _, grad = _sdf_backward(state, saved, (g_sdf, g_sdf_b, g_feat, g_nrm, g_nrm_b, g_raux), dy_dx=dy_dx, gg_out=gg,
                                after_sweeps=scatter)
        n_w = state.mlp.mp.n_w
        return (None, done.pop(), None, grad[:n_w], grad[n_w:]) + (None,) * 10


def hash_node_features(x, divide_factor, embeddings, offsets, enc, pitch, level_major=True):
    _, aux, aux_lm, _, _ = _encode_points(x, divide_factor, embeddings, offsets, enc, pitch, level_major, False)
    return aux, aux_lm


class ColorMlpFunction(torch.autograd.Function):

    @staticmethod
    def forward(ctx, x, dirs, nrm, feat, code, flat_w, flat_b, wpack, bpack, cmlp, spr, save):
        mp = cmlp.mp
        plan = cmlp.plan
        x = _need_cuda(x.detach(), 'points')
        dirs = _need_cuda(dirs.detach(), 'view dirs')
        nrm = _need_cuda(nrm.detach(), 'normals')
        feat = feat.detach()
        P = x.shape[0]
        P_pad = _pad64(max(P, 1))
        dev = x.device
        Fk = 16 * plan.layer[0].kt
        ctx.feat_cols = feat.shape[1]
        if feat.shape[1] > Fk or Fk - feat.shape[1] >= 16:
            raise RuntimeError('monosdf_amd: feature width %d does not fit the colour network plan (%d slots)'
                               % (feat.shape[1], Fk))
        if feat.shape[1] < Fk:
            if feat.is_cuda and feat.dim() == 2 and feat.stride() == (Fk, 1) and \
                    feat.untyped_storage().nbytes() // 4 - feat.storage_offset() >= P * Fk:
                feat = feat.as_strided((P, Fk), (Fk, 1))
            else:
                feat = torch.nn.functional.pad(feat, (0, Fk - feat.shape[1]))
        feat = _need_cuda(feat, 'features')
        room = feat.untyped_storage().nbytes() // 4 - feat.storage_offset()
        if room < P_pad * feat.shape[1]:
            padded = torch.zeros(P_pad, feat.shape[1], device=dev, dtype=torch.float32)
            padded[:P] = feat
            feat = padded[:P]
        has_code = plan.aux_tiles > 0
        if has_code:
            code = _need_cuda(code.detach(), 'image code')
        woff, total = planlib.color_workspace(mp, P_pad)
        ws = torch.empty(max(total if save else 64, 64), device=dev, dtype=torch.float32)
        rgb = torch.empty(P, 3, device=dev, dtype=torch.float32)
        a = _lib.ColorFwdArgs()
        a.wpack, a.bpack = wpack.data_ptr(), bpack.data_ptr()
        a.x, a.dirs, a.nrm, a.feat = x.data_ptr(), dirs.data_ptr(), nrm.data_ptr(), feat.data_ptr()
        a.code = _addr(code) if has_code else None
        a.P, a.P_pad, a.spr, a.save = P, P_pad, int(spr), 1 if save else 0
        a.rgb = rgb.data_ptr()
        base = ws.data_ptr()
        a.H = base + 4 * woff['H'] if save else None
        a.MISC = base + 4 * woff['MISC'] if save else None
        if P > 0:
            _lib.call('msdf_color_forward', C.byref(plan), C.byref(a), _lib.stream_ptr())
        ctx.cmlp, ctx.P, ctx.P_pad, ctx.saved, ctx.has_code, ctx.spr = cmlp, P, P_pad, save, has_code, spr
        ctx.save_for_backward(rgb, feat, ws, wpack, bpack)
        return rgb

    @staticmethod
    @torch.autograd.function.once_differentiable
    def backward(ctx, g_rgb):
        if not ctx.saved:
            raise RuntimeError('monosdf_amd: backward through an inference-mode colour evaluation')
        rgb, feat, ws, wpack, bpack = ctx.saved_tensors
        cmlp, P, P_pad = ctx.cmlp, ctx.P, ctx.P_pad
        mp = cmlp.mp
        plan = cmlp.plan
        dev = rgb.device
        woff, _ = planlib.color_workspace(mp, P_pad)
        g_rgb = g_rgb.contiguous()
        g_feat = torch.empty_like(feat)
# ... 391 lines not shown
```

Measured before the change: 119,300 rays/s.

## Reuse sampler's first-round SDF hidden activations in the training forward pass

During the first sampler round, the no-grad SDF evaluation now saves the softplus hidden activations for points that also appear in the final sample set into a staging buffer. A row map built by the sampler links final sorted sample rows to these saved rows. The training fwd_grad kernel then skips recomputing the forward layers for those points, loading the staged activations and copying them into the workspace during the backward sweep. This cuts redundant MLP forward work at the cost of extra stores in the sampler pass, indirection through a row map, and extra API and state complexity. It also adds NaN-to-inf handling in the sort.

```diff
diff --git a/include/monosdf_hip.h b/include/monosdf_hip.h
--- a/include/monosdf_hip.h
+++ b/include/monosdf_hip.h
@@ -89,6 +89,10 @@
 int msdf_sdf_forward_lm(const msdf_plan_t* plan, const void* wpack, const float* bpack, const float* x,
                         const float* aux, int aux_C, int aux_LC, int P, float clamp_radius, float sphere_scale,
                         float* sdf, const uint32_t* run_flag, void* stream);
+int msdf_sdf_forward_save(const msdf_plan_t* plan, const void* wpack, const float* bpack, const float* x,
+                          const float* aux, int aux_C, int aux_LC, int P, float clamp_radius, float sphere_scale,
+                          float* sdf, const uint32_t* run_flag, float* H, int P_pad, const int32_t* col_slot,
+                          int n_cols, int n_slots, uint32_t* h_saved, void* stream);
 
 typedef struct {
   const void* wpack;
@@ -112,6 +116,12 @@
   int32_t aux_LC;
   float aux_dx_scale;
   const float* dy_dx;
+  const int32_t* row_map;
+  const uint32_t* smp_flags;
+  const uint32_t* h_saved;
+  int32_t n_reuse;
+  int32_t stage_pad;
+  const float* h_stage;
 } msdf_fg_args_t;
 int msdf_sdf_fwd_grad(const msdf_plan_t* plan, const msdf_fg_args_t* args, void* stream);
 
@@ -142,6 +152,7 @@
   float* gg_out;
   float aux_dx_scale;
   int32_t pad_;
+  const int32_t* row_map;
 } msdf_bw_args_t;
 int msdf_sdf_backward(const msdf_plan_t* plan, const msdf_bw_args_t* args, void* stream);
 
@@ -307,6 +318,8 @@
   const float* eik_u;
   int32_t eik_unit;
   int32_t pad_;
+  int32_t* row_map;
+  uint32_t* h_saved;
 } msdf_sampler_args_t;
 int msdf_sampler_init(const msdf_sampler_args_t* args, void* stream);
 int msdf_sampler_beta(const msdf_sampler_args_t* args, void* stream);
diff --git a/monosdf_amd/_lib.py b/monosdf_amd/_lib.py
--- a/monosdf_amd/_lib.py
+++ b/monosdf_amd/_lib.py
@@ -49,7 +49,8 @@
                 ('clamp_radius', C.c_float), ('sphere_scale', C.c_float),
                 ('sdf', _P), ('feat', _P), ('nrm', _P), ('r_aux', _P), ('clamped', _P),
                 ('H', _P), ('PM', _P), ('IN0', _P), ('save', C.c_int32), ('aux_C', C.c_int32), ('aux_LC', C.c_int32),
-                ('aux_dx_scale', C.c_float), ('dy_dx', _P)]
+                ('aux_dx_scale', C.c_float), ('dy_dx', _P),
+                ('row_map', _P), ('smp_flags', _P), ('h_saved', _P), ('n_reuse', C.c_int32), ('stage_pad', C.c_int32), ('h_stage', _P)]
 
 
 class BwArgs(C.Structure):
@@ -58,7 +59,8 @@
                 ('g_sdf', _P), ('g_feat', _P), ('g_nrm', _P), ('g_raux', _P), ('clamped', _P),
                 ('H', _P), ('PM', _P), ('QB', _P), ('T', _P), ('AB', _P), ('GSDF', _P), ('QLAST', _P),
                 ('g_aux', _P), ('g_sdf_b', _P), ('g_nrm_b', _P), ('aux_C', C.c_int32), ('aux_LC', C.c_int32),
-                ('dy_dx', _P), ('gg_out', _P), ('aux_dx_scale', C.c_float), ('pad_', C.c_int32)]
+                ('dy_dx', _P), ('gg_out', _P), ('aux_dx_scale', C.c_float), ('pad_', C.c_int32),
+                ('row_map', _P)]
 
 
 class ColorFwdArgs(C.Structure):
@@ -122,7 +124,7 @@
                 ('extra_idx', _P), ('eik_idx', _P), ('z_out', _P), ('z_eik', _P), ('pts_out', _P),
                 ('eik_uniform', _P), ('nei_rand', _P), ('far_out', _P), ('rounds_out', _P),
                 ('dbg_dstar', _P), ('dbg_err0', _P), ('dbg_cdf', _P), ('eik_u', _P), ('eik_unit', C.c_int32),
-                ('pad_', C.c_int32)]
+                ('pad_', C.c_int32), ('row_map', _P), ('h_saved', _P)]
 
 
 _ERR = {1: 'invalid argument', 2: 'kernel launch failed', 3: 'unsupported configuration'}
@@ -159,6 +161,8 @@
     'msdf_sdf_forward': [C.POINTER(Plan), _P, _P, _P, _P, C.c_int, C.c_float, C.c_float, _P, _P],
     'msdf_sdf_forward_if': [C.POINTER(Plan), _P, _P, _P, _P, C.c_int, C.c_float, C.c_float, _P, _P, _P],
     'msdf_sdf_forward_lm': [C.POINTER(Plan), _P, _P, _P, _P, C.c_int, C.c_int, C.c_int, C.c_float, C.c_float, _P, _P, _P],
+    'msdf_sdf_forward_save': [C.POINTER(Plan), _P, _P, _P, _P, C.c_int, C.c_int, C.c_int, C.c_float, C.c_float, _P, _P,
+                              _P, C.c_int, _P, C.c_int, C.c_int, _P, _P],
     'msdf_sdf_fwd_grad': [C.POINTER(Plan), C.POINTER(FgArgs), _P],
     'msdf_sdf_backward': [C.POINTER(Plan), C.POINTER(BwArgs), _P],
     'msdf_color_forward': [C.POINTER(Plan), C.POINTER(ColorFwdArgs), _P],
diff --git a/monosdf_amd/csrc/mlp_core.h b/monosdf_amd/csrc/mlp_core.h
--- a/monosdf_amd/csrc/mlp_core.h
+++ b/monosdf_amd/csrc/mlp_core.h
@@ -293,6 +293,7 @@
 #define MLP_F32_AUX_LEVEL_MAJOR true
 #endif
   static constexpr bool AUX_LEVEL_MAJOR = MLP_F32_AUX_LEVEL_MAJOR;
+  static constexpr bool ROW_MAP = true;
   static __device__ __forceinline__ float softplus(const float a) {
     float h, s;
     softplus100(a, h, s);
diff --git a/monosdf_amd/csrc/mlp_core_b16.h b/monosdf_amd/csrc/mlp_core_b16.h
--- a/monosdf_amd/csrc/mlp_core_b16.h
+++ b/monosdf_amd/csrc/mlp_core_b16.h
@@ -213,6 +213,7 @@
   static constexpr int LDS_BYTES = 2 * B16Cfg<NS>::BUF_V8 * 16;
   static constexpr bool BIAS_IN_HOOKS = (NS == 3);
   static constexpr bool AUX_LEVEL_MAJOR = false;
+  static constexpr bool ROW_MAP = false;
   static __device__ __forceinline__ float softplus(const float a) {
     if constexpr (NS == 2) return softplus100_lean(a);
     float h, s;
diff --git a/monosdf_amd/csrc/sampler.hip b/monosdf_amd/csrc/sampler.hip
--- a/monosdf_amd/csrc/sampler.hip
+++ b/monosdf_amd/csrc/sampler.hip
@@ -39,6 +39,7 @@
   const int lane = lane_id();
   if (ray == 0 && a.flags != nullptr)
     for (int i = lane; i < 2 * a.max_rounds; i += 64) a.flags[i] = 0u;
+  if (ray == 0 && lane == 0 && a.h_saved != nullptr) a.h_saved[0] = 0u;
   const int n = a.n_eval;
   const float o0 = a.ray_o[ray * 3 + 0], o1 = a.ray_o[ray * 3 + 1], o2 = a.ray_o[ray * 3 + 2];
   const float d0 = a.ray_d[ray * 3 + 0], d1 = a.ray_d[ray * 3 + 1], d2 = a.ray_d[ray * 3 + 2];
@@ -316,6 +317,7 @@
     else if (j == a.n_final) x = a.near;
     else if (j == a.n_final + 1) x = a.far;
     else x = zrow[min((int)extra[j - a.n_final - 2], rounds * a.n_eval - 1)];
+    if (x != x) x = INFINITY;
     v[j] = x;
   }
   smp_sync();
@@ -323,10 +325,19 @@
   const float d0 = a.ray_d[ray * 3 + 0], d1 = a.ray_d[ray * 3 + 1], d2 = a.ray_d[ray * 3 + 2];
   for (int j = lane; j < S; j += 64) {
     const float x = v[j];
-    int r = 0;
-    for (int k = 0; k < S; ++k) r += (v[k] < x || (v[k] == x && k < j)) ? 1 : 0;
+    int r = 0, rn = 0;
+    for (int k = 0; k < S; ++k) {
+      const int before = (v[k] < x || (v[k] == x && k < j)) ? 1 : 0;
+      r += before;
+      rn += (k < a.n_final + 2) ? before : 0;
+    }
     sorted[r] = x;
     a.z_out[(size_t)ray * S + r] = x;
+    if (a.row_map != nullptr) {
+      const int e = j - a.n_final - 2;
+      const int er = (e >= 0) ? ray * a.n_extra + e : a.N * a.n_extra + ray * (S - a.n_extra) + rn;
+      a.row_map[er] = ray * S + r;
+    }
     if (a.pts_out != nullptr) {
       float* p = a.pts_out + ((size_t)ray * S + r) * 3;
       p[0] = o0 + x * d0; p[1] = o1 + x * d1; p[2] = o2 + x * d2;
@@ -340,6 +351,8 @@
     if (a.z_eik != nullptr) a.z_eik[ray] = ze;
     if (a.pts_out != nullptr && a.eik_uniform != nullptr) {
       float* e = a.pts_out + (size_t)a.N * S * 3;
+      if (a.row_map != nullptr)
+        for (int i = 0; i < 4; ++i) a.row_map[a.N * S + i * a.N + ray] = a.N * S + i * a.N + ray;
       const float od[3] = {o0 + ze * d0, o1 + ze * d1, o2 + ze * d2};
 #pragma unroll
       for (int c = 0; c < 3; ++c) {
diff --git a/monosdf_amd/csrc/sdf_kernels.h b/monosdf_amd/csrc/sdf_kernels.h
--- a/monosdf_amd/csrc/sdf_kernels.h
+++ b/monosdf_amd/csrc/sdf_kernels.h
@@ -10,13 +10,25 @@
 };
 
 template <class Core>
-__device__ __forceinline__ PointCtx load_point(const float* __restrict__ x, const int P) {
+__device__ __forceinline__ int eval_row() {
+  return blockIdx.x * Core::PTS_PER_WG + (threadIdx.x >> 6) * MLP_PTS_PER_WAVE + (lane_id() & 15);
+}
+
+template <class Core>
+__device__ __forceinline__ PointCtx load_point(const float* __restrict__ x, const int P,
+                                               const int32_t* __restrict__ row_map = nullptr) {
   PointCtx c;
   const int lane = lane_id();
-  const int wave = threadIdx.x >> 6;
-  c.pt = blockIdx.x * Core::PTS_PER_WG + wave * MLP_PTS_PER_WAVE + (lane & 15);
-  c.valid = c.pt < P;
-  c.ptc = c.valid ? c.pt : (P - 1);
+  const int pe = eval_row<Core>();
+  c.valid = pe < P;
+  c.ptc = c.valid ? pe : (P - 1);
+  if constexpr (Core::ROW_MAP) {
+    if (row_map != nullptr) {
+      const int m = row_map[c.ptc];
+      if ((unsigned)m < (unsigned)P) c.ptc = m;
+    }
+  }
+  c.pt = c.valid ? c.ptc : pe;
   c.q = lane >> 4;
   c.x0 = x[(size_t)c.ptc * 3 + 0];
   c.x1 = x[(size_t)c.ptc * 3 + 1];
@@ -158,6 +170,25 @@
     }
   }
   __device__ __forceinline__ void drain() { st.issue(); }
+};
+
+template <class Core>
+struct SoftplusSaveLaneHooks {
+  PendingStores st;
+  bool on;
+  __device__ __forceinline__ SoftplusSaveLaneHooks(float* H) : on(H != nullptr) { st.dst = H; st.n = 0; st.t0 = 0; }
+  __device__ __forceinline__ void pre(const int, const int) { if (on) st.issue(); else st.n = 0; }
+  __device__ __forceinline__ void post(const int o0, const int, const bool pair, v4f& a0, v4f& a1) {
+#pragma unroll
+    for (int r = 0; r < 4; ++r) a0[r] = Core::softplus(a0[r]);
+    st.s0 = a0; st.t0 = o0; st.n = 1;
+    if (pair) {
+#pragma unroll
+      for (int r = 0; r < 4; ++r) a1[r] = Core::softplus(a1[r]);
+      st.s1 = a1; st.n = 2;
+    }
+  }
+  __device__ __forceinline__ void drain() { if (on) st.issue(); else st.n = 0; }
 };
 
 struct GradSweepHooks {
@@ -181,6 +212,39 @@
       for (int r = 0; r < 4; ++r) a0[r] = (1.0f - one_minus_sigmoid_from_h(h0[r])) * a0[r];
       st.s0 = a0; st.t0 = o0; st.n = save ? 1 : 0;
       if (pair && o1 < ot) {
+#pragma unroll
+        for (int r = 0; r < 4; ++r) a1[r] = (1.0f - one_minus_sigmoid_from_h(h1[r])) * a1[r];
+        st.s1 = a1; st.n = save ? 2 : 0;
+      }
+    }
+  }
+  __device__ __forceinline__ void drain() { st.issue(); }
+};
+
+struct GradSweepCopyHooks {
+  const float* HS;
+  float* H;
+  int ot;
+  bool save;
+  v4f h0, h1;
+  PendingStores st;
+  __device__ __forceinline__ GradSweepCopyHooks(const float* HS_, float* H_, float* PM, const int ot_, const bool save_)
+      : HS(HS_), H(H_), ot(ot_), save(save_) { st.dst = PM; st.n = 0; st.t0 = 0; }
+  __device__ __forceinline__ void pre(const int o0, const int o1) {
+    st.issue();
+    if (ot > 0) {
+      h0 = *(const v4f*)(HS + 16 * (o0 < ot ? o0 : ot - 1));
+      h1 = *(const v4f*)(HS + 16 * (o1 < ot ? o1 : ot - 1));
+    }
+  }
+  __device__ __forceinline__ void post(const int o0, const int o1, const bool pair, v4f& a0, v4f& a1) {
+    if (o0 < ot) {
+      *(v4f*)(H + 16 * o0) = h0;
+#pragma unroll
+      for (int r = 0; r < 4; ++r) a0[r] = (1.0f - one_minus_sigmoid_from_h(h0[r])) * a0[r];
+      st.s0 = a0; st.t0 = o0; st.n = save ? 1 : 0;
+      if (pair && o1 < ot) {
+        *(v4f*)(H + 16 * o1) = h1;
 #pragma unroll
         for (int r = 0; r < 4; ++r) a1[r] = (1.0f - one_minus_sigmoid_from_h(h1[r])) * a1[r];
         st.s1 = a1; st.n = save ? 2 : 0;
@@ -254,13 +318,27 @@
   __device__ __forceinline__ void drain() { st.issue(); }
 };
 
-template <class Core>
+struct HSaveArgs {
+  float* H;
+  int P_pad;
+  const int32_t* col_slot;
+  int n_cols, n_slots;
+};
+
+template <class Core, bool SAVE = false>
 __device__ __forceinline__ void sdf_forward_body(const msdf_plan_t& plan, const typename Core::wvec* __restrict__ wpack,
                                                  const float* __restrict__ bpack, const float* __restrict__ x,
                                                  const float* __restrict__ aux, const AuxView av, const int P,
                                                  const float clamp_radius, const float sphere_scale,
-                                                 float* __restrict__ sdf_out, void* lds) {
+                                                 float* __restrict__ sdf_out, void* lds,
+                                                 const HSaveArgs hs = HSaveArgs()) {
   const PointCtx c = load_point<Core>(x, P);
+  int srow = -1;
+  if constexpr (SAVE) {
+    const int ray = c.ptc / hs.n_cols;
+    const int slot = hs.col_slot[c.ptc - ray * hs.n_cols];
+    if (c.valid && slot >= 0 && slot < hs.n_slots) srow = ray * hs.n_slots + slot;
+  }
   v4f in[MT], acc[MT];
   const int in0_tiles = plan.e_tiles + plan.aux_tiles;
   {
@@ -276,7 +354,12 @@
       load_input_tiles<Core::AUX_LEVEL_MAJOR>(in0, plan, aux, av, c);
       place_tiles(in, L.skip_tile, in0, in0_tiles);
     }
-    if constexpr (Core::BIAS_IN_HOOKS) {
+    if constexpr (SAVE) {
+      static_assert(!SAVE || Core::BIAS_IN_HOOKS, "the save kernel exists for the fp32 core");
+      float* Hl = (srow >= 0) ? hs.H + (size_t)L.hpre * hs.P_pad + (size_t)srow * (16 * L.ot) + 4 * c.q : nullptr;
+      Core::gemm_bias(L.ktp, acc, in, L.ot, wpack + L.wf_off, lds, SoftplusSaveLaneHooks<Core>(Hl),
+                      bpack + L.bias_off + 4 * c.q);
+    } else if constexpr (Core::BIAS_IN_HOOKS) {
       Core::gemm_bias(L.ktp, acc, in, L.ot, wpack + L.wf_off, lds, SoftplusHooks<Core>(), bpack + L.bias_off + 4 * c.q);
     } else {
       load_bias(acc, bpack + L.bias_off, L.ot, c.q);
@@ -296,9 +379,19 @@
 typedef msdf_fg_args_t FgArgs;
 
 template <class Core>
+__device__ __forceinline__ bool sdf_fwd_grad_reuses(const msdf_plan_t& plan, const FgArgs& a) {
+  if constexpr (Core::ROW_MAP) {
+    if ((int)((blockIdx.x + 1) * Core::PTS_PER_WG) <= a.n_reuse && plan.n_layers >= 2 && a.smp_flags != nullptr &&
+        a.h_saved != nullptr && a.h_stage != nullptr)
+      return a.smp_flags[1] == 0u && a.h_saved[0] != 0u;
+  }
+  return false;
+}
+
+template <class Core, bool REUSE = false>
 __device__ __forceinline__ void sdf_fwd_grad_body(const msdf_plan_t& plan, const FgArgs& a, void* lds) {
   typedef typename Core::wvec wvec;
-  const PointCtx c = load_point<Core>(a.x, a.P);
+  const PointCtx c = load_point<Core>(a.x, a.P, a.row_map);
   const AuxView av = {a.aux_C, a.aux_LC, a.P};
   v4f in[MT], acc[MT];
   const int nl = plan.n_layers;
@@ -316,7 +409,20 @@
   }
   const bool want_feat = (int)(blockIdx.x * Core::PTS_PER_WG) < a.n_feat;
 
-  for (int l = 0; l < nl - 1; ++l) {
+  auto srow = [&](const msdf_layer_t& L) {
+    return (size_t)L.hpre * (size_t)a.stage_pad + (size_t)eval_row<Core>() * (16 * L.ot) + 4 * c.q;
+  };
+  if constexpr (REUSE) {
+    const msdf_layer_t L = plan.layer[nl - 2];
+    const float* Hs = a.h_stage + srow(L);
+    const int otl = L.ot - 1;
+#pragma unroll
+    for (int t = 0; t < MT; ++t) {
+      const v4f h = *(const v4f*)(Hs + 16 * (t < otl ? t : otl));
+      in[t] = (t < L.ot) ? h : V4ZERO;
+    }
+  }
+  for (int l = 0; l < (REUSE ? 0 : nl - 1); ++l) {
     const msdf_layer_t L = plan.layer[l];
     if (L.skip_tile >= 0) {
       v4f in0[5];
@@ -378,7 +484,7 @@
   auto row = [&](const msdf_layer_t& L) { return (size_t)L.hpre * Pp + (size_t)c.pt * (16 * L.ot) + 4 * c.q; };
   if (nl >= 2) {
     const msdf_layer_t L = plan.layer[nl - 2];
-    const float* Hl = a.H + row(L);
+    const float* Hl = REUSE ? a.h_stage + srow(L) : a.H + row(L);
     float* Pl = a.PM + row(L);
     const int otl = L.ot - 1;
     v4f hh[MT];
@@ -387,6 +493,7 @@
 #pragma unroll
     for (int t = 0; t < MT; ++t) {
       if (t == 0 || t < L.ot) {
+        if constexpr (REUSE) *(v4f*)(a.H + row(L) + 16 * t) = hh[t];
 #pragma unroll
         for (int r = 0; r < 4; ++r) acc[t][r] = (1.0f - one_minus_sigmoid_from_h(hh[t][r])) * acc[t][r];
         if (a.save) *(v4f*)(Pl + 16 * t) = acc[t];
@@ -399,8 +506,13 @@
     for (int t = 0; t < MT; ++t) in[t] = (t < L.ot) ? acc[t] : V4ZERO;
     zero_tiles(acc);
     const msdf_layer_t Lp = plan.layer[l > 0 ? l - 1 : 0];
-    Core::gemm(L.otp, acc, in, L.kt, (const wvec*)a.wpack + L.wb_off, lds,
-               GradSweepHooks(a.H + row(Lp), a.PM + row(Lp), l > 0 ? Lp.ot : 0, a.save != 0));
+    if constexpr (REUSE) {
+      Core::gemm(L.otp, acc, in, L.kt, (const wvec*)a.wpack + L.wb_off, lds,
+                 GradSweepCopyHooks(a.h_stage + srow(Lp), a.H + row(Lp), a.PM + row(Lp), l > 0 ? Lp.ot : 0, a.save != 0));
+    } else {
+      Core::gemm(L.otp, acc, in, L.kt, (const wvec*)a.wpack + L.wb_off, lds,
+                 GradSweepHooks(a.H + row(Lp), a.PM + row(Lp), l > 0 ? Lp.ot : 0, a.save != 0));
+    }
     if (l == 0) take_input_grad(0);
     else if (L.skip_tile >= 0) take_input_grad(L.skip_tile);
   }
@@ -467,7 +579,7 @@
 template <class Core>
 __device__ __forceinline__ void sdf_backward_body(const msdf_plan_t& plan, const BwArgs& a, void* lds) {
   typedef typename Core::wvec wvec;
-  const PointCtx c = load_point<Core>(a.x, a.P);
+  const PointCtx c = load_point<Core>(a.x, a.P, a.row_map);
   const int nl = plan.n_layers;
   const size_t Pp = (size_t)a.P_pad;
   const bool live = c.valid && !(a.clamped != nullptr && a.clamped[c.ptc]);
diff --git a/monosdf_amd/csrc/sdf_mlp.hip b/monosdf_amd/csrc/sdf_mlp.hip
--- a/monosdf_amd/csrc/sdf_mlp.hip
+++ b/monosdf_amd/csrc/sdf_mlp.hip
@@ -56,9 +56,21 @@
 }
 
 __global__ void __launch_bounds__(CoreF32::THREADS, CoreF32::WGS_PER_CU)
+msdf_sdf_forward_save_k(const msdf_plan_t plan, const v4f* __restrict__ wpack, const float* __restrict__ bpack,
+                        const float* __restrict__ x, const float* __restrict__ aux, const AuxView av, const int P,
+                        const float clamp_radius, const float sphere_scale, float* __restrict__ sdf_out,
+                        const uint32_t* __restrict__ run_flag, const HSaveArgs hs, uint32_t* __restrict__ h_saved) {
+  extern __shared__ v4f lds[];
+  if (run_flag != nullptr && *run_flag == 0u) return;
+  if (blockIdx.x == 0 && threadIdx.x == 0) *h_saved = 1u;
+  sdf_forward_body<CoreF32, true>(plan, wpack, bpack, x, aux, av, P, clamp_radius, sphere_scale, sdf_out, lds, hs);
+}
+
+__global__ void __launch_bounds__(CoreF32::THREADS, CoreF32::WGS_PER_CU)
 msdf_sdf_fwd_grad_k(const msdf_plan_t plan, const FgArgs a) {
   extern __shared__ v4f lds[];
-  sdf_fwd_grad_body<CoreF32>(plan, a, lds);
+  if (sdf_fwd_grad_reuses<CoreF32>(plan, a)) sdf_fwd_grad_body<CoreF32, true>(plan, a, lds);
+  else sdf_fwd_grad_body<CoreF32>(plan, a, lds);
 }
 
 __global__ void __launch_bounds__(CoreF32::THREADS, CoreF32::WGS_PER_CU)
@@ -116,6 +128,26 @@
   });
 }
 
+extern "C" int msdf_sdf_forward_save(const msdf_plan_t* plan, const void* wpack, const float* bpack, const float* x,
+                                     const float* aux, int aux_C, int aux_LC, int P, float clamp_radius,
+                                     float sphere_scale, float* sdf, const uint32_t* run_flag, float* H, int P_pad,
+                                     const int32_t* col_slot, int n_cols, int n_slots, uint32_t* h_saved,
+                                     void* stream) {
+  if (plan == nullptr || P < 0 || H == nullptr || col_slot == nullptr || h_saved == nullptr) return MSDF_ERR_ARG;
+  if (plan->precision != MSDF_PRECISION_F32) return MSDF_ERR_UNSUPPORTED;
+  if (n_cols < 1 || n_slots < 1 || n_slots > n_cols || (P % n_cols) != 0 || !padded_ok(0, P_pad) ||
+      (int64_t)(P / n_cols) * n_slots > (int64_t)P_pad)
+    return MSDF_ERR_ARG;
+  if (P == 0) return MSDF_OK;
+  if (plan->aux_tiles > 0 && aux == nullptr) return MSDF_ERR_ARG;
+  if (!aux_layout_ok(plan, aux_C, aux_LC)) return MSDF_ERR_ARG;
+  const AuxView av = {aux_C, aux_LC, P};
+  const HSaveArgs hs = {H, P_pad, col_slot, n_cols, n_slots};
+  return mlp_launch<CoreF32>(msdf_sdf_forward_save_k, (P + CoreF32::PTS_PER_WG - 1) / CoreF32::PTS_PER_WG, stream, *plan,
+                             (const v4f*)wpack, bpack, x, aux, av, P, clamp_radius, sphere_scale, sdf, run_flag, hs,
+                             h_saved);
+}
+
 extern "C" int msdf_sdf_forward_if(const msdf_plan_t* plan, const void* wpack, const float* bpack, const float* x,
                                    const float* aux, int P, float clamp_radius, float sphere_scale, float* sdf,
                                    const uint32_t* run_flag, void* stream) {
@@ -135,6 +167,10 @@
   if (plan->aux_tiles > 0 && a->aux == nullptr) return MSDF_ERR_ARG;
   if (!aux_layout_ok(plan, a->aux_C, a->aux_LC)) return MSDF_ERR_ARG;
   if (a->dy_dx != nullptr && (a->aux_C != 2 || a->r_aux == nullptr)) return MSDF_ERR_ARG;
+  if (a->n_reuse < 0 || (a->n_reuse % CoreF32::PTS_PER_WG) != 0 || a->n_reuse > a->P) return MSDF_ERR_ARG;
+  if (a->n_reuse > 0 && (a->row_map == nullptr || a->n_reuse > a->n_feat || a->h_stage == nullptr ||
+                         a->stage_pad < a->n_reuse))
+    return MSDF_ERR_ARG;
   return mlp_with_core(plan, [&](auto core) {
     typedef decltype(core) Core;
     if (!Core::AUX_LEVEL_MAJOR && (a->aux_C != 0 || a->dy_dx != nullptr)) return MSDF_ERR_UNSUPPORTED;
diff --git a/monosdf_amd/model/network.py b/monosdf_amd/model/network.py
--- a/monosdf_amd/model/network.py
+++ b/monosdf_amd/model/network.py
@@ -124,7 +124,7 @@
         return planlib.build_sdf_plan(shapes, self.skip_in, self.multires, self.aux_cols, self.aux_active,
                                       self.feature_vector_size)
 
-    def evaluate(self, x, n_clamp, n_feat, save=None, split=None):
+    def evaluate(self, x, n_clamp, n_feat, save=None, split=None, reuse=None):
         if save is None:
             save = torch.is_grad_enabled()
         x = x.detach()
@@ -144,7 +144,7 @@
         radius = self.sdf_bounding_sphere if self.clamps else 0.0
         sdf, _, feat, nrm, nrm_b, r_aux = ops.SdfMlpFunction.apply(
             x, aux, flat_w, flat_b, wpack, bpack, fused, int(n_clamp), int(n_feat), radius, self.sphere_scale,
-            bool(save), ns)
+            bool(save), ns, reuse)
         if self.aux_active:
             r_aux = r_aux[:, :self.aux_cols]
             through_grid = self.encoding.input_gradient(handle, r_aux) * (0.5 / self.divide_factor)
@@ -176,8 +176,19 @@
         with torch.no_grad():
             return self._sdf_only(x, clamp=False)[:, 0]
 
-    def _sdf_only(self, x, run_flag=None, clamp=True):
+    def sdf_reuse(self, device, N, S, n_extra, n_eik, save):
+        fused = self.packed(device)[0]
+        if fused.precision != 'fp32' or self.aux_active or N <= 0 or n_extra <= 0:
+            return None
+        return ops.SdfReuse(fused, N, S, n_extra, n_eik, save, device)
+
+    def _sdf_only(self, x, run_flag=None, clamp=True, save_for=None):
         fused, _, _, wpack, bpack = self.packed(x.device)
+        if save_for is not None:
+            reuse, col_slot, n_cols = save_for
+            radius = self.sdf_bounding_sphere if (self.clamps and clamp) else 0.0
+            return ops.sdf_forward_save(fused, wpack, bpack, x.detach(), radius, self.sphere_scale, run_flag, reuse,
+                                        col_slot, n_cols)
         aux, aux_lm = None, None
         if self.aux_active:
             enc = self.encoding
@@ -382,13 +393,17 @@
             mode = self.speculate_rounds
             guess = 0 if not mode else (K if mode == 'all' else min(K, self.ray_sampler.guess_rounds()))
             for attempt in (guess, K if guess else 0):
+                smp = self.ray_sampler
+                reuse = net.sdf_reuse(device, ray_dirs.shape[0], smp.N_samples + smp.N_samples_extra + 2,
+                                      smp.N_samples_extra, 4 * ray_dirs.shape[0] if self.training else 0,
+                                      torch.is_grad_enabled())
                 z_vals, z_samples_eik, x_all = self.ray_sampler.sample(ray_dirs, cam_loc, self, speculate=attempt,
-                                                                      beta0=beta)
+                                                                      beta0=beta, sdf_reuse=reuse)
                 N, S = z_vals.shape
                 P = N * S
                 points_flat = x_all[:P]
                 sdf, feature_vectors, gradients_sdf, grad_eik = net.evaluate(x_all, P, P, save=torch.is_grad_enabled(),
-                                                                                split=P)
+                                                                                split=P, reuse=reuse)
                 rgb_flat = self.rendering_network(points_flat, gradients_sdf, ray_dirs, feature_vectors, indices,
                                                   if_pixel_input=if_pixel_input, samples_per_ray=S)['rgb']
                 rgb = rgb_flat.reshape(-1, S, 3)
diff --git a/monosdf_amd/model/ray_sampler.py b/monosdf_amd/model/ray_sampler.py
--- a/monosdf_amd/model/ray_sampler.py
+++ b/monosdf_amd/model/ray_sampler.py
@@ -93,25 +93,41 @@
                   int(beta.numel() == N and N > 1), N, M, _lib.ptr(out), _lib.stream_ptr())
         return out
 
-    def _extra_columns(self, training, noise, dev):
+    @staticmethod
+    def column_slots(row0, n_eval):
+        row0 = row0.reshape(-1).to(torch.int64)
+        n = row0.numel()
+        if n == 0 or int(row0.min()) < 0 or int(row0.max()) >= n_eval or torch.unique(row0).numel() != n:
+            return None
+        slots = torch.full((n_eval,), -1, dtype=torch.int32)
+        slots[row0] = torch.arange(n, dtype=torch.int32)
+        return slots
+
+    def _extra_columns(self, training, noise, dev, want_slots=False):
         n_extra, n_eval, K = self.N_samples_extra, self.N_samples_eval, self.max_total_iters
         if n_extra <= 0:
-            return torch.zeros(K, 1, device=dev, dtype=torch.int64)
+            return torch.zeros(K, 1, device=dev, dtype=torch.int64), None
         if training:
             given = noise.get('extra_idx')
             if given is not None:
                 given = given.to(device=dev, dtype=torch.int64)
-                if given.dim() == 2:
-                    return given.contiguous()
-                return given.reshape(1, n_extra).expand(K, n_extra).contiguous()
-            host = torch.empty(K, n_extra, dtype=torch.int64, pin_memory=True)
+                table = given.contiguous() if given.dim() == 2 else \
+                    given.reshape(1, n_extra).expand(K, n_extra).contiguous()
+                slots = self.column_slots(table[0].cpu(), n_eval) if want_slots else None
+                return table, (slots.to(dev) if slots is not None else None)
+            words = K * n_extra + (n_eval + 1) // 2
+            host = torch.empty(words, dtype=torch.int64, pin_memory=True)
+            table = host[:K * n_extra].view(K, n_extra)
             for k in range(K):
-                host[k] = torch.randperm(n_eval * (k + 1))[:n_extra]
-            return host.to(dev, non_blocking=True)
+                table[k] = torch.randperm(n_eval * (k + 1))[:n_extra]
+            host[K * n_extra:].view(torch.int32)[:n_eval] = self.column_slots(table[0], n_eval)
+            on_dev = host.to(dev, non_blocking=True)
+            return on_dev[:K * n_extra].view(K, n_extra), on_dev[K * n_extra:].view(torch.int32)[:n_eval]
         key = (str(dev), n_eval, K, n_extra)
         if key not in self._eval_columns:
             rows = [torch.linspace(0, n_eval * (k + 1) - 1, n_extra).long() for k in range(K)]
-            self._eval_columns[key] = torch.stack(rows).to(dev)
+            slots = self.column_slots(rows[0], n_eval)
+            self._eval_columns[key] = (torch.stack(rows).to(dev), slots.to(dev) if slots is not None else None)
         return self._eval_columns[key]
 
     @property
@@ -160,7 +176,7 @@
             return self.max_total_iters
         return max(self._hist[which]) if self._hist[which] else 1
 
-    def sample(self, ray_dirs, cam_loc, model, want_points=True, speculate=0, beta0=None):
+    def sample(self, ray_dirs, cam_loc, model, want_points=True, speculate=0, beta0=None, sdf_reuse=None):
         dev = ray_dirs.device
         ray_dirs, cam_loc = _need_gpu(ray_dirs), _need_gpu(cam_loc)
         self._resolve()
@@ -210,10 +226,19 @@
         a.jitter = jitter.data_ptr() if jitter is not None else None
         a.u_final = u_final.data_ptr() if u_final is not None else None
         a.final_z = final_z.data_ptr()
+        extra_idx = col_slot = None
+        if sdf_reuse is not None:
+            assert want_points and (sdf_reuse.N, sdf_reuse.S, sdf_reuse.n_extra) == (N, S, n_extra)
+            assert sdf_reuse.P == N * S + (4 * N if training else 0)
+            sdf_reuse.flags = flags
+            sdf_reuse.round_pts = pts
+            a.row_map, a.h_saved = sdf_reuse.row_map.data_ptr(), sdf_reuse.h_saved.data_ptr()
+            if sdf_reuse.n_reuse > 0 and speculate in (0, 1):
+                extra_idx, col_slot = self._extra_columns(training, noise, dev, want_slots=True)
         st = _lib.stream_ptr()
         a.M = n_eval
         _lib.call('msdf_sampler_init', C.byref(a), st)
-        z_out = z_eik = x_all = extra_idx = eik_idx = None
+        z_out = z_eik = x_all = eik_idx = None
 
         def prepare_finish():
             nonlocal z_out, z_eik, x_all, extra_idx, eik_idx
@@ -245,7 +270,8 @@
                     nei = nei_drawn.view(2 * N, 3) if nei is None else nei.to(**f32).contiguous()
                     a.eik_uniform, a.nei_rand = eik_uniform.data_ptr(), nei.data_ptr()
                     self._keep = (eik_uniform, nei)
-            extra_idx = self._extra_columns(training, noise, dev)
+            if extra_idx is None:
+                extra_idx = self._extra_columns(training, noise, dev)[0]
             a.extra_idx = extra_idx.data_ptr()
 
         group = self.global_rounds
@@ -254,7 +280,8 @@
         with torch.no_grad():
             while True:
                 run_flag = flags.data_ptr() + 4 * (2 * rounds - 1) if (speculate > 0 and rounds > 0) else None
-                new_sdf = net._sdf_only(pts, run_flag=run_flag)
+                save_for = (sdf_reuse, col_slot, n_eval) if (rounds == 0 and col_slot is not None) else None
+                new_sdf = net._sdf_only(pts, run_flag=run_flag, save_for=save_for)
                 a.new_sdf = new_sdf.data_ptr()
                 a.M, a.round_idx = n_eval * (rounds + 1), rounds
                 _lib.call('msdf_sampler_beta', C.byref(a), st)
diff --git a/monosdf_amd/ops.py b/monosdf_amd/ops.py
--- a/monosdf_amd/ops.py
+++ b/monosdf_amd/ops.py
@@ -229,6 +229,41 @@
     return FusedWeightNormFunction.apply(state, tuple(shapes), *params)
 
 
+REUSE_SAMPLER_H = _os.environ.get('MSDF_REUSE_SAMPLER_H', '1') != '0'
+
+
+class SdfReuse:
+
+    def __init__(self, mlp, N, S, n_extra, n_eik, save, device):
+        self.mlp, self.N, self.S, self.n_extra, self.save = mlp, N, S, n_extra, bool(save)
+        self.P = N * S + n_eik
+        self.P_pad = _pad64(max(self.P, 1))
+        woff, total = planlib.sdf_workspace(mlp.mp, self.P_pad)
+        if not save:
+            total = woff['PM']
+        self.ws = torch.empty(max(total, 64), device=device, dtype=torch.float32)
+        self.stage_pad = _pad64(max(N * n_extra, 1))
+        self.stage = torch.empty(mlp.plan.hsum * self.stage_pad, device=device, dtype=torch.float32) \
+            if REUSE_SAMPLER_H else None
+        self.row_map = torch.empty(max(self.P, 1), device=device, dtype=torch.int32)
+        self.h_saved = torch.empty(1, device=device, dtype=torch.int32)
+        self.flags = None
+        self.round_pts = None
+        self.n_split = N * S
+        self.n_reuse = (N * n_extra) // 64 * 64 if REUSE_SAMPLER_H else 0
+
+
+def sdf_forward_save(mlp, wpack, bpack, x, clamp_radius, sphere_scale, run_flag, reuse, col_slot, n_cols):
+    x = _need_cuda(x, 'points')
+    P = x.shape[0]
+    out = torch.empty(P, 1, device=x.device, dtype=torch.float32)
+    _lib.call('msdf_sdf_forward_save', C.byref(mlp.plan), _lib.ptr(wpack), _lib.ptr(bpack), _lib.ptr(x), None, 0, 0, P,
+              float(clamp_radius), float(sphere_scale), _lib.ptr(out), C.c_void_p(run_flag) if run_flag else None,
+              _lib.ptr(reuse.stage), reuse.stage_pad, _lib.ptr(col_slot), int(n_cols), reuse.n_extra,
+              _lib.ptr(reuse.h_saved), _lib.stream_ptr())
+    return out
+
+
 def sdf_forward_nograd(mlp, wpack, bpack, x, aux, clamp_radius, sphere_scale, run_flag=None, aux_lm=None):
     x = _need_cuda(x, 'points')
     P = x.shape[0]
@@ -245,7 +280,7 @@
 
 
 def _sdf_fwd_grad(x, aux, wpack, bpack, mlp, n_clamp, n_feat, clamp_radius, sphere_scale, save, n_split=None,
-                  aux_lm=None, aux_jac=None):
+                  aux_lm=None, aux_jac=None, reuse=None):
     mp = mlp.mp
     plan = mlp.plan
     x = _need_cuda(x.detach(), 'points')
@@ -257,7 +292,15 @@
     woff, total = planlib.sdf_workspace(mp, P_pad)
     if not save:
         total = woff['PM']
-    ws = torch.empty(max(total, 64), device=dev, dtype=torch.float32)
+    if reuse is not None:
+        ns = P if n_split is None else int(n_split)
+        if not (mlp.precision == 'fp32' and reuse.mlp is mlp and reuse.P == P and reuse.P_pad == P_pad and
+                bool(save) == reuse.save and not has_aux and n_feat == n_clamp == ns == reuse.n_split and
+                reuse.n_reuse <= n_feat and reuse.flags is not None):
+            raise RuntimeError('monosdf_amd: SdfReuse does not describe this SDF evaluation')
+        ws = reuse.ws
+    else:
+        ws = torch.empty(max(total, 64), device=dev, dtype=torch.float32)
     F = 16 * plan.feat_tiles
     sdf = torch.empty(P, 1, device=dev, dtype=torch.float32)
     feat_full = torch.empty(_pad64(max(n_feat, 1)), F, device=dev, dtype=torch.float32)
@@ -284,17 +327,23 @@
     if aux_jac is not None and aC == 2:
         jac_scale = float(aux_jac[1])
         a.dy_dx, a.aux_dx_scale = aux_jac[0].data_ptr(), jac_scale
+    saved = (x, ws, clamped, wpack, bpack)
+    if reuse is not None:
+        a.row_map, a.n_reuse = reuse.row_map.data_ptr(), reuse.n_reuse
+        a.smp_flags, a.h_saved = reuse.flags.data_ptr(), reuse.h_saved.data_ptr()
+        a.h_stage, a.stage_pad = _addr(reuse.stage), reuse.stage_pad
+        saved += (reuse.row_map,)
     if P > 0:
         _lib.call('msdf_sdf_fwd_grad', C.byref(plan), C.byref(a), _lib.stream_ptr())
     ns = P if n_split is None else int(n_split)
     state = _SdfState(mlp, P, P_pad, n_feat, ns, save, has_aux, (int(aC), int(aLC)), aux_shape, jac_scale)
-    return (sdf[:ns], sdf[ns:], feat, nrm[:ns], nrm[ns:], r_aux), (x, ws, clamped, wpack, bpack), state
+    return (sdf[:ns], sdf[ns:], feat, nrm[:ns], nrm[ns:], r_aux), saved, state
 
 
 def _sdf_backward(state, saved, grads, dy_dx=None, gg_out=None, after_sweeps=None):
     if not state.saved:
         raise RuntimeError('monosdf_amd: backward through an inference-mode SDF evaluation')
-    x, ws, clamped, wpack, bpack = saved
+    x, ws, clamped, wpack, bpack, *row_map = saved
     mlp, P, P_pad = state.mlp, state.P, state.P_pad
     mp = mlp.mp
     dev = x.device
@@ -311,6 +360,7 @@
     b.g_feat = _addr(g_feat) if state.n_feat > 0 else None
     b.g_raux = _addr(g_raux) if state.has_aux else None
     b.clamped = clamped.data_ptr()
+    b.row_map = row_map[0].data_ptr() if row_map else None
     base = ws.data_ptr()
     for k in ('H', 'PM', 'QB', 'AB', 'GSDF', 'QLAST'):
         setattr(b, k, base + 4 * woff[k])
@@ -328,10 +378,10 @@
 
     @staticmethod
     def forward(ctx, x, aux, flat_w, flat_b, wpack, bpack, mlp, n_clamp, n_feat, clamp_radius,
-                sphere_scale, save, n_split=None):
+                sphere_scale, save, n_split=None, reuse=None):
         ctx.set_materialize_grads(False)
         outs, saved, ctx.state = _sdf_fwd_grad(x, aux, wpack, bpack, mlp, n_clamp, n_feat, clamp_radius,
-                                               sphere_scale, save, n_split)
+                                               sphere_scale, save, n_split, reuse=reuse)
         ctx.save_for_backward(*saved)
         return outs
 
@@ -340,7 +390,7 @@
     def backward(ctx, *grads):
         g_aux, grad = _sdf_backward(ctx.state, ctx.saved_tensors, grads)
         n_w = ctx.state.mlp.mp.n_w
-        return (None, g_aux, grad[:n_w], grad[n_w:]) + (None,) * 9
+        return (None, g_aux, grad[:n_w], grad[n_w:]) + (None,) * 10
 
 
 def _encode_points(x, divide_factor, embeddings, offsets, enc, pitch, level_major, jacobian):
```

Measured after the change: 120,900 rays/s (median of 6 runs). 1.01x the previous value.
